# big-nacho/patolette

Measured on AMD Instinct MI355X. Metric: Mpixels/sec quantized (256-color ICtCp + KMeans) at 1 GPU; palette ΔE vs ref, higher is better.
Workload: dtype f64

## Files before the change

### include/patolette_amd.h

```cpp
#ifndef PATOLETTE_AMD_H
#define PATOLETTE_AMD_H

#include <stddef.h>
#include <stdint.h>

#include "patolette.h"

#ifdef __cplusplus
extern "C" {
#endif

int  patolette_amd_device_count(void);
int  patolette_amd_set_device(int ordinal);
const char *patolette_amd_last_error(void);
void *patolette_amd_malloc(size_t bytes);
void patolette_amd_free(void *dptr);
int  patolette_amd_memcpy_h2d(void *dst, const void *src, size_t bytes);
int  patolette_amd_memcpy_d2h(void *dst, const void *src, size_t bytes);
int  patolette_amd_synchronize(void);
void patolette_amd_release_workspace(void);
int  patolette_amd_fill_image(double *d_planar, size_t n, uint64_t seed);
int  patolette_amd_fill_weights(double *d_weights, size_t n, uint64_t seed);

void patolette_amd_device(size_t width, size_t height, const double *d_data, const double *d_weights,
// ... 74 lines not shown
void patolette_amd_measure_device(size_t frames, size_t width, size_t height, const unsigned char *d_pixels, int channels,
                                  const void *d_palette_maps, int map_elem_bytes, const double *palette,
                                  const unsigned char *palette_u8, size_t palette_rows, long long skip_index, uint64_t *entry_count,
                                  uint64_t *entry_sse, uint32_t *entry_max_se, uint64_t *frame_count, uint64_t *frame_sse,
                                  uint32_t *frame_max_se, double *frame_d_sum, double *frame_d_max, int *exit_code);

void patolette_amd_gif_lzw(size_t frames, size_t width, size_t height, const unsigned char *maps, const int32_t *rects,
                           int min_code_size, size_t segment, unsigned char *out, size_t capacity, uint64_t *offsets, int *exit_code);
void patolette_amd_gif_lzw_device(size_t frames, size_t width, size_t height, const unsigned char *d_maps, const int32_t *rects,
                                  int min_code_size, size_t segment, unsigned char *out, size_t capacity, uint64_t *offsets,
                                  int *exit_code);

void patolette_amd_rgba(size_t width, size_t height, const unsigned char *pixels, int alpha_threshold, const double *weights,
                        double tile_size, size_t palette_size, const patolette__QuantizationOptions *options, double *palette,
                        unsigned char *palette_rgba, void *palette_map, int map_elem_bytes, unsigned char *quantized,
                        int *transparent_index, int *exit_code);
void patolette_amd_rgba_device(size_t width, size_t height, const unsigned char *d_pixels, int alpha_threshold, const double *d_weights,
                               double tile_size, size_t palette_size, const patolette__QuantizationOptions *options, double *palette,
                               unsigned char *palette_rgba, void *d_palette_map, int map_elem_bytes, unsigned char *d_quantized,
                               int *transparent_index, int *exit_code);

void patolette_amd_remap_rgba_u8(size_t frames, size_t width, size_t height, const unsigned char *pixels, int alpha_threshold,
                                 const double *palette, const unsigned char *palette_u8, size_t palette_rows, int transparent_index,
                                 int mode, double spread, void *palette_map, int map_elem_bytes, unsigned char *quantized,
                                 int *exit_code);
void patolette_amd_remap_rgba_u8_device(size_t frames, size_t width, size_t height, const unsigned char *d_pixels, int alpha_threshold,
                                        const double *palette, const unsigned char *palette_u8, size_t palette_rows,
                                        int transparent_index, int mode, double spread, void *d_palette_map, int map_elem_bytes,
                                        unsigned char *d_quantized, int *exit_code);
int patolette_amd_debug_rgba_stamp_quad(int mode);

size_t patolette_amd_hist_bytes(int weighted);
int patolette_amd_hist_clear(void *d_hist, int weighted);
void patolette_amd_hist_add_u8(void *d_hist, int weighted, size_t frames, size_t width, size_t height, const unsigned char *pixels,
                               int channels, int alpha_threshold, const double *weights, double tile_size, int *exit_code);
void patolette_amd_hist_add_u8_device(void *d_hist, int weighted, size_t frames, size_t width, size_t height, const unsigned char *d_pixels,
                                      int channels, int alpha_threshold, const double *d_weights, double tile_size, int *exit_code);
int patolette_amd_hist_merge(void *d_hist, const void *d_other, int weighted);
void patolette_amd_hist_totals(const void *d_hist, int weighted, uint64_t *pixels, uint64_t *colors, int *exit_code);
void patolette_amd_hist_export(const void *d_hist, int weighted, size_t capacity, unsigned char *colors, uint64_t *counts, double *weights,
                               int *exit_code);
void patolette_amd_hist_palette(const void *d_hist, int weighted, size_t palette_size, const patolette__QuantizationOptions *options,
                                double *palette, unsigned char *palette_u8, int *exit_code);

void patolette_amd_batch(size_t count, size_t width, size_t height, const double *const *data,
                         const double *const *weights, double tile_size, size_t palette_size,
                         const patolette__QuantizationOptions *options, double *const *palettes,
                         size_t *const *palette_maps, int *exit_codes);

void patolette_amd_batch_rows(size_t count, size_t width, size_t height, const double *const *rows,
                              const double *const *weights, double tile_size, size_t palette_size,
                              const patolette__QuantizationOptions *options, double *const *palettes,
                              size_t *const *palette_maps, int *exit_codes);

void patolette_amd_batch_u8(size_t count, size_t width, size_t height, const unsigned char *const *pixels, int channels,
                            const double *const *weights, double tile_size, size_t palette_size,
                            const patolette__QuantizationOptions *options, double *const *palettes,
                            unsigned char *const *palettes_u8, void *const *palette_maps, int map_elem_bytes,
                            unsigned char *const *quantized, int *exit_codes);

void patolette_amd_batch_dmap(size_t count, size_t width, size_t height, const void *const *images, int pixel_format,
                              const double *const *weights, double tile_size, size_t palette_size,
                              const patolette__QuantizationOptions *options, double *const *palettes, void *d_palette_maps,
                              int map_elem_bytes, int *exit_codes);

typedef int (*patolette_amd_allreduce_sum_fn)(void *ctx, void *buffer, size_t count, int dtype);
typedef struct patolette_amd__Comm {
    int rank, size;
    patolette_amd_allreduce_sum_fn allreduce_sum;
    void *ctx;
    int host_buffers;
} patolette_amd__Comm;
void patolette_amd_slice(size_t total_pixels, size_t slice_begin, size_t slice_pixels, const double *slice_data,
                         const double *slice_weights, size_t palette_size, const patolette__QuantizationOptions *options,
                         const patolette_amd__Comm *comm, double *palette, size_t *slice_map, int *exit_code);
void patolette_amd_slice_device(size_t total_pixels, size_t slice_begin, size_t slice_pixels, const double *d_slice_data,
                                const double *d_slice_weights, size_t palette_size, const patolette__QuantizationOptions *options,
                                const patolette_amd__Comm *comm, double *palette, void *d_slice_map, int map_elem_bytes,
                                int *exit_code);
int patolette_amd_set_invariant_sums(int on);
int patolette_amd_set_kmeans_update(int mode);

int patolette_amd_set_split_loop(int mode);
int patolette_amd_set_global_quantiser(int on_device);

int patolette_amd_set_subsample_cache(int on);

int patolette_amd_subsample_indices(size_t n, size_t take, int32_t *out);
int patolette_amd_eigen_sym3(const double a_colmajor[9], double w[3], double z[9]);
int patolette_amd_principal_axis(const double cov6[6], double axis[3]);
int patolette_amd_eigen_sym3_device(const double *a_colmajor, size_t count, double *w, double *z, int *info);
int patolette_amd_pow(const double *x, double y, double *out, size_t n);

enum {
    PAMD_SRGB_TO_ICTCP = 0,
    PAMD_SRGB_TO_CIELUV = 1,
    PAMD_ICTCP_TO_REC2020 = 2,
    PAMD_CIELUV_TO_REC2020 = 3,
    PAMD_SRGB_TO_REC2020 = 4,
    PAMD_REC2020_TO_SRGB = 5,
    PAMD_CIELUV_TO_ICTCP = 6
};
int patolette_amd_convert(int which, double *planar, size_t n);

int patolette_amd_quantize_clusters(const double *colors, const double *weights, size_t n, size_t K,
                                    double *centers, size_t *n_clusters);

int patolette_amd_kmeans_refine(const double *colors, const double *weights, size_t n,
                                double *centers_io, size_t k, int niter, size_t max_samples);
int patolette_amd_debug_km_route(void);

int patolette_amd_nn_map(const double *colors, size_t n, const double *palette, size_t k, size_t *map);
int patolette_amd_debug_nn_route(int route);
int patolette_amd_debug_nn_map_elem(const double *colors, size_t n, const double *palette, size_t k, int map_elem_bytes, int misalign,
                                    void *map);

int patolette_amd_dither(const double *colors, size_t width, size_t height, const double *palette,
                         size_t k, size_t *map);

void patolette_amd_dither_config(int segments, int warm);
void patolette_amd_dither_layout(int lanes);
int patolette_amd_debug_dither_solo_cap(int cap);
int patolette_amd_debug_dither_stall_passes(int n);
int patolette_amd_dither_layout_in_use(size_t width, size_t height, size_t palette_rows);
void patolette_amd_debug_dither_locate(size_t width, size_t height, unsigned long long t, unsigned long long *d, unsigned long long *c);

typedef struct patolette_amd__Stats {
    double ms_total, ms_upload, ms_convert, ms_gq, ms_lq, ms_kmeans, ms_map, ms_download, ms_saliency;
    size_t n_base_clusters;
    size_t n_clusters;
    size_t split_evals;
    size_t split_px;
    size_t lq_rounds;
    size_t kmeans_samples;
    size_t dither_segments;
    size_t dither_repairs;
    size_t dither_rounds;
    size_t dither_through;
    size_t dither_jumps;
    size_t dither_solo;
} patolette_amd__Stats;
void patolette_amd_last_stats(patolette_amd__Stats *out);
size_t patolette_amd_last_map_palette(double *out, size_t capacity_rows);

typedef struct patolette_amd__SplitRecord {
    int32_t row, new_row;
    int32_t split;
    int32_t degenerate;
    uint64_t n, n_left, n_right;
    double sw;
    double axis[3];
    double cov6[6];
    double dist, dist_left, dist_right, benefit;
} patolette_amd__SplitRecord;
typedef struct patolette_amd__SplitTrace {
    int32_t n_base, n_clusters, n_records, stopped_early;
    double gq_axis[3];
    uint64_t gq_cuts[14];
    double gq_cov6[6];
} patolette_amd__SplitTrace;
size_t patolette_amd_last_split_trace(patolette_amd__SplitTrace *hdr, patolette_amd__SplitRecord *recs, size_t capacity);
size_t patolette_amd_last_cluster_centers(double *out, size_t capacity_rows);

int patolette_amd_debug_fault(int which);

int patolette_amd_debug_workspace(int flags);
unsigned long long patolette_amd_debug_late_growths(void);

void patolette_amd_profile_enable(int on);
void patolette_amd_profile_only(const char *kernel_name);
void patolette_amd_profile_sample(int period);
int  patolette_amd_profile_count(void);
int  patolette_amd_profile_get(int i, char *name64, double *total_ms, size_t *launches, double *total_bytes);

#ifdef __cplusplus
}
#endif
#endif
```

### patolette_amd/_native.py

```python
import ctypes as C
import os

HERE = os.path.dirname(os.path.abspath(__file__))
LIB_PATH = os.path.join(HERE, "lib", "libpatolette_amd.so")

dp = C.POINTER(C.c_double)
zp = C.POINTER(C.c_size_t)


class QuantizationOptions(C.Structure):
    _fields_ = [("dither", C.c_bool), ("palette_only", C.c_bool), ("color_space", C.c_int),
                ("kmeans_niter", C.c_int), ("kmeans_max_samples", C.c_size_t), ("verbose", C.c_bool)]


class Stats(C.Structure):
    _fields_ = [(n, C.c_double) for n in ("ms_total", "ms_upload", "ms_convert", "ms_gq", "ms_lq",
                                          "ms_kmeans", "ms_map", "ms_download", "ms_saliency")] + \
               [(n, C.c_size_t) for n in ("n_base_clusters", "n_clusters", "split_evals", "split_px",
                                          "lq_rounds", "kmeans_samples", "dither_segments", "dither_repairs",
                                          "dither_rounds", "dither_through", "dither_jumps", "dither_solo")]

    def as_dict(self):
        return {n: getattr(self, n) for n, _ in self._fields_}

# ... 31 lines not shown
    "patolette_amd_set_device": (C.c_int, [C.c_int]),
    "patolette_amd_last_error": (C.c_char_p, []),
    "patolette_amd_malloc": (C.c_void_p, [C.c_size_t]),
    "patolette_amd_free": (None, [C.c_void_p]),
    "patolette_amd_memcpy_h2d": (C.c_int, [C.c_void_p, C.c_void_p, C.c_size_t]),
    "patolette_amd_memcpy_d2h": (C.c_int, [C.c_void_p, C.c_void_p, C.c_size_t]),
    "patolette_amd_synchronize": (C.c_int, []),
    "patolette_amd_release_workspace": (None, []),
    "patolette_amd_batch_dmap": (None, [C.c_size_t, C.c_size_t, C.c_size_t, C.POINTER(C.c_void_p), C.c_int, C.POINTER(dp), C.c_double,
                                        C.c_size_t, C.POINTER(QuantizationOptions), C.POINTER(dp), C.c_void_p, C.c_int,
                                        C.POINTER(C.c_int)]),
    "patolette_amd_slice": (None, [C.c_size_t, C.c_size_t, C.c_size_t, dp, dp, C.c_size_t, C.POINTER(QuantizationOptions),
                                   C.POINTER(Comm), dp, zp, C.POINTER(C.c_int)]),
    "patolette_amd_slice_device": (None, [C.c_size_t, C.c_size_t, C.c_size_t, C.c_void_p, C.c_void_p, C.c_size_t,
                                          C.POINTER(QuantizationOptions), C.POINTER(Comm), dp, C.c_void_p, C.c_int, C.POINTER(C.c_int)]),
    "patolette_amd_set_invariant_sums": (C.c_int, [C.c_int]),
    "patolette_amd_set_kmeans_update": (C.c_int, [C.c_int]),
    "patolette_amd_set_subsample_cache": (C.c_int, [C.c_int]),
    "patolette_amd_subsample_indices": (C.c_int, [C.c_size_t, C.c_size_t, C.POINTER(C.c_int32)]),
    "patolette_amd_eigen_sym3": (C.c_int, [dp, dp, dp]),
    "patolette_amd_principal_axis": (C.c_int, [dp, dp]),
    "patolette_amd_eigen_sym3_device": (C.c_int, [dp, C.c_size_t, dp, dp, C.POINTER(C.c_int)]),
    "patolette_amd_fill_image": (C.c_int, [C.c_void_p, C.c_size_t, C.c_uint64]),
    "patolette_amd_fill_weights": (C.c_int, [C.c_void_p, C.c_size_t, C.c_uint64]),
    "patolette_amd_device": (None, [C.c_size_t, C.c_size_t, C.c_void_p, C.c_void_p, C.c_size_t,
                                    C.POINTER(QuantizationOptions), dp, C.c_void_p, C.c_int, C.POINTER(C.c_int)]),
    "patolette_amd_quantize": (None, [C.c_size_t, C.c_size_t, dp, dp, C.c_double, C.c_size_t, C.POINTER(QuantizationOptions), dp, zp,
                                      C.POINTER(C.c_int)]),
    "patolette_amd_quantize_rows": (None, [C.c_size_t, C.c_size_t, dp, dp, C.c_double, C.c_size_t, C.POINTER(QuantizationOptions), dp,
                                           zp, C.POINTER(C.c_int)]),
    "patolette_amd_saliency_weights": (C.c_int, [C.c_size_t, C.c_size_t, dp, C.c_double, dp]),
    "patolette_amd_mbd": (C.c_int, [C.c_size_t, C.c_size_t, C.POINTER(C.c_float), C.c_int, C.POINTER(C.c_float)]),
    **_pair("patolette_amd_u8", None, [C.c_size_t, C.c_size_t, C.c_void_p, C.c_int, C.c_void_p, C.c_double, C.c_size_t,
                                       C.POINTER(QuantizationOptions), dp, C.c_void_p, C.c_void_p, C.c_int, C.c_void_p, C.POINTER(C.c_int)]),
    **_pair("patolette_amd_frames_u8", None, [C.c_size_t, C.c_size_t, C.c_size_t, C.c_void_p, C.c_int, C.c_void_p, C.c_double, C.c_size_t,
                                              C.POINTER(QuantizationOptions), dp, C.c_void_p, C.c_void_p, C.c_int, C.c_void_p,
                                              C.POINTER(C.c_int)]),
    **_pair("patolette_amd_remap_u8", None, [C.c_size_t, C.c_size_t, C.c_size_t, C.c_void_p, C.c_int, dp, C.c_void_p, C.c_size_t, C.c_int,
                                             C.c_void_p, C.c_int, C.c_void_p, C.POINTER(C.c_int)]),
    **_pair("patolette_amd_remap_ordered_u8", None, [C.c_size_t, C.c_size_t, C.c_size_t, C.c_void_p, C.c_int, dp, C.c_void_p, C.c_size_t,
                                                     C.c_double, C.c_void_p, C.c_int, C.c_void_p, C.POINTER(C.c_int)]),
    "patolette_amd_debug_remap_two_pass": (C.c_int, [C.c_int]),
    **_pair("patolette_amd_remap_rgba_u8", None, [C.c_size_t, C.c_size_t, C.c_size_t, C.c_void_p, C.c_int, dp, C.c_void_p, C.c_size_t, C.c_int,
                                                  C.c_int, C.c_double, C.c_void_p, C.c_int, C.c_void_p, C.POINTER(C.c_int)]),
    "patolette_amd_debug_rgba_stamp_quad": (C.c_int, [C.c_int]),
    **_pair("patolette_amd_frame_deltas", None, [C.c_size_t, C.c_size_t, C.c_size_t, C.c_void_p, C.c_int, C.c_size_t, C.c_size_t, C.c_void_p,
                                                 C.c_int, dp, C.c_void_p, C.c_double, C.c_void_p, C.c_void_p, C.POINTER(C.c_int32),
                                                 C.POINTER(C.c_uint64), C.POINTER(C.c_int)]),
    **_pair("patolette_amd_frame_deltas_rgba", None, [C.c_size_t, C.c_size_t, C.c_size_t, C.c_void_p, C.c_int, C.c_size_t, C.c_void_p, C.c_int,
                                                      dp, C.c_void_p, C.c_double, C.c_int, C.c_void_p, C.c_void_p, C.POINTER(C.c_int32),
                                                      C.POINTER(C.c_int32), C.POINTER(C.c_uint64), C.POINTER(C.c_int)]),
    "patolette_amd_debug_delta_quad": (C.c_int, [C.c_int]),
    **_pair("patolette_amd_measure", None, [C.c_size_t, C.c_size_t, C.c_size_t, C.c_void_p, C.c_int, C.c_void_p, C.c_int, dp, C.c_void_p,
                                            C.c_size_t, C.c_longlong, C.POINTER(C.c_uint64), C.POINTER(C.c_uint64), C.POINTER(C.c_uint32),
                                            C.POINTER(C.c_uint64), C.POINTER(C.c_uint64), C.POINTER(C.c_uint32), dp, dp,
                                            C.POINTER(C.c_int)]),
    **_pair("patolette_amd_gif_lzw", None, [C.c_size_t, C.c_size_t, C.c_size_t, C.c_void_p, C.POINTER(C.c_int32), C.c_int, C.c_size_t,
                                            C.c_void_p, C.c_size_t, C.POINTER(C.c_uint64), C.POINTER(C.c_int)]),
    **_pair("patolette_amd_rgba", None, [C.c_size_t, C.c_size_t, C.c_void_p, C.c_int, C.c_void_p, C.c_double, C.c_size_t,
                                         C.POINTER(QuantizationOptions), dp, C.c_void_p, C.c_void_p, C.c_int, C.c_void_p,
                                         C.POINTER(C.c_int), C.POINTER(C.c_int)]),
    "patolette_amd_hist_bytes": (C.c_size_t, [C.c_int]),
    "patolette_amd_hist_clear": (C.c_int, [C.c_void_p, C.c_int]),
    **_pair("patolette_amd_hist_add_u8", None, [C.c_void_p, C.c_int, C.c_size_t, C.c_size_t, C.c_size_t, C.c_void_p, C.c_int, C.c_int,
                                                C.c_void_p, C.c_double, C.POINTER(C.c_int)]),
    "patolette_amd_hist_merge": (C.c_int, [C.c_void_p, C.c_void_p, C.c_int]),
    "patolette_amd_hist_totals": (None, [C.c_void_p, C.c_int, C.POINTER(C.c_uint64), C.POINTER(C.c_uint64), C.POINTER(C.c_int)]),
    "patolette_amd_hist_export": (None, [C.c_void_p, C.c_int, C.c_size_t, C.c_void_p, C.POINTER(C.c_uint64), dp, C.POINTER(C.c_int)]),
    "patolette_amd_hist_palette": (None, [C.c_void_p, C.c_int, C.c_size_t, C.POINTER(QuantizationOptions), dp, C.c_void_p,
                                          C.POINTER(C.c_int)]),
    "patolette_amd_batch": (None, [C.c_size_t, C.c_size_t, C.c_size_t, C.POINTER(dp), C.POINTER(dp), C.c_double, C.c_size_t,
                                   C.POINTER(QuantizationOptions), C.POINTER(dp), C.POINTER(zp), C.POINTER(C.c_int)]),
    "patolette_amd_batch_rows": (None, [C.c_size_t, C.c_size_t, C.c_size_t, C.POINTER(dp), C.POINTER(dp), C.c_double, C.c_size_t,
                                        C.POINTER(QuantizationOptions), C.POINTER(dp), C.POINTER(zp), C.POINTER(C.c_int)]),
    "patolette_amd_batch_u8": (None, [C.c_size_t, C.c_size_t, C.c_size_t, C.POINTER(C.c_void_p), C.c_int, C.POINTER(dp), C.c_double, C.c_size_t,
                                      C.POINTER(QuantizationOptions), C.POINTER(dp), C.POINTER(C.c_void_p), C.POINTER(C.c_void_p), C.c_int,
                                      C.POINTER(C.c_void_p), C.POINTER(C.c_int)]),
    "patolette_amd_pow": (C.c_int, [dp, C.c_double, dp, C.c_size_t]),
    "patolette_amd_convert": (C.c_int, [C.c_int, dp, C.c_size_t]),
    "patolette_amd_quantize_clusters": (C.c_int, [dp, dp, C.c_size_t, C.c_size_t, dp, zp]),
    "patolette_amd_kmeans_refine": (C.c_int, [dp, dp, C.c_size_t, dp, C.c_size_t, C.c_int, C.c_size_t]),
    "patolette_amd_nn_map": (C.c_int, [dp, C.c_size_t, dp, C.c_size_t, zp]),
    "patolette_amd_debug_km_route": (C.c_int, []),
    "patolette_amd_debug_nn_route": (C.c_int, [C.c_int]),
    "patolette_amd_debug_nn_map_elem": (C.c_int, [dp, C.c_size_t, dp, C.c_size_t, C.c_int, C.c_int, C.c_void_p]),
    "patolette_amd_set_global_quantiser": (C.c_int, [C.c_int]),
    "patolette_amd_dither": (C.c_int, [dp, C.c_size_t, C.c_size_t, dp, C.c_size_t, zp]),
    "patolette_amd_dither_config": (None, [C.c_int, C.c_int]),
    "patolette_amd_dither_layout": (None, [C.c_int]),
    "patolette_amd_debug_dither_solo_cap": (C.c_int, [C.c_int]),
    "patolette_amd_debug_dither_stall_passes": (C.c_int, [C.c_int]),
    "patolette_amd_dither_layout_in_use": (C.c_int, [C.c_size_t, C.c_size_t, C.c_size_t]),
    "patolette_amd_debug_dither_locate": (None, [C.c_size_t, C.c_size_t, C.c_ulonglong, C.POINTER(C.c_ulonglong),
                                                 C.POINTER(C.c_ulonglong)]),
    "patolette_amd_last_stats": (None, [C.POINTER(Stats)]),
    "patolette_amd_last_map_palette": (C.c_size_t, [dp, C.c_size_t]),
    "patolette_amd_last_split_trace": (C.c_size_t, [C.POINTER(SplitTrace), C.POINTER(SplitRecord), C.c_size_t]),
    "patolette_amd_last_cluster_centers": (C.c_size_t, [dp, C.c_size_t]),
    "patolette_amd_debug_fault": (C.c_int, [C.c_int]),
    "patolette_amd_debug_workspace": (C.c_int, [C.c_int]),
    "patolette_amd_debug_late_growths": (C.c_ulonglong, []),
    "patolette_amd_set_split_loop": (C.c_int, [C.c_int]),
    "patolette_amd_profile_enable": (None, [C.c_int]),
    "patolette_amd_profile_only": (None, [C.c_char_p]),
    "patolette_amd_profile_sample": (None, [C.c_int]),
    "patolette_amd_profile_count": (C.c_int, []),
    "patolette_amd_profile_get": (C.c_int, [C.c_int, C.c_char_p, dp, zp, dp]),
}

_lib = None


def lib():
    global _lib
    if _lib is None:
        if not os.path.exists(LIB_PATH):
            raise ImportError(
                "patolette_amd: %s not found -- build it with `make -C patolette_amd/csrc` "
                "(hipcc, gfx950). There is no CPU fallback." % LIB_PATH)
        L = C.CDLL(LIB_PATH)
        for name, (res, args) in SYMBOLS.items():
            f = getattr(L, name)
            f.restype = res
            f.argtypes = args
        _lib = L
    return _lib


def last_error():
    return lib().patolette_amd_last_error().decode("utf-8", "replace")


def last_stats():
    s = Stats()
    lib().patolette_amd_last_stats(C.byref(s))
    return s.as_dict()


def last_split_trace():
    hdr = SplitTrace()
    n = lib().patolette_amd_last_split_trace(C.byref(hdr), None, 0)
    recs = (SplitRecord * max(1, n))()
    lib().patolette_amd_last_split_trace(C.byref(hdr), recs, n)
    return dict(n_base=hdr.n_base, n_clusters=hdr.n_clusters, stopped_early=bool(hdr.stopped_early),
                gq_axis=[float(v) for v in hdr.gq_axis], gq_cov6=[float(v) for v in hdr.gq_cov6],
                gq_cuts=[int(v) for v in hdr.gq_cuts][:hdr.n_base + 1],
                splits=[dict(row=r.row, new_row=r.new_row, split=r.split, degenerate=r.degenerate, n=r.n, n_left=r.n_left,
                             n_right=r.n_right, sw=r.sw, axis=[float(v) for v in r.axis], cov6=[float(v) for v in r.cov6],
                             dist=r.dist, dist_left=r.dist_left, dist_right=r.dist_right, benefit=r.benefit) for r in recs[:n]])


def last_cluster_centers():
    import numpy as np
    n = lib().patolette_amd_last_cluster_centers(None, 0)
    out = np.zeros((max(1, n), 3), order="F")
    lib().patolette_amd_last_cluster_centers(out.ctypes.data_as(dp), max(1, n))
    return np.ascontiguousarray(out[:n])


def profile(enable=True, only=None, sample=1):
    lib().patolette_amd_profile_only(only.encode() if only else None)
    lib().patolette_amd_profile_sample(int(sample) if only else 1)
    lib().patolette_amd_profile_enable(1 if enable else 0)


def profile_results():
    L = lib()
    out = {}
    for i in range(L.patolette_amd_profile_count()):
        name = C.create_string_buffer(64)
        ms = C.c_double(0)
        n = C.c_size_t(0)
        by = C.c_double(0)
        if L.patolette_amd_profile_get(i, name, C.byref(ms), C.byref(n), C.byref(by)) == 0:
            out[name.value.decode()] = {"total_ms": ms.value, "launches": n.value, "bytes": by.value}
    return out
```

### patolette_amd/csrc/pipeline.hip

```cpp
#include <algorithm>
#include <functional>
#include <chrono>
#include <cmath>
#include <atomic>
#include <memory>
#include <mutex>
#include <thread>
#include <future>
#include <type_traits>

#include "color_device.h"
#include "common.h"
#include "host_math.h"
#include "kmeans.h"
#include "map.h"
#include "ordered.h"
#include "delta.h"
#include "measure.h"
#include "lzw.h"
#include "hist.h"
#include "saliency.h"
#include "quant.h"
#include "rgba.h"
#include "compact.h"
#include "split_frontier.h"
#include "given.h"

namespace pamd {

void launch_convert(int which, const double *src, double *dst, size_t n, ConvertStats *stats, hipStream_t s, BinK sumk = BinK{0.0, 0.0},
                    BinK momk = BinK{0.0, 0.0}, size_t begin = 0, size_t end = ~(size_t)0, bool init_stats = true);
void launch_convert_rows(int which, const double *rows, double *dst, size_t n, ConvertStats *stats, hipStream_t s,
                         BinK sumk = BinK{0.0, 0.0}, BinK momk = BinK{0.0, 0.0}, size_t begin = 0, size_t end = ~(size_t)0,
                         bool init_stats = true);
void launch_convert_u8(int which, const unsigned char *pixels, int channels, double *dst, size_t n, ConvertStats *stats,
                       hipStream_t s, BinK sumk = BinK{0.0, 0.0}, BinK momk = BinK{0.0, 0.0}, size_t begin = 0, size_t end = ~(size_t)0,
                       bool init_stats = true);
void launch_reconstruct(const void *map, int map_elem, size_t n, const unsigned char *pal_u8, int k, unsigned char *out,
                        hipStream_t s);
void launch_weight_stats(const double *w, size_t n, ConvertStats *stats, hipStream_t s);
void launch_pow(const double *x, double y, double *out, size_t n, hipStream_t s);
void launch_fill_image(double *d, size_t n, uint64_t seed, hipStream_t s);
void launch_fill_weights(double *d, size_t n, uint64_t seed, hipStream_t s);

KernelTimer &ktimer() { static thread_local KernelTimer *t = new KernelTimer; return *t; }

std::atomic<int> g_debug_ws{getenv("PAMD_DEBUG_WORKSPACE") ? atoi(getenv("PAMD_DEBUG_WORKSPACE")) & (kWsPoison | kWsCount | kWsLog) : 0};
std::atomic<unsigned long long> g_late_growths{0};
WsStreams &ws_streams() { static thread_local WsStreams w; return w; }
void ws_growth(size_t bytes, const char *file, int line) {
    const int dbg = g_debug_ws.load(std::memory_order_relaxed);
    if (!(dbg & (kWsCount | kWsLog))) return;
    bool queued = false;
    for (const hipStream_t *sp : ws_streams().s)
        if (sp && *sp && hipStreamQuery(*sp) == hipErrorNotReady) queued = true;
    if (!queued) return;
    g_late_growths.fetch_add(1);
    if (dbg & kWsLog) fprintf(stderr, "patolette_amd: workspace growth to %zu bytes while work is queued (%s:%d)\n", bytes, file, line);
}
void ws_poison_dev(void *p, size_t bytes) {
    if (!bytes) return;
    HIP_CHECK(hipMemsetAsync(p, 0xFF, bytes, nullptr));
    HIP_CHECK(hipStreamSynchronize(nullptr));
}
void ws_poison_dev_rows(void *p, size_t pitch, size_t width, size_t rows) {
    if (!width || !rows) return;
    HIP_CHECK(hipMemset2DAsync(p, pitch, 0xFF, width, rows, nullptr));
    HIP_CHECK(hipStreamSynchronize(nullptr));
}
int KernelTimer::id_of(const char *name) {
    for (size_t i = 0; i < names.size(); i++) if (names[i] == name) return (int)i;
    names.emplace_back(name); total_ms.push_back(0); total_bytes.push_back(0); launches.push_back(0);
    return (int)names.size() - 1;
}
hipEvent_t KernelTimer::get_event() {
    if (!pool.empty()) { hipEvent_t e = pool.back(); pool.pop_back(); return e; }
    hipEvent_t e; HIP_CHECK(hipEventCreate(&e)); return e;
}
void KernelTimer::begin(int id, hipStream_t s, double bytes, const double *src) {
    Rec r; r.id = id; r.bytes = bytes; r.src = src; r.a = get_event(); r.b = get_event();
    HIP_CHECK(hipEventRecord(r.a, s));
    pending.push_back(r);
}
void KernelTimer::end(hipStream_t s) { HIP_CHECK(hipEventRecord(pending.back().b, s)); }
void KernelTimer::collect() {
    for (auto &r : pending) {
        float ms = 0;
        if (hipEventSynchronize(r.b) == hipSuccess && hipEventElapsedTime(&ms, r.a, r.b) == hipSuccess && !(r.src && *r.src == 0.0)) {
            total_ms[r.id] += ms; total_bytes[r.id] += r.src ? r.bytes * *r.src : r.bytes; launches[r.id] += 1;
        }
        pool.push_back(r.a); pool.push_back(r.b);
    }
    pending.clear();
}
void KernelTimer::reset() { collect(); names.clear(); total_ms.clear(); total_bytes.clear(); launches.clear(); }

__global__ __launch_bounds__(256) void k_gq_prepare(Tile *tA, int ntA, Tile *tP, int ntP, unsigned long long N, int *round_nodes, int *node_tile0,
                                                    double *hist, unsigned long long nhist, unsigned long long *hsize, unsigned int *hcount) {
    const unsigned long long stride = (unsigned long long)gridDim.x * blockDim.x, t0 = (unsigned long long)blockIdx.x * blockDim.x + threadIdx.x;
    for (unsigned long long i = t0; i < (unsigned long long)ntA; i += stride) {
        const unsigned long long o = i * (unsigned long long)kTileA;
        tA[i] = Tile{o, (unsigned)(N - o < (unsigned long long)kTileA ? N - o : (unsigned long long)kTileA), 0u};
    }
    for (unsigned long long i = t0; i < (unsigned long long)ntP; i += stride) {
        const unsigned long long o = i * (unsigned long long)kTileP;
        tP[i] = Tile{o, (unsigned)(N - o < (unsigned long long)kTileP ? N - o : (unsigned long long)kTileP), 0u};
    }
    for (unsigned long long i = t0; i < nhist; i += stride) hist[i] = 0.0;
    for (unsigned long long i = t0; i < (unsigned long long)kBuckets; i += stride) { hsize[i] = 0ULL; hcount[i] = 0u; }
    if (t0 == 0) { round_nodes[0] = 0; node_tile0[0] = 0; node_tile0[1] = ntP; }
}

__global__ void k_put_nodes(NodeDev *table, const NodeIn *stage, const int *ids, int n) {
    int i = blockIdx.x * blockDim.x + threadIdx.x;
    if (i >= n) return;
    const NodeIn in = stage[i];
    NodeDev &d = table[ids[i]];
    d.begin = in.begin; d.n = in.n; d.gn = in.gn; d.buf = in.buf; d.slot = in.slot; d.child0 = in.child0; d.nchild = in.nchild;
    for (int j = 0; j < 3; j++) { d.axis[j] = in.axis[j]; d.mean[j] = in.mean[j]; }
    d.sw = in.sw; d.klin = in.klin; d.kquad = in.kquad;
    node_reset_outputs(d);
    d.split = in.split; d.psplit = -1;
}
__global__ void k_put_node1(NodeDev *table, const int id, const NodeIn in) {
    NodeDev &d = table[id];
    d.begin = in.begin; d.n = in.n; d.gn = in.gn; d.buf = in.buf; d.slot = in.slot; d.child0 = in.child0; d.nchild = in.nchild;
    for (int j = 0; j < 3; j++) { d.axis[j] = in.axis[j]; d.mean[j] = in.mean[j]; }
    d.sw = in.sw; d.klin = in.klin; d.kquad = in.kquad;
    node_reset_outputs(d);
    d.split = in.split; d.psplit = -1;
}
__global__ void k_get_nodes(const NodeDev *table, NodeOut *stage, const int *ids, int n) {
    int i = blockIdx.x * blockDim.x + threadIdx.x;
    if (i >= n) return;
    const NodeDev &d = table[ids[i]];
    NodeOut o;
    o.begin = d.begin; o.n = d.n; o.gn = d.gn; o.buf = d.buf; o.degenerate = d.degenerate; o.split = d.split; o.psplit = d.psplit;
    o.sw = d.sw;
    for (int j = 0; j < 3; j++) o.mean[j] = d.mean[j];
    for (int q = 0; q < 7; q++) {
        double s0 = 0, s1 = 0;
        for (int k = 0; k < kSlots; k++) { s0 += d.acc[k][q][0]; s1 += d.acc[k][q][1]; }
        o.acc[q][0] = s0; o.acc[q][1] = s1;
    }
    stage[i] = o;
}

struct RoundSetup {
    const NodeIn *recs; const int *ids; const int *tA0; const int *tP0;
    int nr, ntA, ntP;
    Tile *tilesA, *tilesP;
    double *hist; size_t nhist;
    unsigned long long *hsize; unsigned int *hcount; size_t nbk;
};
__device__ __forceinline__ int node_of_tile(const int *t0, int nr, int t) {
    int lo = 0, hi = nr;
    while (hi - lo > 1) { const int mid = (lo + hi) >> 1; if (t0[mid] <= t) lo = mid; else hi = mid; }
    return lo;
}
__global__ __launch_bounds__(256) void k_round_setup(NodeDev *table, RoundSetup a) {
    const size_t tid = (size_t)blockIdx.x * blockDim.x + threadIdx.x, stride = (size_t)gridDim.x * blockDim.x;
    for (size_t i = tid; i < (size_t)a.nr; i += stride) {
        const NodeIn in = a.recs[i];
        NodeDev &d = table[a.ids[i]];
        d.begin = in.begin; d.n = in.n; d.gn = in.gn; d.buf = in.buf; d.slot = in.slot; d.child0 = in.child0; d.nchild = in.nchild;
        for (int j = 0; j < 3; j++) { d.axis[j] = in.axis[j]; d.mean[j] = in.mean[j]; }
        d.sw = in.sw; d.klin = in.klin; d.kquad = in.kquad;
    }
    for (size_t i = tid; i < (size_t)a.nr * kNodeResetElems; i += stride)
        node_reset_element(table[a.ids[i / kNodeResetElems]], (int)(i % kNodeResetElems));
    for (size_t t = tid; t < (size_t)a.ntA; t += stride) {
        const int r = node_of_tile(a.tA0, a.nr, (int)t);
        const unsigned long long o = (unsigned long long)((int)t - a.tA0[r]) * kTileA, n = a.recs[r].n;
        a.tilesA[t] = Tile{a.recs[r].begin + o, (unsigned)(n - o < (unsigned long long)kTileA ? n - o : kTileA), (unsigned)a.ids[r]};
    }
    for (size_t t = tid; t < (size_t)a.ntP; t += stride) {
        const int r = node_of_tile(a.tP0, a.nr, (int)t);
        const unsigned long long o = (unsigned long long)((int)t - a.tP0[r]) * kTileP, n = a.recs[r].n;
        a.tilesP[t] = Tile{a.recs[r].begin + o, (unsigned)(n - o < (unsigned long long)kTileP ? n - o : kTileP), (unsigned)a.ids[r]};
    }
    for (size_t i = tid; i < a.nhist; i += stride) a.hist[i] = 0.0;
    for (size_t i = tid; i < a.nbk; i += stride) { a.hsize[i] = 0ULL; a.hcount[i] = 0u; }
}


struct GqOut { int kbase, error, pad[2]; int cuts[16]; unsigned long long ticks[8]; };

constexpr int kLqDevMaxK = 256;
constexpr int kLqNodeCap = 16 * kLqDevMaxK + 256;
constexpr int kLqRoundCap = 512;
constexpr int kLqMaxRounds = 96;

struct LqCen { double mean[3]; double gn; };
// ... 576 lines not shown
    for (int k = 0; k < kSlots; k++) { a = d.minkey[k] < a ? d.minkey[k] : a; b = d.maxkey[k] > b ? d.maxkey[k] : b; }
    for (int r = 0; r < size; r++) {
        unsigned long long *row = buf + ((size_t)r * n + i) * 3;
        row[0] = r == rank ? a : 0ULL; row[1] = r == rank ? b : 0ULL; row[2] = r == rank ? d.n : 0ULL;
    }
}
__global__ void k_shard_unpack_keys(NodeDev *table, const int *ids, int n, int rank, int size, const unsigned long long *buf) {
    const int i = blockIdx.x * blockDim.x + threadIdx.x;
    if (i >= n) return;
    NodeDev &d = table[ids[i]];
    unsigned long long a = ~0ULL, b = 0ULL, before = 0ULL;
    for (int r = 0; r < size; r++) {
        const unsigned long long *row = buf + ((size_t)r * n + i) * 3;
        a = row[0] < a ? row[0] : a; b = row[1] > b ? row[1] : b;
        if (r < rank) before += row[2];
    }
    for (int k = 0; k < kSlots; k++) { d.minkey[k] = ~0ULL; d.maxkey[k] = 0ULL; }
    d.minkey[0] = a; d.maxkey[0] = b; d.gslot0 = before;
}
__global__ void k_shard_pack_acc(const NodeDev *table, const int *ids, int n, double *buf) {
    const int i = blockIdx.x * blockDim.x + threadIdx.x;
    if (i >= n) return;
    const NodeDev &d = table[ids[i]];
    for (int q = 0; q < 7; q++) {
        double s0 = 0, s1 = 0;
        for (int k = 0; k < kSlots; k++) { s0 += d.acc[k][q][0]; s1 += d.acc[k][q][1]; }
        buf[(size_t)i * 14 + 2 * q] = s0; buf[(size_t)i * 14 + 2 * q + 1] = s1;
    }
}
__global__ void k_shard_unpack_acc(NodeDev *table, const int *ids, int n, const double *buf) {
    const int i = blockIdx.x * blockDim.x + threadIdx.x;
    if (i >= n) return;
    NodeDev &d = table[ids[i]];
    for (int q = 0; q < 7; q++) {
        for (int k = 1; k < kSlots; k++) { d.acc[k][q][0] = 0; d.acc[k][q][1] = 0; }
        d.acc[0][q][0] = buf[(size_t)i * 14 + 2 * q]; d.acc[0][q][1] = buf[(size_t)i * 14 + 2 * q + 1];
    }
}
__global__ void k_shard_children_local(NodeDev *table, const int *round_nodes, int nround) {
    const int i = blockIdx.x * blockDim.x + threadIdx.x;
    if (i >= nround) return;
    const NodeDev &nd = table[round_nodes[i]];
    for (int k = 0; k < nd.nchild; k++) {
        NodeDev &ch = table[nd.child0 + k];
        ch.begin = nd.cbegin[k]; ch.n = nd.cbegin[k + 1] - nd.cbegin[k];
    }
}

struct Bounds {
    double cmax, range, wmax; int e_lin, e_quad; double lo[3], hi[3];
    bool have_sum = false; double sum[3] = {0, 0, 0};
    bool have_mom = false;
    double sum2[3][2] = {{0, 0}, {0, 0}, {0, 0}}, mom2[6][2] = {{0, 0}, {0, 0}, {0, 0}, {0, 0}, {0, 0}, {0, 0}};
    bool nonfinite = false;
    double wmin = 0; bool bad_w = false;
};

static int exp_bound(double v) {
    if (!(v > 0) || !std::isfinite(v)) return 1;
    return std::ilogb(v) + 1;
}

struct Shard {
    size_t total = 0, begin = 0;
    patolette_amd__Comm comm{};
};

struct Engine {
    int device = -1;
    hipStream_t stream = nullptr;
    const Shard *shard = nullptr;
    bool invariant = false;
    DevBuf<unsigned char> commbuf;
    PinBuf<unsigned char> h_comm;
    DevBuf<int> shard_ids;
    PinBuf<float> h_cent;
    PinBuf<ConvertStats> h_cstats;
    hipEvent_t ev_stats = nullptr;
    hipStream_t stream2 = nullptr;
    hipEvent_t ev_up[2] = {nullptr, nullptr}, ev_join = nullptr;
    size_t prep_N = 0, prep_planes = 0;
    DevBuf<double> src, wsrc, cvt, bufA, bufB, aux;
    DevBuf<unsigned short> bkt;
    DevBuf<NodeDev> nodes;
    DevBuf<NodeIn> stage_in;
    DevBuf<NodeOut> stage_out;
    DevBuf<int> ids, round_nodes, node_tile0;
    DevBuf<Tile> tilesA, tilesP;
    DevBuf<double> hist, sum6, dpal;
    DevBuf<unsigned long long> hsize, tileoff;
    DevBuf<unsigned int> hcount, tilecnt;
    DevBuf<unsigned char> lut, dmap, src8, pal8, quant8;
    DevBuf<unsigned char> dl_maps, dl_shown;
    DevBuf<unsigned long long> dl_words, dl_masks;
    DevBuf<unsigned long long> ms_words;
    DevBuf<MeasureTile> ms_tiles;
    DevBuf<unsigned> ms_p8;
    DevBuf<LzwFrame> lz_frames;
    DevBuf<unsigned> lz_stage, lz_bits, lz_out;
    DevBuf<unsigned long long> lz_gbit, lz_words;
    DevBuf<unsigned> rgba_cnt;
    DevBuf<int> rgba_cpos;
    DevBuf<unsigned char> rgba_rgb, rgba_map;
    DevBuf<double> rgba_w;
    PinBuf<unsigned> h_rgba_m;
    DevBuf<unsigned> rr_words;
    PinBuf<unsigned> h_rr_words;
    DevBuf<unsigned long long> hs_units, hs_words, hs_counts;
    DevBuf<unsigned> hs_tiles;
    DevBuf<unsigned char> hs_rgb;
    DevBuf<double> hs_w;
    DevBuf<ConvertStats> cstats;
    PinBuf<NodeIn> h_stage_in;
    PinBuf<NodeOut> h_stage_out;
    PinBuf<int> h_ids, h_ids_get;
    PinBuf<int> h_round;
    PinBuf<double> h_dbl;
    PinBuf<unsigned char> h_bytes, h_packet, h_mapstage;
    DevBuf<unsigned char> packet;
    KMeansWork km;
    NNWork nn;
    SalWork sal;
    DevBuf<double> wsal;
    DevBuf<GqDpDev> gq;
    PinBuf<GqDpDev> h_gq;
    DevBuf<GqOut> gqout;
    PinBuf<GqOut> h_gqout;
    PinBuf<double> h_pal;
    DevBuf<LqCtl> lqctl;
    PinBuf<LqHead> h_lqhead;
    PinBuf<LqRec> h_lqrec;
    PinBuf<LqCen> h_lqcen;
    std::vector<LqRec> lq_rec_local;
    std::vector<LqCommit> lq_commits;
    bool trace_pending = false;
    size_t lq_hint_N = 0, lq_hint_K = 0; int lq_hint_rounds = 0;
    DevBuf<int> perm_dev;
    size_t perm_N = 0, perm_nx = 0;
    PinBuf<int32_t> h_perm;
    size_t hperm_N = 0, hperm_nx = 0;
    hm::PermScratch perm_ws;
    std::future<void> perm_job;
    patolette_amd__Stats stats{};
    double ms_saliency = 0.0;
    std::string last_error;
    std::vector<double> map_palette;
    patolette_amd__SplitTrace trace_hdr{};
    std::vector<patolette_amd__SplitRecord> trace;
    std::vector<double> cluster_centers;

    void init() {
        if (stream) return;
        int cnt = 0;
        if (hipGetDeviceCount(&cnt) != hipSuccess || cnt <= 0)
            throw HipError("patolette_amd: no HIP device available (this library has no CPU fallback)");
        if (device < 0) { HIP_CHECK(hipGetDevice(&device)); }
        HIP_CHECK(hipSetDevice(device));
        HIP_CHECK(hipStreamCreateWithFlags(&stream, hipStreamNonBlocking));
    }
    void sync() { HIP_CHECK(hipStreamSynchronize(stream)); if (ktimer().enabled) ktimer().collect(); }
    ~Engine() {
        if (stream) { (void)hipSetDevice(device); (void)hipStreamSynchronize(stream); if (ev_stats) (void)hipEventDestroy(ev_stats);
                      for (hipEvent_t e : {ev_up[0], ev_up[1], ev_join}) if (e) (void)hipEventDestroy(e);
                      if (stream2) (void)hipStreamDestroy(stream2);
                      (void)hipStreamDestroy(stream); }
    }
// ... 126 lines not shown
    NodeIn d;
    std::memset(&d, 0, sizeof d);
    d.begin = h.begin; d.n = h.n; d.gn = h.gn; d.buf = h.buf; d.slot = -1; d.child0 = -1; d.nchild = 0; d.split = -1;
    for (int j = 0; j < 3; j++) d.mean[j] = h.mean[j];
    d.sw = h.sw;
    int P = 1;
    while ((1ULL << P) < (h.gn > 1 ? h.gn : 2)) P++;
    d.klin = make_bink(b.e_lin, P);
    d.kquad = make_bink(b.e_quad, P);
    return d;
}

static void put_nodes(Engine &E, const std::vector<int> &ids, const std::vector<NodeIn> &recs) {
    const int n = (int)ids.size();
    if (!n) return;
    if (n == 1) {
        hipLaunchKernelGGL(k_put_node1, 1, 1, 0, E.stream, E.nodes.p, ids[0], recs[0]);
        HIP_CHECK(hipGetLastError());
        return;
    }
    E.stage_in.reserve(n); E.ids.reserve(n); E.h_stage_in.reserve(n); E.h_ids.reserve(n);
    std::memcpy(E.h_stage_in.p, recs.data(), n * sizeof(NodeIn));
    std::memcpy(E.h_ids.p, ids.data(), n * sizeof(int));
    HIP_CHECK(hipMemcpyAsync(E.stage_in.p, E.h_stage_in.p, n * sizeof(NodeIn), hipMemcpyHostToDevice, E.stream));
    HIP_CHECK(hipMemcpyAsync(E.ids.p, E.h_ids.p, n * sizeof(int), hipMemcpyHostToDevice, E.stream));
    hipLaunchKernelGGL(k_put_nodes, (n + 63) / 64, 64, 0, E.stream, E.nodes.p, E.stage_in.p, E.ids.p, n);
    HIP_CHECK(hipGetLastError());
}

static void get_nodes(Engine &E, const std::vector<int> &ids, std::vector<NodeOut> &recs) {
    const int n = (int)ids.size();
    recs.resize(n);
    if (!n) return;
    E.stage_out.reserve(n); E.ids.reserve(n); E.h_stage_out.reserve(n); E.h_ids_get.reserve(n);
    std::memcpy(E.h_ids_get.p, ids.data(), n * sizeof(int));
    HIP_CHECK(hipMemcpyAsync(E.ids.p, E.h_ids_get.p, n * sizeof(int), hipMemcpyHostToDevice, E.stream));
    hipLaunchKernelGGL(k_get_nodes, (n + 63) / 64, 64, 0, E.stream, E.nodes.p, E.stage_out.p, E.ids.p, n);
    HIP_CHECK(hipGetLastError());
    HIP_CHECK(hipMemcpyAsync(E.h_stage_out.p, E.stage_out.p, n * sizeof(NodeOut), hipMemcpyDeviceToHost, E.stream));
    E.sync();
    std::memcpy(recs.data(), E.h_stage_out.p, n * sizeof(NodeOut));
}

static void get_nodes_dev(Engine &E, const int *d_ids, int n, std::vector<NodeOut> &recs) {
    recs.resize(n);
    if (!n) return;
    E.h_stage_out.reserve(n);
    hipLaunchKernelGGL(k_get_nodes, (n + 63) / 64, 64, 0, E.stream, E.nodes.p, E.h_stage_out.p, d_ids, n);
    HIP_CHECK(hipGetLastError());
    E.sync();
    std::memcpy(recs.data(), E.h_stage_out.p, n * sizeof(NodeOut));
}

static void absorb_moments(HNode &h, const NodeOut &d) {
    for (int q = 0; q < 6; q++) h.cov6[q] = d.acc[q][0] + d.acc[q][1];
    h.dist = d.acc[6][0] + d.acc[6][1];
}

static bool node_axis(const HNode &h, double axis[3]) {
    if (h.axis_state != 0) {
        for (int j = 0; j < 3; j++) axis[j] = h.axis[j];
        return h.axis_state > 0;
    }
    double c6[6];
    for (int q = 0; q < 6; q++) c6[q] = h.cov6[q] / h.sw;
    return hm::principal_axis(c6, axis);
}

static void leaf_bound(HNode &h) {
    h.ub = h.dist;
    h.axis_state = 0;
    if (h.gn <= 1 || !(h.sw > 0)) { h.ub = 0; return; }
    double c6[6];
    for (int q = 0; q < 6; q++) c6[q] = h.cov6[q] / h.sw;
    double a[9] = {c6[0], c6[1], c6[2], c6[1], c6[3], c6[4], c6[2], c6[4], c6[5]};
    double w[3];
    if (hm::eigen_sym3(a, w) != 0) { h.axis_state = -1; return; }
    h.axis[0] = a[6]; h.axis[1] = a[7]; h.axis[2] = a[8]; h.axis_state = 1;
    const double b = w[2] * h.sw * (1.0 + 1e-9) + 1e-9 * h.dist;
    if (b == b && b < h.ub) h.ub = b;
}

struct QuantSizes {
    size_t bufA, bufB, bkt, tilesA, tilesP, tilecnt, tileoff, hist, hsize, hcount, lut;
    QuantSizes(size_t pixels, size_t planes, size_t nodes) {
        const size_t slack = nodes > 1 ? nodes : 0;
        bufA = bufB = planes * pixels + 64;
        bkt = pixels;
        tilesA = ceil_div(pixels, (size_t)kTileA) + slack; tilesP = ceil_div(pixels, (size_t)kTileP) + slack;
        tilecnt = tileoff = tilesP * kMaxChildren;
        hist = std::max(hist_slot_doubles(), (size_t)kNQ_LQ * 2 * kBuckets * nodes);
        hsize = hcount = lut = nodes * kBuckets;
    }
};
static void reserve_quant_tables(Engine &E, const QuantSizes &z, const char *file = __builtin_FILE(), int line = __builtin_LINE()) {
    E.bufA.reserve(z.bufA, file, line); E.bufB.reserve(z.bufB, file, line); E.bkt.reserve(z.bkt, file, line);
    E.tilesA.reserve(z.tilesA, file, line); E.tilesP.reserve(z.tilesP, file, line);
    E.tilecnt.reserve(z.tilecnt, file, line); E.tileoff.reserve(z.tileoff, file, line);
    E.hist.reserve(z.hist, file, line); E.hsize.reserve(z.hsize, file, line); E.hcount.reserve(z.hcount, file, line); E.lut.reserve(z.lut, file, line);
}

static void gq_prepare(Engine &E, size_t N, bool weighted) {
    hipStream_t s = E.stream;
    const size_t planes = weighted ? 4 : 3;
    const QuantSizes z(N, planes, 1);
    reserve_quant_tables(E, z);
    const int ntA = (int)z.tilesA, ntP = (int)z.tilesP;
    E.h_round.reserve(kBuckets);
    E.round_nodes.reserve(1); E.node_tile0.reserve(2);
    const size_t hs = hist_slot_doubles();
    hipLaunchKernelGGL(k_gq_prepare, 64, 256, 0, s, E.tilesA.p, ntA, E.tilesP.p, ntP, (unsigned long long)N, E.round_nodes.p, E.node_tile0.p,
                       E.hist.p, (unsigned long long)hs, E.hsize.p, E.hcount.p);
    HIP_CHECK(hipGetLastError());
    E.prep_N = N; E.prep_planes = planes;
}



std::atomic<int> g_lq_device{getenv("PAMD_LQ_DEVICE") ? atoi(getenv("PAMD_LQ_DEVICE")) : 2};
std::atomic<int> g_gq_device{getenv("PAMD_GQ_DEVICE") ? atoi(getenv("PAMD_GQ_DEVICE")) : 1};
constexpr size_t kLqDeviceAutoPixels = (size_t)40 << 20;

static bool lq_device_eligible(const Engine &E, size_t N, size_t K, bool verbose, bool allow_device) {
    const int lq_mode = g_lq_device.load(std::memory_order_relaxed);
    return allow_device && (lq_mode == 1 || (lq_mode == 2 && N < kLqDeviceAutoPixels)) && !E.shard && !verbose && K <= (size_t)kLqDevMaxK;
}

static void ws_prepare(Engine &E, size_t N, size_t K, bool weighted, bool verbose) {
    const size_t planes = weighted ? 4 : 3;
    const bool lq_dev = lq_device_eligible(E, N, K, verbose, true);
    E.cvt.reserve(planes * N); E.cstats.reserve(1);
    reserve_quant_tables(E, QuantSizes(N, planes, lq_dev ? (size_t)kLqRoundCap : 1));
    E.round_nodes.reserve(1); E.node_tile0.reserve(2); E.h_round.reserve(kBuckets);
    E.nodes.reserve(std::max<size_t>(4 * K + 64, lq_dev ? (size_t)kLqNodeCap : 0));
    E.h_dbl.reserve(16 * kBuckets * 2 + 64);
    E.gq.reserve(1); E.gqout.reserve(1); E.h_gqout.reserve(1); E.h_gq.reserve(1);
    const size_t nput = kGqMaxK + 1;
    E.stage_in.reserve(nput); E.stage_out.reserve(nput); E.ids.reserve(nput); E.h_stage_in.reserve(nput); E.h_stage_out.reserve(nput);
    E.h_ids.reserve(nput); E.h_ids_get.reserve(nput);
    E.h_cent.reserve(3 * K);
    if (lq_dev) { E.lqctl.reserve(1); E.h_lqhead.reserve(1); E.h_lqrec.reserve(kLqNodeCap); E.h_lqcen.reserve(kLqNodeCap); }
}

static int lq_device_loop(Engine &E, size_t N, size_t K, bool weighted, bool inv_sums, const Bounds &bnd, const QuantBuffers &qlq, int kbase,
                          int first_base, int nnodes, std::vector<double> &centers, size_t &len, unsigned long long *max_members) {
    hipStream_t s = E.stream;
    const size_t lqs = (size_t)kNQ_LQ * 2 * kBuckets;
    const QuantSizes z(N, weighted ? 4 : 3, kLqRoundCap);
    const int ntA_ub = (int)z.tilesA, ntP_ub = (int)z.tilesP;
    E.lqctl.reserve(1); E.h_lqhead.reserve(1); E.h_lqrec.reserve(kLqNodeCap); E.h_lqcen.reserve(kLqNodeCap);
    reserve_quant_tables(E, z);
    LqCtl *c = E.lqctl.p;
    LqHead *head = E.h_lqhead.p;
    for (int r = 0; r < kLqMaxRounds; r++) { head->round_px[r] = 0.0; head->round_nr[r] = 0.0; }
    const RoundDyn *dyn = &c->dyn;
    const int *d_round = c->round_ids, *d_tP0 = c->tP0;
    int call = 0;
    const GqOut *gq = kbase < 0 ? (const GqOut *)E.gqout.p : nullptr;
    const int kb_ub = kbase < 0 ? kGqMaxK : kbase;
    auto control = [&]() {
        const bool first = call == 0;
        {
            KTIME("k_lq_children", s, 0.0);
            if (first) hipLaunchKernelGGL(k_lq_children, (kb_ub + 3) / 4, 256, 0, s, E.nodes.p, c, call, kb_ub, first_base, nnodes, (int)K, gq);
            else hipLaunchKernelGGL(k_lq_children, 2 * kLqRoundCap / 4, 256, 0, s, E.nodes.p, c, call, 0, 0, 0, 0, (const GqOut *)nullptr);
        }
        KTIME("k_lq_select", s, 0.0);
        hipLaunchKernelGGL(k_lq_select, 1 + (first ? (kb_ub + 3) / 4 : 2 * kLqRoundCap / 4), 256, 0, s, E.nodes.p, c, call, bnd.e_lin, bnd.e_quad);
        HIP_CHECK(hipGetLastError());
        call++;
    };
    int enq = 0;
    auto round = [&]() {
        if (enq >= kLqMaxRounds) throw HipError("patolette_amd: split loop exceeded its round limit");
        const double *px_src = &head->round_px[enq], *nr_src = &head->round_nr[enq];
        const bool rev = enq % 2 == 1;
        static const bool setup_kernel = getenv("PAMD_LQ_SETUP_KERNEL") && atoi(getenv("PAMD_LQ_SETUP_KERNEL")) != 0;
        if (setup_kernel) {
            hipLaunchKernelGGL(k_round_setup_dyn, 1024, 256, 0, s, E.nodes.p, (const LqCtl *)c, E.tilesA.p, E.tilesP.p, E.hist.p, E.hsize.p, E.hcount.p, lqs);
            HIP_CHECK(hipGetLastError());
            launch_minmax(qlq, E.tilesA.p, ntA_ub, 0, E.nodes.p, s, rev, dyn, px_src);
        } else {
            const RoundLists rl{c->round_ids, c->tA0, c->tP0, E.tilesA.p, E.tilesP.p, E.hist.p, lqs, E.hsize.p, E.hcount.p};
            launch_minmax(qlq, E.tilesA.p, ntA_ub, 0, E.nodes.p, s, rev, dyn, px_src, &rl);
        }
        launch_hist(qlq, false, E.tilesA.p, ntA_ub, 0, E.nodes.p, E.hist.p, E.hsize.p, E.hcount.p, s, !rev, false, dyn, px_src);
        launch_cut(weighted, E.nodes.p, d_round, kLqRoundCap, E.hist.p, E.hsize.p, E.hcount.p, E.lut.p, s, dyn, nr_src);
        launch_partition(qlq, E.tilesP.p, ntP_ub, 0, d_round, d_tP0, kLqRoundCap, E.nodes.p, E.lut.p, E.tilecnt.p, E.tileoff.p, true, s, inv_sums, rev, dyn, px_src);
        enq++;
        control();
    };
    control();
    int want = (E.lq_hint_N == N && E.lq_hint_K == K && E.lq_hint_rounds > 0) ? E.lq_hint_rounds : 9;
    const bool fault_full = g_debug_fault.load(std::memory_order_relaxed) == 4;
    if (fault_full) want = 3;
    for (;;) {
        while (enq < want) round();
        hipLaunchKernelGGL(k_lq_export, 16, 256, 0, s, (const LqCtl *)c, head, E.h_lqrec.p, E.h_lqcen.p);
        HIP_CHECK(hipGetLastError());
        E.sync();
        if (fault_full) return -2;
        if (head->done) break;
        want = enq + 2;
    }
    if (head->error == 2) return -2;
    if (head->error == 3) return -1;
    if (kbase < 0) kbase = E.h_gqout.p->kbase;
    E.lq_hint_N = N; E.lq_hint_K = K; E.lq_hint_rounds = head->rounds;
    LqReplay rp;
    const double t_rp0 = now_ms();
    E.lq_rec_local.resize((size_t)head->nnodes);
    std::memcpy(E.lq_rec_local.data(), E.h_lqrec.p, (size_t)head->nnodes * sizeof(LqRec));
    const int fault = g_debug_fault.load(std::memory_order_relaxed);
    const bool replay_ok = lq_replay(E.lq_rec_local.data(), kbase, first_base, K, kDelta, fault, rp);
    const double t_rp1 = now_ms();
    static const bool replay_check = getenv("PAMD_LQ_REPLAY_CHECK") != nullptr;
    if (replay_check || !replay_ok) {
        LqReplay ref;
        const bool ref_ok = lq_replay_plain(E.lq_rec_local.data(), kbase, first_base, K, kDelta, fault, ref);
        if (ref_ok != replay_ok || ref.result != rp.result || ref.stopped_early != rp.stopped_early)
            fprintf(stderr, "patolette_amd: split loop: the two replays DISAGREE (plain %d, %zu rows; blocked %d, %zu rows), kbase %d, K %zu, nodes %d, rounds %d\n",
                    (int)ref_ok, ref.result.size(), (int)replay_ok, rp.result.size(), kbase, K, head->nnodes, head->rounds);
        else if (!replay_ok)
            fprintf(stderr, "patolette_amd: split loop: both replays blocked after %zu commits, kbase %d, K %zu, nodes %d, rounds %d, evaluated %d, tau %.17g\n",
                    rp.commits.size(), kbase, K, head->nnodes, head->rounds, head->neval, head->tau);
    }
    if (!replay_ok) throw HipError("patolette_amd: split loop: the replay met an unevaluated node");
    len = rp.result.size();
    centers.assign(3 * len, 0.0);
    unsigned long long mg = 0;
    for (size_t i = 0; i < len; i++) {
        const LqCen &cn = E.h_lqcen.p[rp.result[i]];
        for (int j = 0; j < 3; j++) centers[(size_t)j * len + i] = cn.mean[j];
        mg = std::max(mg, (unsigned long long)cn.gn);
    }
    if (max_members) *max_members = mg;
    E.stats.split_evals = (size_t)head->split_evals; E.stats.split_px = (size_t)head->split_px; E.stats.lq_rounds = (size_t)head->rounds;
    E.lq_commits.swap(rp.commits);
    E.trace.clear();
    E.trace_pending = true;
    E.trace_hdr.stopped_early = rp.stopped_early ? 1 : 0;
    static const bool lq_times = getenv("PAMD_LQ_TIMES") != nullptr;
    if (lq_times) {
        fprintf(stderr, "patolette_amd: device-driven split loop: %d rounds, %d evaluated, %zu commits, tau %.3g; host replay %.1f us\n", head->rounds, head->neval,
                E.lq_commits.size(), head->tau, 1e3 * (t_rp1 - t_rp0));
        if (gq) {
            const unsigned long long *t = E.h_gqout.p->ticks;
            fprintf(stderr, "patolette_amd: k_gq_control us: prefixes %.1f, axis %.1f, search %.1f, records %.1f\n", (t[1] - t[0]) * 0.01, (t[2] - t[1]) * 0.01,
                    (t[3] - t[2]) * 0.01, (t[4] - t[3]) * 0.01);
            fprintf(stderr, "patolette_amd: k_gq_control us: of the prefixes, staging %.1f\n", (t[5] - t[0]) * 0.01);
        }
    }
    return 0;
}

static void materialise_trace(Engine &E) {
    if (!E.trace_pending) return;
    E.trace_pending = false;
    const int n = (int)E.lq_commits.size();
    E.trace.assign(n, patolette_amd__SplitRecord{});
    if (!n) return;
    DevBuf<LqCommit> dc; DevBuf<patolette_amd__SplitRecord> dr;
    dc.reserve(n); dr.reserve(n);
    HIP_CHECK(hipMemcpyAsync(dc.p, E.lq_commits.data(), sizeof(LqCommit) * n, hipMemcpyHostToDevice, E.stream));
    hipLaunchKernelGGL(k_lq_trace, (n + 63) / 64, 64, 0, E.stream, (const NodeDev *)E.nodes.p, (const LqCommit *)dc.p, n, dr.p);
    HIP_CHECK(hipGetLastError());
    HIP_CHECK(hipMemcpyAsync(E.trace.data(), dr.p, sizeof(patolette_amd__SplitRecord) * n, hipMemcpyDeviceToHost, E.stream));
    HIP_CHECK(hipStreamSynchronize(E.stream));
}

struct QuantCall {
// ... 9 lines not shown
    double t0;
    std::vector<HNode> hn;
    bool mom_path = false;
    double axis[3] = {0, 0, 0};
    int kbase = 0;
    std::vector<int> base_ids;
    std::vector<NodeOut> got;
};

static void gq_root_mean(QuantCall &C) {
    Engine &E = C.E;
    const size_t Nt = C.Nt;
    const Bounds &bnd = C.bnd;
    HNode root; root.begin = 0; root.n = C.N; root.gn = Nt; root.buf = 0; root.sw = (double)Nt;
    E.h_dbl.reserve(16 * kBuckets * 2 + 64);
    if (bnd.have_sum) {
        const double inv = 1 / (double)Nt;
        for (int j = 0; j < 3; j++) root.mean[j] = bnd.sum[j] * inv;
    } else {
        int rootP = 1; while ((1ULL << rootP) < (Nt > 1 ? Nt : 2)) rootP++;
        E.sum6.reserve(kSum3Slots * 6);
        launch_sum3(E.cvt.p, C.N, make_bink(bnd.e_lin, rootP), E.sum6.p, E.stream);
        if (C.sh) comm_sum_dev(E, E.sum6.p, kSum3Slots * 6, 0);
        HIP_CHECK(hipMemcpyAsync(E.h_dbl.p, E.sum6.p, kSum3Slots * 6 * sizeof(double), hipMemcpyDeviceToHost, E.stream));
        E.sync();
        const double inv = 1 / (double)Nt;
        for (int j = 0; j < 3; j++) {
            double p0 = 0, p1 = 0;
            for (int sl = 0; sl < kSum3Slots; sl++) { p0 += E.h_dbl.p[sl * 6 + 2 * j]; p1 += E.h_dbl.p[sl * 6 + 2 * j + 1]; }
            root.mean[j] = (p0 + p1) * inv;
        }
    }
    C.hn.push_back(root);
}

static void gq_root_covariance(QuantCall &C) {
    Engine &E = C.E;
    const Bounds &bnd = C.bnd;
    std::vector<HNode> &hn = C.hn;
    C.mom_path = bnd.have_mom && !C.sh;
    if (C.mom_path) {
        const long double nn = (long double)C.Nt;
        long double s1[3], c6[6], s2d[3] = {0, 0, 0};
        for (int j = 0; j < 3; j++) s1[j] = (long double)bnd.sum2[j][0] + (long double)bnd.sum2[j][1];
        static const int ja[6] = {0, 1, 2, 1, 2, 2}, jb[6] = {0, 0, 0, 1, 1, 2};
        for (int q = 0; q < 6; q++) {
            const long double s2 = (long double)bnd.mom2[q][0] + (long double)bnd.mom2[q][1];
            if (ja[q] == jb[q]) s2d[ja[q]] = s2;
            c6[q] = s2 - s1[ja[q]] * s1[jb[q]] / nn;
        }
        const long double tr = c6[0] + c6[3] + c6[5], tr2 = s2d[0] + s2d[1] + s2d[2];
        if (!(tr > 1e-6L * tr2) || c6[0] < 0 || c6[3] < 0 || c6[5] < 0) C.mom_path = false;
        else {
            for (int q = 0; q < 6; q++) hn[0].cov6[q] = (double)c6[q];
            hn[0].dist = (double)tr;
        }
    }
    if (!C.mom_path) {
        NodeIn d = make_nodedev(hn[0], bnd);
        put_nodes(E, {0}, {d});
        launch_cov_nodes(C.qroot, E.cvt.p, E.tilesA.p, C.ntA0, C.N, E.nodes.p, E.stream, true);
        if (C.sh) shard_exchange_acc(E, shard_upload_ids(E, {0}), 1);
        get_nodes(E, {0}, C.got);
        absorb_moments(hn[0], C.got[0]);
    }
}

static bool gq_root_histogram(QuantCall &C) {
    Engine &E = C.E;
    hipStream_t s = E.stream;
    const HNode &root = C.hn[0];
    if (!node_axis(root, C.axis)) return false;
    E.trace.clear();
    E.trace_pending = false;
    E.trace_hdr = patolette_amd__SplitTrace{};
    for (int j = 0; j < 3; j++) E.trace_hdr.gq_axis[j] = C.axis[j];
    for (int q = 0; q < 6; q++) E.trace_hdr.gq_cov6[q] = root.cov6[q] / root.sw;
    {
        NodeIn d = make_nodedev(root, C.bnd);
        for (int j = 0; j < 3; j++) d.axis[j] = C.axis[j];
        d.slot = 0;
        put_nodes(E, {0}, {d});
    }
    launch_minmax(C.qroot, E.tilesA.p, C.ntA0, C.N, E.nodes.p, s, C.mom_path);
    if (C.sh) shard_exchange_keys(E, shard_upload_ids(E, {0}), 1);
    launch_hist(C.qroot, true, E.tilesA.p, C.ntA0, C.N, E.nodes.p, E.hist.p, E.hsize.p, E.hcount.p, s, !C.mom_path, C.Nt >= ((size_t)1 << 18));
    if (C.sh) { comm_sum_dev(E, E.hist.p, C.hs, 0); comm_sum_dev(E, E.hcount.p, kBuckets, 2); }
    return true;
}

static void gq_trace_header(Engine &E) {
    const GqOut &o = *E.h_gqout.p;
    E.trace_hdr.n_base = o.kbase;
    for (int j = 0; j <= o.kbase && j < 14; j++) E.trace_hdr.gq_cuts[j] = (size_t)o.cuts[j];
}

static int finish_device_loop(QuantCall &C, int kbase, int first_base, int nnodes) {
    Engine &E = C.E;
    if (kbase >= 0) E.stats.n_base_clusters = (size_t)kbase;
    E.stats.ms_gq = now_ms() - C.t0;
    C.t0 = now_ms();
    const int rc = lq_device_loop(E, C.N, C.K, C.weighted, C.inv_sums, C.bnd, C.qlq, kbase, first_base, nnodes, C.centers, C.len, C.max_members);
    if (kbase < 0) {
        gq_trace_header(E);
        E.stats.n_base_clusters = (size_t)E.h_gqout.p->kbase;
    }
    if (rc != 0) return rc;
    E.stats.n_clusters = C.len;
    E.trace_hdr.n_clusters = (int32_t)C.len; E.trace_hdr.n_records = (int32_t)E.lq_commits.size();
    E.cluster_centers = C.centers;
    E.stats.ms_lq = now_ms() - C.t0;
    return 0;
}

constexpr int kHostLoop = 1;

static int gq_device_turn(QuantCall &C) {
    Engine &E = C.E;
    hipStream_t s = E.stream;
    E.gq.reserve(1); E.gqout.reserve(1); E.h_gqout.reserve(1);
    *E.h_gqout.p = GqOut{};
    {
        KTIME("k_gq_control", s, (double)C.hs * 8);
        hipLaunchKernelGGL(k_gq_control, 1, 1024, 0, s, (const double *)E.hist.p, (const unsigned int *)E.hcount.p, E.gq.p, (int)std::min<size_t>(C.K, (size_t)1 << 30),
                           C.weighted ? 1 : 0, E.nodes.p, 1, E.lut.p, E.gqout.p, E.h_gqout.p);
        HIP_CHECK(hipGetLastError());
    }
    launch_partition(C.qroot, E.tilesP.p, C.ntP0, C.N, E.round_nodes.p, E.node_tile0.p, 1, E.nodes.p, E.lut.p, E.tilecnt.p, E.tileoff.p, true, s, C.inv_sums,
                     C.mom_path, nullptr, nullptr, true);
    launch_cov_children(C.qroot, E.tilesA.p, C.ntA0, C.N, E.nodes.p, s, !C.mom_path, true);
    if (C.dev_eligible) return finish_device_loop(C, -1, 1, 0);
    std::vector<int> all(kGqMaxK);
    for (int j = 0; j < kGqMaxK; j++) all[j] = 1 + j;
    get_nodes(E, all, C.got);
    if (E.h_gqout.p->error) return -1;
    gq_trace_header(E);
    C.kbase = E.h_gqout.p->kbase;
    for (int j = 0; j < C.kbase; j++) {
        const NodeOut &g = C.got[j];
        HNode c; c.buf = 1; c.begin = g.begin; c.n = g.n; c.gn = g.gn; c.sw = g.sw;
        for (int q = 0; q < 3; q++) c.mean[q] = g.mean[q];
        absorb_moments(c, g);
        leaf_bound(c);
        C.base_ids.push_back((int)C.hn.size());
        C.hn.push_back(c);
    }
    return kHostLoop;
}

static int gq_host_turn(QuantCall &C) {
    Engine &E = C.E;
    hipStream_t s = E.stream;
    const size_t K = C.K, hs = C.hs;
    const bool weighted = C.weighted;
    std::vector<HNode> &hn = C.hn;
    const int gq_kmax = (int)std::min<size_t>(K, kGqMaxK);
    E.gq.reserve(1); E.h_gq.reserve(1);
    launch_gq_dp(E.hist.p, E.hcount.p, gq_kmax, E.gq.p, s);
    HIP_CHECK(hipMemcpyAsync(E.h_gq.p->cut, E.gq.p->cut, sizeof(E.h_gq.p->cut), hipMemcpyDeviceToHost, s));
    std::vector<double> hh(hs);
    std::vector<unsigned int> hc(kBuckets);
    HIP_CHECK(hipMemcpyAsync(E.h_dbl.p, E.hist.p, hs * sizeof(double), hipMemcpyDeviceToHost, s));
    E.h_round.reserve(kBuckets);
    HIP_CHECK(hipMemcpyAsync(E.h_round.p, E.hcount.p, kBuckets * sizeof(unsigned int), hipMemcpyDeviceToHost, s));
    E.sync();
    std::memcpy(hh.data(), E.h_dbl.p, hs * sizeof(double));
    std::memcpy(hc.data(), E.h_round.p, kBuckets * sizeof(unsigned int));
// ... 106 lines not shown
    leaf_bound(c);
}

static double lq_round_threshold(const SplitFrontier &F, size_t K) {
    double thr = std::max(kDelta, kSpecBeta * F.reference_benefit());
    const size_t R = K - F.count;
    std::vector<double> kb;
    F.known_values(kb);
    if (kb.size() >= R && R > 0) {
        std::nth_element(kb.begin(), kb.begin() + (R - 1), kb.end(), std::greater<double>());
        thr = std::max(thr, kb[R - 1] * (1.0 - 1e-9));
    }
    return thr;
}

static void lq_host_round(QuantCall &C, LqHostLoop &L) {
    Engine &E = C.E;
    hipStream_t s = E.stream;
    std::vector<HNode> &hn = C.hn;
    LqLaps &laps = L.laps;
    const HnRec rec{hn};
    const double thr = lq_round_threshold(L.F, C.K);
    laps.lap(laps.greedy);
    std::vector<int> round;
    {
        std::vector<int> keep;
        for (int id : L.leaves) {
            HNode &h = hn[id];
            if (hn_known(h)) continue;
            if (h.ub >= thr) round.push_back(id); else keep.push_back(id);
        }
        L.leaves.swap(keep);
    }
    if (round.empty()) {
        throw HipError("patolette_amd: split loop blocked without candidates");
    }
    laps.lap(laps.select);
    HIP_CHECK(hipStreamSynchronize(s));
    E.nodes.grow(hn.size() + 2 * round.size() + 2, hn.size());
    std::vector<int> todo;
    std::vector<NodeIn> recs;
    for (int id : round) {
        double ax[3];
        if (!node_axis(hn[id], ax)) { hn[id].nosplit = true; continue; }
        NodeIn d = make_nodedev(hn[id], C.bnd);
        for (int j = 0; j < 3; j++) d.axis[j] = ax[j];
        d.slot = (int)todo.size();
        d.child0 = (int)hn.size(); d.nchild = 2;
        hn[id].left = (int)hn.size(); hn[id].right = (int)hn.size() + 1;
        hn.push_back(HNode()); hn.push_back(HNode());
        todo.push_back(id); recs.push_back(d);
    }
    L.F.reload(rec);
    laps.lap(laps.axes);
    if (todo.empty()) return;
    const int nr = (int)todo.size();
    size_t rpx = 0;
    for (int id : todo) rpx += hn[id].n;
    static const bool lq_trace = getenv("PAMD_LQ_TRACE") != nullptr;
    if (lq_trace) fprintf(stderr, "patolette_amd: split round %zu: %d nodes, %zu pixels (%.2f of the image), %zu of %zu colours committed\n",
                          E.stats.lq_rounds + 1, nr, rpx, (double)rpx / (double)(C.N ? C.N : 1), L.F.count, C.K);
    std::vector<int> cids;
    for (int id : todo) { cids.push_back(hn[id].left); cids.push_back(hn[id].right); }
    std::vector<int> tAg = {0}, tPg = {0};
    for (int id : todo) {
        const unsigned long long n = hn[id].n;
        tAg.push_back(tAg.back() + (int)((n + kTileA - 1) / kTileA)); tPg.push_back(tPg.back() + (int)((n + kTileP - 1) / kTileP));
    }
    const int ntA = tAg[nr], ntP = tPg[nr];
    const size_t o_recs = 0, o_ids = o_recs + (size_t)nr * sizeof(NodeIn), o_cids = o_ids + (size_t)nr * sizeof(int),
                 o_tA = o_cids + cids.size() * sizeof(int), o_tP = o_tA + tAg.size() * sizeof(int),
                 pk_bytes = o_tP + tPg.size() * sizeof(int);
    E.h_packet.reserve(pk_bytes); E.packet.reserve(pk_bytes);
    const size_t lqs = (size_t)kNQ_LQ * 2 * kBuckets;
    reserve_quant_tables(E, QuantSizes(C.N, C.weighted ? 4 : 3, (size_t)nr));
    E.h_stage_out.reserve(cids.size());
    std::memcpy(E.h_packet.p + o_recs, recs.data(), (size_t)nr * sizeof(NodeIn));
    std::memcpy(E.h_packet.p + o_ids, todo.data(), (size_t)nr * sizeof(int));
    std::memcpy(E.h_packet.p + o_cids, cids.data(), cids.size() * sizeof(int));
    std::memcpy(E.h_packet.p + o_tA, tAg.data(), tAg.size() * sizeof(int));
    std::memcpy(E.h_packet.p + o_tP, tPg.data(), tPg.size() * sizeof(int));
    laps.lap(laps.packet);
    HIP_CHECK(hipMemcpyAsync(E.packet.p, E.h_packet.p, pk_bytes, hipMemcpyHostToDevice, s));
    const bool rev = E.stats.lq_rounds % 2 == 1;
    const int *d_ids = (const int *)(E.packet.p + o_ids), *d_cids = (const int *)(E.packet.p + o_cids);
    const int *d_tA0 = (const int *)(E.packet.p + o_tA), *d_tP0 = (const int *)(E.packet.p + o_tP);
    RoundSetup rs{(const NodeIn *)(E.packet.p + o_recs), d_ids, d_tA0, d_tP0, nr, ntA, ntP,
                  E.tilesA.p, E.tilesP.p, E.hist.p, lqs * nr, E.hsize.p, E.hcount.p, (size_t)nr * kBuckets};
    {
        const size_t work = std::max<size_t>(std::max<size_t>(std::max<size_t>(ntP, lqs * nr / 4), (size_t)nr * kNodeResetElems), 256);
        hipLaunchKernelGGL(k_round_setup, (unsigned)std::min<size_t>((work + 255) / 256, 2048), 256, 0, s, E.nodes.p, rs);
        HIP_CHECK(hipGetLastError());
    }
    launch_minmax(C.qlq, E.tilesA.p, ntA, rpx, E.nodes.p, s, rev);
    if (C.sh) shard_exchange_keys(E, d_ids, nr);
    launch_hist(C.qlq, false, E.tilesA.p, ntA, rpx, E.nodes.p, E.hist.p, E.hsize.p, E.hcount.p, s, !rev);
    if (C.sh) {
        comm_sum_dev(E, E.hist.p, lqs * nr, 0);
        if (C.weighted) comm_sum_dev(E, E.hsize.p, (size_t)nr * kBuckets, 1);
        comm_sum_dev(E, E.hcount.p, (size_t)nr * kBuckets, 2);
    }
    launch_cut(C.weighted, E.nodes.p, d_ids, nr, E.hist.p, E.hsize.p, E.hcount.p, E.lut.p, s);
    launch_partition(C.qlq, E.tilesP.p, ntP, rpx, d_ids, d_tP0, nr, E.nodes.p, E.lut.p, E.tilecnt.p, E.tileoff.p, true, s, C.inv_sums, rev);
    if (C.sh) {
        hipLaunchKernelGGL(k_shard_children_local, (nr + 63) / 64, 64, 0, s, E.nodes.p, d_ids, nr);
        HIP_CHECK(hipGetLastError());
        shard_exchange_acc(E, d_cids, 2 * nr);
    }
    laps.lap(laps.enqueue);
    get_nodes_dev(E, d_cids, (int)cids.size(), C.got);
    laps.lap(laps.wait);
    for (size_t i = 0; i < cids.size(); i++) absorb_child(hn[cids[i]], C.got[i]);
    for (int id : todo) { hn[id].split_done = true; E.stats.split_evals++; E.stats.split_px += hn[id].n; }
    for (int id : cids) L.leaves.push_back(id);
    L.F.reload(rec);
    E.stats.lq_rounds++;
    laps.lap(laps.children);
}

static void lq_host_loop(QuantCall &C, LqHostLoop &L) {
    Engine &E = C.E;
    const std::vector<HNode> &hn = C.hn;
    const HnRec rec{hn};
    SplitFrontier &F = L.F;
    E.stats.split_evals = 0; E.stats.split_px = 0; E.stats.lq_rounds = 0;
    if (F.count >= C.K) return;
    while (F.count < C.K) {
        const SplitFrontier::Step st = F.step(rec, g_debug_fault.load(std::memory_order_relaxed));
        if (st.status == SplitFrontier::kBlocked) { lq_host_round(C, L); continue; }
        if (st.status == SplitFrontier::kStopped) { E.trace_hdr.stopped_early = 1; break; }
        const HNode &h = hn[st.commit.node];
        const int l = st.commit.left, r = l + 1;
        patolette_amd__SplitRecord tr{};
        tr.row = st.commit.row; tr.new_row = st.commit.new_row;
        tr.split = hn[l].psplit < 0 ? -1 : (hn[l].psplit & 0xffff); tr.degenerate = hn[l].psplit < 0 ? 0 : (hn[l].psplit >> 16) & 1;
        tr.n = h.gn; tr.n_left = hn[l].gn; tr.n_right = hn[r].gn; tr.sw = h.sw;
        for (int j = 0; j < 3; j++) tr.axis[j] = h.axis[j];
        for (int q = 0; q < 6; q++) tr.cov6[q] = h.cov6[q] / h.sw;
        tr.dist = h.dist; tr.dist_left = hn[l].dist; tr.dist_right = hn[r].dist; tr.benefit = st.benefit;
        E.trace.push_back(tr);
        if (C.verbose) { printf("patolette ======== Processed colors: %zu\r", F.count); fflush(stdout); }
    }
    const LqLaps &t = L.laps;
    if (t.on) fprintf(stderr, "patolette_amd: split loop host ms: greedy %.3f select %.3f axes %.3f packet %.3f enqueue %.3f wait(gpu) %.3f children %.3f\n",
                      t.greedy, t.select, t.axes, t.packet, t.enqueue, t.wait, t.children);
}

static void lq_host_epilogue(QuantCall &C, const SplitFrontier &F) {
    Engine &E = C.E;
    const std::vector<HNode> &hn = C.hn;
    const size_t len = C.len = F.count;
    C.centers.assign(3 * len, 0.0);
    for (size_t i = 0; i < len; i++) for (int j = 0; j < 3; j++) C.centers[(size_t)j * len + i] = hn[F.result[i]].mean[j];
    if (C.max_members) { *C.max_members = 0; for (size_t i = 0; i < len; i++) *C.max_members = std::max(*C.max_members, hn[F.result[i]].gn); }
    E.stats.n_clusters = len;
    E.trace_hdr.n_clusters = (int32_t)len; E.trace_hdr.n_records = (int32_t)E.trace.size();
    E.cluster_centers = C.centers;
    E.stats.ms_lq = now_ms() - C.t0;
}

static int quantize_clusters_run(Engine &E, size_t N, size_t K, bool weighted, const Bounds &bnd,
                                 std::vector<double> &centers, size_t &len, bool verbose, unsigned long long *max_members, bool allow_device) {
    const size_t planes = weighted ? 4 : 3;
    const Shard *sh = E.shard;
    if (E.prep_N != N || E.prep_planes != planes) gq_prepare(E, N, weighted);
    E.prep_N = 0;
    const bool dev_eligible = lq_device_eligible(E, N, K, verbose, allow_device);
    E.nodes.reserve(std::max<size_t>(4 * K + 64, dev_eligible ? (size_t)kLqNodeCap : 0));
    const QuantSizes root(N, planes, 1);
    QuantCall C{E, N, sh ? sh->total : N, K, weighted, sh || E.invariant, verbose, dev_eligible, sh, bnd, centers, len, max_members,
                QuantBuffers{{E.cvt.p, E.bufA.p}, E.bkt.p, N, weighted}, QuantBuffers{{E.bufB.p, E.bufA.p}, E.bkt.p, N, weighted},
                (int)root.tilesA, (int)root.tilesP, hist_slot_doubles(), now_ms()};
    C.hn.reserve(4 * K + 64);

    gq_root_mean(C);
    gq_root_covariance(C);
    if (!gq_root_histogram(C)) return -1;
    const bool gq_dev = g_gq_device.load(std::memory_order_relaxed) != 0 && !sh && !verbose && K > (size_t)kGqMaxK;
    const int rc = gq_dev ? gq_device_turn(C) : gq_host_turn(C);
    if (rc != kHostLoop) return rc;
    E.stats.n_base_clusters = (size_t)C.kbase;
    if (verbose) printf("patolette ======== Base cluster count: %zu\n", (size_t)C.kbase);
    E.stats.ms_gq = now_ms() - C.t0;
    C.t0 = now_ms();

    LqHostLoop L{SplitFrontier(K, C.kbase, C.base_ids[0], kDelta, HnRec{C.hn}), C.base_ids, LqLaps{}};
    lq_host_loop(C, L);
    lq_host_epilogue(C, L.F);
    return 0;
}

static int quantize_clusters(Engine &E, size_t N, size_t K, bool weighted, const Bounds &bnd,
                             std::vector<double> &centers, size_t &len, bool verbose = false, unsigned long long *max_members = nullptr) {
    WsGuard wg(&E.stream, &E.stream2);
    int rc = quantize_clusters_run(E, N, K, weighted, bnd, centers, len, verbose, max_members, true);
    if (rc == -2) {
        E.prep_N = 0;
        rc = quantize_clusters_run(E, N, K, weighted, bnd, centers, len, verbose, max_members, false);
    }
    return rc;
}

std::atomic<int> g_km_update{-1};
std::atomic<int> g_perm_cache{1};

static void subsample_start(Engine &E, size_t Nt, size_t K, size_t max_samples) {
    if (E.perm_job.valid()) {
        try { E.perm_job.get(); } catch (...) { E.hperm_N = 0; E.hperm_nx = 0; }
    }
    const size_t ms = std::max(max_samples, (size_t)(256 * 256));
    if (K == 0 || Nt < K) return;
    const size_t nxK = K * (size_t)(int)(ms / K);
    if (!(Nt > nxK)) return;
    const size_t take = std::min(ms, Nt);
    if (!g_perm_cache.load(std::memory_order_relaxed)) { E.perm_N = 0; E.perm_nx = 0; E.hperm_N = 0; E.hperm_nx = 0; }
    if (E.perm_N == Nt && E.perm_nx >= nxK) return;
    if (E.hperm_N == Nt && E.hperm_nx >= nxK) return;
    E.h_perm.reserve(take);
    E.hperm_N = 0; E.hperm_nx = 0;
    int32_t *dst = E.h_perm.p;
    hm::PermScratch *ws = &E.perm_ws;
    E.perm_job = std::async(std::launch::async, [dst, Nt, take, ws] { hm::rand_perm_prefix(Nt, take, 1234u, dst, *ws); });
    E.hperm_N = Nt; E.hperm_nx = take;
}
static const int *subsample_list(Engine &E, size_t Nt, size_t nx, hipStream_t s) {
    if (E.perm_job.valid()) {
        try { E.perm_job.get(); } catch (...) { E.hperm_N = 0; E.hperm_nx = 0; throw; }
    }
    if (E.perm_N == Nt && E.perm_nx >= nx) return E.perm_dev.p;
    if (!(E.hperm_N == Nt && E.hperm_nx >= nx)) {
        E.h_perm.reserve(nx);
        hm::rand_perm_prefix(Nt, nx, 1234u, E.h_perm.p, E.perm_ws);
        E.hperm_N = Nt; E.hperm_nx = nx;
    }
    E.perm_dev.reserve(E.hperm_nx);
    HIP_CHECK(hipMemcpyAsync(E.perm_dev.p, E.h_perm.p, E.hperm_nx * sizeof(int), hipMemcpyHostToDevice, s));
    E.perm_N = Nt; E.perm_nx = E.hperm_nx;
    return E.perm_dev.p;
}
static bool km_update_order_free() {
    static const bool env = getenv("PAMD_KMEANS_UPDATE") && atoi(getenv("PAMD_KMEANS_UPDATE")) != 0;
    const int v = g_km_update.load(std::memory_order_relaxed);
    return v < 0 ? env : v != 0;
}
static bool km_domain_ok(const double bound_x, const double bound_c, const bool weighted, const double bound_w, const double min_w, const size_t nx) {
    const double fmax = 3.4028234663852886e38, fmin = 1.1754943508222875e-38;
    const double B = std::max(1.0, std::max(bound_x, bound_c)), m = (double)std::min<size_t>(nx, (size_t)1 << 25);
    if (!(B < fmax) || !(bound_w < fmax)) return false;
    double Cb = 8.0 * B;
    if (weighted) {
        if (min_w > 0 && min_w < fmin) return false;
        const double by_n = std::exp(std::min((double)nx * 0x1p-23, 700.0)) * B;
        Cb = 4.0 * (min_w > 0 ? std::min(by_n, 4.0 * m * (std::max(bound_w, min_w) / min_w) * B) : by_n);
    }
// ... 1955 lines not shown
                         double tile_size, size_t palette_size, const patolette__QuantizationOptions *options, double *const *palettes,
                         size_t *const *palette_maps, int *exit_codes) {
    batch_impl(false, count, width, height, data, weights, tile_size, palette_size, options, palettes, palette_maps, exit_codes);
}
void patolette_amd_batch_rows(size_t count, size_t width, size_t height, const double *const *rows, const double *const *weights,
                              double tile_size, size_t palette_size, const patolette__QuantizationOptions *options,
                              double *const *palettes, size_t *const *palette_maps, int *exit_codes) {
    batch_impl(true, count, width, height, rows, weights, tile_size, palette_size, options, palettes, palette_maps, exit_codes);
}

int patolette_amd_pow(const double *x, double y, double *out, size_t n) {
    return guarded([&](Engine &E) -> int {
        if (n == 0) return 0;
        E.src.reserve(2 * n);
        HIP_CHECK(hipMemcpyAsync(E.src.p, x, n * sizeof(double), hipMemcpyHostToDevice, E.stream));
        launch_pow(E.src.p, y, E.src.p + n, n, E.stream);
        HIP_CHECK(hipMemcpyAsync(out, E.src.p + n, n * sizeof(double), hipMemcpyDeviceToHost, E.stream));
        E.sync();
        return 0;
    });
}

int patolette_amd_convert(int which, double *planar, size_t n) {
    return guarded([&](Engine &E) -> int {
        if (n == 0) return 0;
        E.src.reserve(3 * n); E.aux.reserve(3 * n);
        HIP_CHECK(hipMemcpy(E.src.p, planar, 3 * n * sizeof(double), hipMemcpyHostToDevice));
        launch_convert(which, E.src.p, E.aux.p, n, nullptr, E.stream);
        E.sync();
        HIP_CHECK(hipMemcpy(planar, E.aux.p, 3 * n * sizeof(double), hipMemcpyDeviceToHost));
        return 0;
    });
}

int patolette_amd_quantize_clusters(const double *colors, const double *weights, size_t n, size_t K, double *centers, size_t *n_clusters) {
    return guarded([&](Engine &E) -> int {
        if (n == 0 || K == 0) return -1;
        const bool weighted = weights != nullptr;
        E.src.reserve(3 * n);
        E.cvt.reserve((weighted ? 4 : 3) * n);
        E.cstats.reserve(1);
        HIP_CHECK(hipMemcpy(E.src.p, colors, 3 * n * sizeof(double), hipMemcpyHostToDevice));
        launch_convert(PAMD_COPY, E.src.p, E.cvt.p, n, E.cstats.p, E.stream);
        if (weighted) {
            HIP_CHECK(hipMemcpyAsync(E.cvt.p + 3 * n, weights, n * sizeof(double), hipMemcpyHostToDevice, E.stream));
            launch_weight_stats(E.cvt.p + 3 * n, n, E.cstats.p, E.stream);
        }
        Bounds b = read_bounds(E, weighted);
        E.stats = patolette_amd__Stats{};
        std::vector<double> pal;
        size_t len = 0;
        if (quantize_clusters(E, n, K, weighted, b, pal, len) != 0) return -1;
        for (size_t j = 0; j < 3 * K; j++) centers[j] = NAN;
        for (int j = 0; j < 3; j++) for (size_t i = 0; i < len; i++) centers[(size_t)j * K + i] = pal[(size_t)j * len + i];
        *n_clusters = len;
        return 0;
    });
}

int patolette_amd_kmeans_refine(const double *colors, const double *weights, size_t n, double *centers_io, size_t k, int niter, size_t max_samples) {
    return guarded([&](Engine &E) -> int {
        const bool weighted = weights != nullptr;
        E.cvt.reserve((weighted ? 4 : 3) * n);
        HIP_CHECK(hipMemcpy(E.cvt.p, colors, 3 * n * sizeof(double), hipMemcpyHostToDevice));
        if (weighted) HIP_CHECK(hipMemcpy(E.cvt.p + 3 * n, weights, n * sizeof(double), hipMemcpyHostToDevice));
        std::vector<double> pal(centers_io, centers_io + 3 * k);
        bool nonfinite = false;
        double bx = 0, bw = 1, min_w = 0;
        for (size_t i = 0; i < 3 * n && !nonfinite; i++) { nonfinite = !(std::fabs(colors[i]) < 0x1.ffffffp127); bx = std::max(bx, std::fabs(colors[i])); }
        bool bad_w = false;
        if (!nonfinite && weighted) for (size_t i = 0; i < n; i++) {
            const float wf = (float)weights[i];
            bw = std::max(bw, std::fabs(weights[i]));
            if (!(wf >= 0.f) || !std::isfinite(wf)) bad_w = true;
            else if (wf > 0.f && (min_w == 0 || (double)wf < min_w)) min_w = (double)wf;
        }
        kmeans_refine(E, n, weighted, pal, k, niter, max_samples, nonfinite, 0, bx, bw, min_w, bad_w);
        std::memcpy(centers_io, pal.data(), 3 * k * sizeof(double));
        return 0;
    });
}

int patolette_amd_debug_km_route(void) { return holder().e ? holder().e->km.route : 0; }

int patolette_amd_debug_nn_route(int route) { return nn_debug_route(route); }

int patolette_amd_debug_nn_map_elem(const double *colors, size_t n, const double *palette, size_t k, int map_elem_bytes, int misalign, void *map) {
    return guarded([&](Engine &E) -> int {
        const int eb = map_elem_bytes;
        if ((eb != 1 && eb != 4 && eb != 8) || (eb == 1 && k > 256) || k == 0 || (misalign != 0 && (misalign != 1 || eb != 1)))
            throw HipError("patolette_amd_debug_nn_map_elem: elements of 1 (up to 256 rows), 4 or 8 bytes; misalign 0, or 1 with 1-byte elements");
        if (n == 0) return 0;
        E.src.reserve(3 * n); E.dpal.reserve(3 * k); E.dmap.reserve(n * (size_t)eb + 1);
        HIP_CHECK(hipMemcpy(E.src.p, colors, 3 * n * sizeof(double), hipMemcpyHostToDevice));
        HIP_CHECK(hipMemcpy(E.dpal.p, palette, 3 * k * sizeof(double), hipMemcpyHostToDevice));
        launch_nn_map(E.src.p, n, n, E.dpal.p, (int)k, E.dmap.p + misalign, eb, nullptr, nullptr, E.nn, E.stream);
        E.sync();
        HIP_CHECK(hipMemcpy(map, E.dmap.p + misalign, n * (size_t)eb, hipMemcpyDeviceToHost));
        return 0;
    });
}

int patolette_amd_nn_map(const double *colors, size_t n, const double *palette, size_t k, size_t *map) {
    return guarded([&](Engine &E) -> int {
        if (n == 0) return 0;
        E.src.reserve(3 * n); E.dpal.reserve(3 * k); E.dmap.reserve(n * 4);
        HIP_CHECK(hipMemcpy(E.src.p, colors, 3 * n * sizeof(double), hipMemcpyHostToDevice));
        HIP_CHECK(hipMemcpy(E.dpal.p, palette, 3 * k * sizeof(double), hipMemcpyHostToDevice));
        launch_nn_map(E.src.p, n, n, E.dpal.p, (int)k, E.dmap.p, 4, nullptr, nullptr, E.nn, E.stream);
        E.sync();
        download_map(E.dmap.p, 4, n, map, 8);
        return 0;
    });
}

int patolette_amd_dither(const double *colors, size_t width, size_t height, const double *palette, size_t k, size_t *map) {
    return guarded([&](Engine &E) -> int {
        const size_t n = width * height;
        if (n == 0) return 0;
        E.src.reserve(3 * n); E.dpal.reserve(3 * k); E.dmap.reserve(n * 4);
        HIP_CHECK(hipMemcpy(E.src.p, colors, 3 * n * sizeof(double), hipMemcpyHostToDevice));
        HIP_CHECK(hipMemcpy(E.dpal.p, palette, 3 * k * sizeof(double), hipMemcpyHostToDevice));
        launch_dither(E.src.p, n, PAMD_COPY, width, height, E.dpal.p, palette, (int)k, E.dmap.p, 4, E.nn, E.stream);
        copy_dither_stats(E);
        E.sync();
        if (map_touched(true, width, height)) download_map(E.dmap.p, 4, n, map, 8);
        return 0;
    });
}

int patolette_amd_debug_fault(int which) { return g_debug_fault.exchange(which); }
int patolette_amd_debug_workspace(int flags) { return g_debug_ws.exchange(flags & (kWsPoison | kWsCount | kWsLog)); }
unsigned long long patolette_amd_debug_late_growths(void) { return g_late_growths.load(); }
int patolette_amd_set_split_loop(int mode) { return g_lq_device.exchange(mode < 0 || mode > 2 ? 2 : mode); }
int patolette_amd_set_global_quantiser(int on_device) { return g_gq_device.exchange(on_device ? 1 : 0); }
void patolette_amd_dither_config(int segments, int warm) { dither_config(segments, warm); }
void patolette_amd_dither_layout(int lanes) { dither_layout(lanes); }
int patolette_amd_debug_dither_solo_cap(int cap) { return dither_solo_cap(cap); }
int patolette_amd_debug_dither_stall_passes(int n) { return dither_stall_passes(n); }
int patolette_amd_dither_layout_in_use(size_t width, size_t height, size_t k) { return dither_lane_layout(width, height, (int)k) ? 1 : 0; }
void patolette_amd_last_stats(patolette_amd__Stats *out) { *out = engine().stats; }
size_t patolette_amd_last_split_trace(patolette_amd__SplitTrace *hdr, patolette_amd__SplitRecord *recs, size_t capacity) {
    Engine &E = engine();
    try { materialise_trace(E); } catch (const std::exception &e) { E.last_error = e.what(); E.trace.clear(); }
    if (hdr) *hdr = E.trace_hdr;
    if (recs) std::memcpy(recs, E.trace.data(), sizeof *recs * std::min(capacity, E.trace.size()));
    return E.trace.size();
}
size_t patolette_amd_last_cluster_centers(double *out, size_t capacity_rows) {
    Engine &E = engine();
    const size_t len = E.cluster_centers.size() / 3;
    if (out && len <= capacity_rows)
        for (int j = 0; j < 3; j++) for (size_t i = 0; i < len; i++) out[(size_t)j * capacity_rows + i] = E.cluster_centers[(size_t)j * len + i];
    return len;
}
size_t patolette_amd_last_map_palette(double *out, size_t capacity_rows) {
    const std::vector<double> &mp = engine().map_palette;
    const size_t len = mp.size() / 3;
    if (out && capacity_rows >= len)
        for (int j = 0; j < 3; j++) for (size_t i = 0; i < len; i++) out[(size_t)j * capacity_rows + i] = mp[(size_t)j * len + i];
    return len;
}

void patolette_amd_profile_enable(int on) {
    KernelTimer &t = ktimer();
    if (engine().stream) (void)hipStreamSynchronize(engine().stream);
    t.reset();
    t.enabled = on != 0;
}
void patolette_amd_profile_only(const char *kernel_name) { ktimer().only = kernel_name ? kernel_name : ""; ktimer().only_seen = 0; }
void patolette_amd_profile_sample(int period) { ktimer().sample_period = period > 1 ? (unsigned)period : 1u; }
int patolette_amd_profile_count(void) { return (int)ktimer().names.size(); }
int patolette_amd_profile_get(int i, char *name64, double *total_ms, size_t *launches, double *total_bytes) {
    KernelTimer &t = ktimer();
    if (i < 0 || i >= (int)t.names.size()) return -1;
    snprintf(name64, 64, "%s", t.names[i].c_str());
    *total_ms = t.total_ms[i];
    *launches = t.launches[i];
    *total_bytes = t.total_bytes[i];
    return 0;
}

}
```

### patolette_amd/csrc/quant.h

```cpp
#pragma once

#include <atomic>

#include "common.h"
#include "devutil.h"

namespace pamd {

constexpr int kMaxChildren = 16;
constexpr int kTileA = 8192;
constexpr int kTileP = 2048;
constexpr size_t kInfinityCacheBytes = (size_t)256 << 20;

constexpr int kNQ_LQ = 4;
constexpr int kNQ_GQ = 14;

constexpr int kSlots = 16;

struct NodeIn {
    unsigned long long begin, n, gn;
    int buf, slot, child0, nchild;
    int split;
    double axis[3], mean[3], sw;
    BinK klin, kquad;
};
struct NodeOut {
    unsigned long long begin, n, gn;
    int buf, degenerate, split, psplit;
    double sw, mean[3];
    double acc[7][2];
};

struct NodeDev {
    unsigned long long begin;
    unsigned long long n;
    unsigned long long gn;
    unsigned long long gslot0;
    int buf;
    int slot;
    int child0;
    int nchild;
    double axis[3];
    double mean[3];
    double sw;
    BinK klin, kquad;
    unsigned long long minkey[kSlots], maxkey[kSlots];
    int degenerate;
    int split;
    int psplit;
    int axis_state;
    double cov6[6], dist, ub;
    unsigned long long cbegin[kMaxChildren + 1];
    double acc[kSlots][7][2];
};

template <> struct WsPoison<NodeDev> {
    static void dev(NodeDev *p, size_t a, size_t b) {
        char *c = reinterpret_cast<char *>(p + a);
        ws_poison_dev_rows(c + offsetof(NodeDev, axis), sizeof(NodeDev), offsetof(NodeDev, klin) - offsetof(NodeDev, axis), b - a);
        ws_poison_dev_rows(c + offsetof(NodeDev, cov6), sizeof(NodeDev), offsetof(NodeDev, cbegin) - offsetof(NodeDev, cov6), b - a);
        ws_poison_dev_rows(c + offsetof(NodeDev, acc), sizeof(NodeDev), sizeof(NodeDev::acc), b - a);
    }
    static void host(NodeDev *, size_t, size_t) {}
};

__device__ __forceinline__ void node_reset_outputs(NodeDev &d) {
    for (int i = 0; i < kSlots; i++) { d.minkey[i] = ~0ULL; d.maxkey[i] = 0ULL; }
    for (int i = 0; i < kSlots; i++) for (int q = 0; q < 7; q++) { d.acc[i][q][0] = 0; d.acc[i][q][1] = 0; }
    d.degenerate = 0; d.split = -1; d.gslot0 = 0;
}
constexpr int kNodeResetElems = kSlots * 14 + 2 * kSlots;
__device__ __forceinline__ void node_reset_element(NodeDev &d, int e) {
    if (e < kSlots * 14) (&d.acc[0][0][0])[e] = 0.0;
    else if (e < kSlots * 15) d.minkey[e - kSlots * 14] = ~0ULL;
    else d.maxkey[e - kSlots * 15] = 0ULL;
    if (e == 0) { d.degenerate = 0; d.split = -1; d.gslot0 = 0; }
}
__device__ __forceinline__ void node_minmax(const NodeDev &d, double &mn, double &mx) {
    unsigned long long a = ~0ULL, b = 0ULL;
    for (int i = 0; i < kSlots; i++) { a = d.minkey[i] < a ? d.minkey[i] : a; b = d.maxkey[i] > b ? d.maxkey[i] : b; }
    mn = key_f64(a); mx = key_f64(b);
}

struct RoundDyn {
    int nr;
    int ntA, ntP;
    int pad;
};

struct RoundLists {
    const int *round_ids, *tA0, *tP0;
    struct Tile *tilesA, *tilesP;
    double *hist; size_t lqs;
    unsigned long long *hsize; unsigned int *hcount;
};

struct Tile {
    unsigned long long start;
    unsigned int count;
    unsigned int node;
};

struct QuantBuffers {
    double *buf[2];
    unsigned short *bkt;
    size_t N;
    bool weighted;
};

constexpr int kSum3Slots = 32;
void launch_sum3(const double *planar, size_t N, BinK k, double *d_out6, hipStream_t s);
constexpr int kGqMaxK = 12;
struct GqDpDev {
    unsigned long long w0[kBuckets + 1];
    double w1[3][kBuckets + 1], w2[kBuckets + 1];
    double E[2][kBuckets + 1];
    int cut[kGqMaxK + 1][kBuckets + 1];
};
void launch_gq_dp(const double *d_hist, const unsigned int *d_hcount, int kmax, GqDpDev *d_g, hipStream_t s);

void launch_minmax(const QuantBuffers &qb, const Tile *d_tiles, int ntiles, size_t px, NodeDev *d_nodes, hipStream_t s, bool from_end = false,
                   const RoundDyn *dyn = nullptr, const double *px_src = nullptr, const RoundLists *lists = nullptr);
void launch_hist(const QuantBuffers &qb, bool gq, const Tile *d_tiles, int ntiles, size_t px, NodeDev *d_nodes,
                 double *d_hist, unsigned long long *d_hsize, unsigned int *d_hcount, hipStream_t s, bool from_end = false,
                 bool fixed_point = false, const RoundDyn *dyn = nullptr, const double *px_src = nullptr);
void launch_cut(bool weighted, NodeDev *d_nodes, const int *d_round_nodes, int nround, const double *d_hist,
                const unsigned long long *d_hsize, const unsigned int *d_hcount, unsigned char *d_lut, hipStream_t s,
                const RoundDyn *dyn = nullptr, const double *nr_src = nullptr);
void launch_partition(const QuantBuffers &qb, const Tile *d_ptiles, int nptiles, size_t px, const int *d_round_nodes,
                      const int *d_node_tile0, int nround, NodeDev *d_nodes, const unsigned char *d_lut,
                      unsigned int *d_tilecnt, unsigned long long *d_tileoff, bool fuse_cov, hipStream_t s,
                      bool invariant = false, bool from_end = false, const RoundDyn *dyn = nullptr, const double *px_src = nullptr,
                      bool gated = false);
void launch_cov_children(const QuantBuffers &qb, const Tile *d_tiles, int ntiles, size_t px, NodeDev *d_nodes, hipStream_t s, bool from_end = false,
                         bool gated = false);
void launch_cov_nodes(const QuantBuffers &qb, const double *planar_override, const Tile *d_tiles, int ntiles, size_t px,
                      NodeDev *d_nodes, hipStream_t s, bool from_end = false);

extern std::atomic<int> g_debug_fault;
size_t hist_slot_doubles();

}
```

### patolette_amd/csrc/quant.hip

```cpp
#include "quant.h"

#include <atomic>

#include <type_traits>

namespace pamd {

template <typename T>
__device__ __forceinline__ T block_scan_incl(T v, T *smem) {
    const int lane = threadIdx.x & 63, wid = threadIdx.x >> 6, nw = blockDim.x >> 6;
#pragma unroll
    for (int o = 1; o < 64; o <<= 1) {
        T t = __shfl_up(v, o, 64);
        if (lane >= o) v += t;
    }
    __syncthreads();
    if (lane == 63) smem[wid] = v;
    __syncthreads();
    if (wid == 0) {
        T s = lane < nw ? smem[lane] : T(0);
#pragma unroll
        for (int o = 1; o < 16; o <<= 1) {
            T t = __shfl_up(s, o, 64);
            if (lane >= o) s += t;
        }
        if (lane < nw) smem[lane] = s;
    }
    __syncthreads();
    if (wid > 0) v += smem[wid - 1];
    return v;
}
template <typename T, int N>
__device__ __forceinline__ void block_scan_incl_vec(T (&v)[N], T *smem) {
    const int lane = threadIdx.x & 63, wid = threadIdx.x >> 6, nw = blockDim.x >> 6;
#pragma unroll
    for (int o = 1; o < 64; o <<= 1) {
#pragma unroll
        for (int i = 0; i < N; i++) { T t = __shfl_up(v[i], o, 64); if (lane >= o) v[i] += t; }
    }
    __syncthreads();
    if (lane == 63) {
#pragma unroll
        for (int i = 0; i < N; i++) smem[i * 16 + wid] = v[i];
    }
    __syncthreads();
    if (wid == 0 && lane < 16 * N) {
        const int i = lane >> 4, e = lane & 15;
        T s = (i < N && e < nw) ? smem[i * 16 + e] : T(0);
#pragma unroll
        for (int o = 1; o < 16; o <<= 1) { T t = __shfl_up(s, o, 16); if (e >= o) s += t; }
        if (i < N && e < nw) smem[i * 16 + e] = s;
    }
    __syncthreads();
    if (wid > 0) {
#pragma unroll
        for (int i = 0; i < N; i++) v[i] += smem[i * 16 + wid - 1];
    }
}

__global__ __launch_bounds__(256) void k_sum3(const double *__restrict__ c, size_t N, BinK k, double *out6) {
    __shared__ double sm[6 * 4];
    double a[6] = {0, 0, 0, 0, 0, 0};
    const size_t stride = (size_t)gridDim.x * blockDim.x;
    for (size_t i = (size_t)blockIdx.x * blockDim.x + threadIdx.x; i < N; i += stride) {
        bin_add(c[i], k, a[0], a[1]);
        bin_add(c[N + i], k, a[2], a[3]);
        bin_add(c[2 * N + i], k, a[4], a[5]);
    }
    block_sum<6>(a, sm);
    if (threadIdx.x == 0)
        for (int q = 0; q < 6; q++) unsafeAtomicAdd(&out6[(blockIdx.x & (kSum3Slots - 1)) * 6 + q], a[q]);
}

__device__ __forceinline__ double project(double x, double y, double z, const double a0, const double a1, const double a2) {
    return (x * a0 + y * a1) + z * a2;
}

template <bool NT, typename T>
__device__ __forceinline__ T load_last_use(const T *p) {
    if constexpr (NT) return __builtin_nontemporal_load(p); else return *p;
}

__device__ __forceinline__ int tile_node(const int *t0, int nr, int t) {
    int lo = 0, hi = nr;
    while (hi - lo > 1) { const int mid = (lo + hi) >> 1; if (t0[mid] <= t) lo = mid; else hi = mid; }
    return lo;
}
template <bool LISTS>
__global__ __launch_bounds__(256) void k_minmax(QuantBuffers qb, const Tile *__restrict__ tiles, NodeDev *nodes, const int from_end,
                                                const RoundDyn *__restrict__ dyn, const RoundLists L) {
    const unsigned nt = dyn ? (unsigned)dyn->ntA : gridDim.x;
    if (blockIdx.x >= nt) return;
    const unsigned tix = from_end ? nt - 1u - blockIdx.x : blockIdx.x;
    Tile t;
    if constexpr (LISTS) {
        const int nr = dyn->nr, ntP = dyn->ntP;
        {
            const int r = tile_node(L.tA0, nr, (int)tix);
            const int id = L.round_ids[r];
            const unsigned long long o = (unsigned long long)((int)tix - L.tA0[r]) * kTileA, n = nodes[id].n;
            t = Tile{nodes[id].begin + o, (unsigned)(n - o < (unsigned long long)kTileA ? n - o : kTileA), (unsigned)id};
            if (threadIdx.x == 0) L.tilesA[tix] = t;
        }
        for (int tp = (int)blockIdx.x + (int)threadIdx.x * (int)nt; tp < ntP; tp += (int)nt * 256) {
            const int r = tile_node(L.tP0, nr, tp);
            const int id = L.round_ids[r];
            const unsigned long long o = (unsigned long long)(tp - L.tP0[r]) * kTileP, n = nodes[id].n;
            L.tilesP[tp] = Tile{nodes[id].begin + o, (unsigned)(n - o < (unsigned long long)kTileP ? n - o : kTileP), (unsigned)id};
        }
        const size_t nh = L.lqs * (size_t)nr, nb = (size_t)nr * kBuckets;
        for (size_t i = (size_t)blockIdx.x * 256 + threadIdx.x; i < nh; i += (size_t)nt * 256) L.hist[i] = 0.0;
        for (size_t i = (size_t)blockIdx.x * 256 + threadIdx.x; i < nb; i += (size_t)nt * 256) { L.hsize[i] = 0ULL; L.hcount[i] = 0u; }
    } else {
        t = tiles[tix];
    }
    NodeDev &nd = nodes[t.node];
    const double a0 = nd.axis[0], a1 = nd.axis[1], a2 = nd.axis[2];
    const double *px = qb.buf[nd.buf], *py = px + qb.N, *pz = py + qb.N;
    double mn = INFINITY, mx = -INFINITY;
    unsigned i = threadIdx.x;
    for (; i + 3 * 256 < t.count; i += 4 * 256) {
        const size_t p = t.start + i;
        double x[4], y[4], z[4];
#pragma unroll
        for (int u = 0; u < 4; u++) { x[u] = px[p + u * 256]; y[u] = py[p + u * 256]; z[u] = pz[p + u * 256]; }
#pragma unroll
        for (int u = 0; u < 4; u++) {
            double d = project(x[u], y[u], z[u], a0, a1, a2);
            mn = fmin(mn, d); mx = fmax(mx, d);
        }
    }
    for (; i < t.count; i += 256) {
        size_t p = t.start + i;
        double d = project(px[p], py[p], pz[p], a0, a1, a2);
        mn = fmin(mn, d); mx = fmax(mx, d);
    }
#pragma unroll
    for (int o = 32; o > 0; o >>= 1) { mn = fmin(mn, __shfl_down(mn, o, 64)); mx = fmax(mx, __shfl_down(mx, o, 64)); }
    __shared__ double smn[4], smx[4];
    if ((threadIdx.x & 63) == 0) { smn[threadIdx.x >> 6] = mn; smx[threadIdx.x >> 6] = mx; }
    __syncthreads();
    if (threadIdx.x == 0) {
        for (int w = 1; w < 4; w++) { mn = fmin(mn, smn[w]); mx = fmax(mx, smx[w]); }
        if (mn <= mx) {
            atomicMin(&nd.minkey[blockIdx.x & (kSlots - 1)], f64_key(mn));
            atomicMax(&nd.maxkey[blockIdx.x & (kSlots - 1)], f64_key(mx));
        }
    }
}

constexpr int kHistCombineMin = 12;
template <bool W, bool GQ>
__global__ __launch_bounds__(512) void k_hist(QuantBuffers qb, const Tile *__restrict__ tiles, int ntiles, NodeDev *nodes,
                                              double *hist, unsigned long long *hsize, unsigned int *hcount, const int from_end,
                                              const RoundDyn *__restrict__ dyn) {
    constexpr int NQ = GQ ? (W ? 14 : 10) : (W ? 4 : 3);
    int nblk = (int)gridDim.x;
    if (dyn) {
        ntiles = dyn->ntA;
        nblk = min(ntiles, nblk);
        if ((int)blockIdx.x >= nblk) return;
    }
    constexpr int NQS = GQ ? kNQ_GQ : kNQ_LQ;
    extern __shared__ double lds[];
    double *h = lds;
    unsigned long long *siz = (unsigned long long *)(h + NQ * 2 * kBuckets);
    unsigned int *cnt = (unsigned int *)(siz + kBuckets);
    for (int i = threadIdx.x; i < NQ * 2 * kBuckets; i += blockDim.x) h[i] = 0.0;
    for (int i = threadIdx.x; i < kBuckets; i += blockDim.x) { cnt[i] = 0u; siz[i] = 0ULL; }
    __syncthreads();

    const int per = (ntiles + nblk - 1) / nblk;
    const int bid = from_end ? nblk - 1 - (int)blockIdx.x : (int)blockIdx.x;
    const int tfirst = bid * per, tlast = min(ntiles, tfirst + per);
    for (int ti = tfirst; ti < tlast; ti++) {
        const Tile t = tiles[ti];
        NodeDev &nd = nodes[t.node];
        const double a0 = nd.axis[0], a1 = nd.axis[1], a2 = nd.axis[2];
        double mn, mx;
        node_minmax(nd, mn, mx);
        const bool degenerate = (mx - mn < kDelta);
        const double sc = 1 / (mx - mn);
        const BinK klin = nd.klin, kquad = nd.kquad;
        const double *px = qb.buf[nd.buf], *py = px + qb.N, *pz = py + qb.N, *pw = pz + qb.N;
        const unsigned long long gslot0 = nd.gslot0;
        if (threadIdx.x == 0) nd.degenerate = degenerate ? 1 : 0;

        auto one = [&](const size_t p, const double x, const double y, const double z, const double w) {
            unsigned b;
            if (degenerate) {
                b = (unsigned)((p - nd.begin + gslot0) % kBuckets);
            } else {
                double ratio = (project(x, y, z, a0, a1, a2) - mn) * sc;
                unsigned long long bq = (unsigned long long)((double)kBuckets * ratio);
                b = bq < (unsigned long long)(kBuckets - 1) ? (unsigned)bq : (unsigned)(kBuckets - 1);
            }
            qb.bkt[p] = (unsigned short)b;
            double pv[2 * NQ];
#define HPART(q, val, K) bin_split((val), (K), pv[2 * (q)], pv[2 * (q) + 1])
            if constexpr (!GQ) {
                HPART(0, x * w, klin); HPART(1, y * w, klin); HPART(2, z * w, klin);
                if constexpr (W) HPART(3, w, klin);
            } else {
                HPART(0, x, klin); HPART(1, y, klin); HPART(2, z, klin);
                HPART(3, (x * x + y * y) + z * z, kquad);
                HPART(4, x * x, kquad); HPART(5, x * y, kquad); HPART(6, y * y, kquad);
                HPART(7, x * z, kquad); HPART(8, y * z, kquad); HPART(9, z * z, kquad);
                if constexpr (W) { HPART(10, x * w, klin); HPART(11, y * w, klin); HPART(12, z * w, klin); HPART(13, w, klin); }
            }
#undef HPART
            unsigned long long wi = 0ULL;
            if constexpr (W && !GQ) wi = (unsigned long long)w;
            bool direct = true;
            if (__ballot(true) == ~0ULL) {
                unsigned long long left = ~0ULL;
#pragma unroll 1
                for (int g = 0; g < 3 && left != 0ULL; g++) {
                    const int first = __builtin_ctzll(left);
                    const unsigned b0 = (unsigned)__builtin_amdgcn_readlane((int)b, first);
                    const bool mine = direct && b == b0;
                    const unsigned long long m = __ballot(mine);
                    if (__popcll(m) < kHistCombineMin) break;
#pragma unroll
                    for (int k2 = 0; k2 < 2 * NQ; k2++) {
                        const double sum = wave_sum_dpp63(mine ? pv[k2] : 0.0);
                        if ((threadIdx.x & 63) == 63) unsafeAtomicAdd(&h[k2 * kBuckets + b0], sum);
                    }
                    if constexpr (W && !GQ) {
                        unsigned long long sw2 = mine ? wi : 0ULL;
// ... 114 lines not shown
#undef HPART
            unsigned long long wi = 0ULL;
            if constexpr (W && !GQ) wi = (unsigned long long)w;
            bool direct = true;
            if (__ballot(true) == ~0ULL) {
                unsigned long long left = ~0ULL;
#pragma unroll 1
                for (int g = 0; g < 3 && left != 0ULL; g++) {
                    const int first = __builtin_ctzll(left);
                    const unsigned b0 = (unsigned)__builtin_amdgcn_readlane((int)b, first);
                    const bool mine = direct && b == b0;
                    const unsigned long long m = __ballot(mine);
                    if (__popcll(m) < kHistCombineMin) break;
#pragma unroll
                    for (int k2 = 0; k2 < NQ; k2++) {
                        const double vq = (pv[k2] + pm[k2]) - pm[k2];
                        const double sum = wave_sum_dpp63(mine ? vq : 0.0);
                        if ((threadIdx.x & 63) == 63) atomicAdd(&h[k2 * kBuckets + b0], (unsigned long long)fix_quant(sum, pm[k2]));
                    }
                    if constexpr (W && !GQ) {
                        unsigned long long sw2 = mine ? wi : 0ULL;
#pragma unroll
                        for (int o = 32; o > 0; o >>= 1) sw2 += __shfl_down(sw2, o, 64);
                        if ((threadIdx.x & 63) == 0) atomicAdd(&siz[b0], sw2);
                    }
                    if ((threadIdx.x & 63) == 0) atomicAdd(&cnt[b0], (unsigned)__popcll(m));
                    if (mine) direct = false;
                    left &= ~m;
                }
            }
            if (direct) {
                atomicAdd(&cnt[b], 1u);
#pragma unroll
                for (int k2 = 0; k2 < NQ; k2++) atomicAdd(&h[k2 * kBuckets + b], (unsigned long long)fix_quant(pv[k2], pm[k2]));
                if constexpr (W && !GQ) atomicAdd(&siz[b], wi);
            }
        };
        unsigned i = threadIdx.x;
        for (; i + 512 < t.count; i += 1024) {
            const size_t p0 = t.start + i, p1 = p0 + 512;
            const double x0 = px[p0], y0 = py[p0], z0 = pz[p0], x1 = px[p1], y1 = py[p1], z1 = pz[p1];
            double w0 = 1.0, w1 = 1.0;
            if constexpr (W) { w0 = pw[p0]; w1 = pw[p1]; }
            one(p0, x0, y0, z0, w0);
            one(p1, x1, y1, z1, w1);
        }
        for (; i < t.count; i += 512) {
            const size_t p = t.start + i;
            double w = 1.0;
            if constexpr (W) w = pw[p];
            one(p, px[p], py[p], pz[p], w);
        }
        since_flush++;
        const bool flush = (ti + 1 == tlast) || tiles[ti + 1].node != t.node || since_flush >= 16;
        if (!flush) continue;
        since_flush = 0;
        __syncthreads();
        const size_t slot = (size_t)nd.slot;
        double *gh = hist + slot * (size_t)(NQS * 2 * kBuckets);
        for (int i2 = threadIdx.x; i2 < NQ * kBuckets; i2 += blockDim.x) {
            const long long S = (long long)h[i2];
            if (S != 0) {
                const int q = i2 / kBuckets, bb = i2 % kBuckets;
                const bool quad = GQ && q >= 3 && q <= 9;
                const FixK &f = quad ? fquad : flin;
                const long long Sh = (S + (1LL << (f.s - 1))) >> f.s, Sl = S - (Sh << f.s);
                if (Sh != 0) unsafeAtomicAdd(&gh[(q * 2 + 0) * kBuckets + bb], (double)Sh * f.ghi);
                if (Sl != 0) unsafeAtomicAdd(&gh[(q * 2 + 1) * kBuckets + bb], (double)Sl * f.glo);
                h[i2] = 0ULL;
            }
        }
        for (int b = threadIdx.x; b < kBuckets; b += blockDim.x) {
            unsigned c = cnt[b];
            if (c) { atomicAdd(&hcount[slot * kBuckets + b], c); cnt[b] = 0u; }
            if constexpr (W && !GQ) { const unsigned long long s2 = siz[b]; if (s2) { atomicAdd(&hsize[slot * kBuckets + b], s2); siz[b] = 0ULL; } }
        }
        __syncthreads();
    }
}

template <bool W>
__global__ __launch_bounds__(512) void k_cut(NodeDev *nodes, const int *__restrict__ round_nodes, const double *__restrict__ hist,
                                             const unsigned long long *__restrict__ hsize, const unsigned int *__restrict__ hcount,
                                             unsigned char *lut, const int fault, const RoundDyn *__restrict__ dyn) {
    if (dyn && (int)blockIdx.x >= dyn->nr) return;
    __shared__ double sd[4 * 16];
    __shared__ unsigned long long su[2 * 16];
    __shared__ double best_v[8];
    __shared__ int best_i[8];
    __shared__ double tot[8];
    __shared__ unsigned long long tots[2];
    __shared__ int s_split;
    const int b = threadIdx.x;
    NodeDev &nd = nodes[round_nodes[blockIdx.x]];
    const size_t slot = (size_t)nd.slot;
    const double *gh = hist + slot * (size_t)(kNQ_LQ * 2 * kBuckets);
    constexpr int NQ = W ? 4 : 3;
    double p[NQ][2];
    {
        double v0[NQ], v1[NQ];
#pragma unroll
        for (int q = 0; q < NQ; q++) { v0[q] = gh[(q * 2 + 0) * kBuckets + b]; v1[q] = gh[(q * 2 + 1) * kBuckets + b]; }
        block_scan_incl_vec<double, NQ>(v0, sd);
        block_scan_incl_vec<double, NQ>(v1, sd);
#pragma unroll
        for (int q = 0; q < NQ; q++) { p[q][0] = v0[q]; p[q][1] = v1[q]; }
    }
    unsigned long long cs[2] = {(unsigned long long)hcount[slot * kBuckets + b], W ? hsize[slot * kBuckets + b] : 0ULL};
    block_scan_incl_vec<unsigned long long, 2>(cs, su);
    const unsigned long long cnt = cs[0], siz = W ? cs[1] : cs[0];
    __syncthreads();
    if (b == kBuckets - 1) {
#pragma unroll
        for (int q = 0; q < NQ; q++) { tot[q * 2] = p[q][0]; tot[q * 2 + 1] = p[q][1]; }
        tots[0] = cnt; tots[1] = siz;
    }
    __syncthreads();
    double obj = 0;
    {
        const double sl = (double)siz, sr = (double)tots[1] - sl;
#pragma unroll
        for (int j = 0; j < 3; j++) {
            double csl = p[j][0] + p[j][1];
            double csr = (tot[j * 2] + tot[j * 2 + 1]) - csl;
            double v = 0;
            if (sl != 0) v += (csl * csl) / sl;
            if (sr != 0) v += (csr * csr) / sr;
            obj += v;
        }
    }
    double bv = obj; int bi = b;
#pragma unroll
    for (int o = 32; o > 0; o >>= 1) {
        double ov = __shfl_down(bv, o, 64); int oi = __shfl_down(bi, o, 64);
        if (ov > bv || (ov == bv && (fault == 3 ? oi > bi : oi < bi))) { bv = ov; bi = oi; }
    }
    if ((b & 63) == 0) { best_v[b >> 6] = bv; best_i[b >> 6] = bi; }
    __syncthreads();
    if (b == 0) {
        for (int w = 1; w < 8; w++)
            if (best_v[w] > bv || (best_v[w] == bv && (fault == 3 ? best_i[w] > bi : best_i[w] < bi))) { bv = best_v[w]; bi = best_i[w]; }
        if (fault == 1) {
            unsigned long long upto = 0;
            for (int i = 0; i <= bi; i++) upto += hcount[slot * kBuckets + i];
            int b2 = bi + 1;
            while (b2 < kBuckets - 1 && hcount[slot * kBuckets + b2] == 0u) b2++;
            if (b2 < kBuckets - 1 && upto + hcount[slot * kBuckets + b2] < tots[0]) bi = b2;
        }
        s_split = bi;
    }
    __syncthreads();
    const int split = s_split;
    lut[slot * kBuckets + b] = b > split ? 1 : 0;
    if (b == split) {
        nd.split = split;
        const unsigned long long nL = cnt, nR = tots[0] - cnt;
        nd.cbegin[0] = nd.begin; nd.cbegin[1] = nd.begin + nL; nd.cbegin[2] = nd.begin + nd.n;
        for (int side = 0; side < 2; side++) {
            NodeDev &ch = nodes[nd.child0 + side];
            ch.begin = side == 0 ? nd.begin : nd.begin + nL;
            ch.n = side == 0 ? nL : nR;
            ch.gn = ch.n;
            ch.buf = 1 - nd.buf;
            ch.slot = -1; ch.child0 = -1; ch.nchild = 0;
            ch.klin = nd.klin; ch.kquad = nd.kquad;
            ch.psplit = split | (nd.degenerate ? 0x10000 : 0);
            double s0[NQ], s1[NQ];
#pragma unroll
            for (int q = 0; q < NQ; q++) {
                s0[q] = side == 0 ? p[q][0] : tot[q * 2] - p[q][0];
                s1[q] = side == 0 ? p[q][1] : tot[q * 2 + 1] - p[q][1];
            }
            double sw = W ? (s0[NQ - 1] + s1[NQ - 1]) : (double)ch.n;
            ch.sw = sw;
            const double inv = 1 / sw;
            for (int j = 0; j < 3; j++) ch.mean[j] = (s0[j] + s1[j]) * inv;
            ch.axis[0] = ch.axis[1] = ch.axis[2] = 0;
        }
    }
    for (int i = b; i < 2 * kNodeResetElems; i += kBuckets)
        node_reset_element(nodes[nd.child0 + i / kNodeResetElems], i % kNodeResetElems);
}

__global__ __launch_bounds__(256) void k_count(QuantBuffers qb, const Tile *__restrict__ tiles, const NodeDev *__restrict__ nodes,
                                               const unsigned char *__restrict__ lut, unsigned int *tilecnt, const int from_end,
                                               const RoundDyn *__restrict__ dyn) {
    __shared__ unsigned int c[kMaxChildren];
    __shared__ unsigned char sl[kBuckets];
    const unsigned nt = dyn ? (unsigned)dyn->ntP : gridDim.x;
    if (blockIdx.x >= nt) return;
    const unsigned tix = from_end ? nt - 1u - blockIdx.x : blockIdx.x;
    const Tile t = tiles[tix];
    const NodeDev &nd = nodes[t.node];
    const unsigned char *l = lut + (size_t)nd.slot * kBuckets;
    if (threadIdx.x < kMaxChildren) c[threadIdx.x] = 0;
    const int nch = nd.nchild;
    typedef unsigned short us8 __attribute__((ext_vector_type(8), aligned(2)));
    const int split = nd.split;
    if (nch == 2 && split >= 0) {
        const unsigned i0 = threadIdx.x * 8u;
        unsigned right = 0;
        if (i0 + 8u <= t.count) {
            const us8 v = *reinterpret_cast<const us8 *>(qb.bkt + t.start + i0);
#pragma unroll
            for (int j = 0; j < 8; j++) right += (int)v[j] > split ? 1u : 0u;
        } else {
            for (unsigned i = i0; i < t.count && i < i0 + 8u; i++) right += (int)qb.bkt[t.start + i] > split ? 1u : 0u;
        }
        __syncthreads();
        right = wave_sum_u32(right);
        if ((threadIdx.x & 63) == 0 && right) atomicAdd(&c[1], right);
        __syncthreads();
        if (threadIdx.x == 0) c[0] = t.count - c[1];
        __syncthreads();
    } else if (nch == 2) {
        for (int b = threadIdx.x; b < kBuckets; b += blockDim.x) sl[b] = l[b];
        __syncthreads();
        const unsigned i0 = threadIdx.x * 8u;
        unsigned right = 0;
        if (i0 + 8u <= t.count) {
            const us8 v = *reinterpret_cast<const us8 *>(qb.bkt + t.start + i0);
#pragma unroll
            for (int j = 0; j < 8; j++) right += sl[v[j]];
        } else {
            for (unsigned i = i0; i < t.count && i < i0 + 8u; i++) right += sl[qb.bkt[t.start + i]];
        }
        right = wave_sum_u32(right);
        if ((threadIdx.x & 63) == 0 && right) atomicAdd(&c[1], right);
        __syncthreads();
        if (threadIdx.x == 0) c[0] = t.count - c[1];
        __syncthreads();
    } else {
        __syncthreads();
        for (unsigned i = threadIdx.x; i < ((t.count + 255u) & ~255u); i += blockDim.x) {
            int child = i < t.count ? (int)l[qb.bkt[t.start + i]] : 255;
            for (int k = 0; k < nch; k++) {
                unsigned long long m = __ballot(child == k);
                if ((threadIdx.x & 63) == 0 && m) atomicAdd(&c[k], (unsigned)__popcll(m));
            }
        }
        __syncthreads();
    }
    if (threadIdx.x < kMaxChildren) tilecnt[(size_t)tix * kMaxChildren + threadIdx.x] = c[threadIdx.x];
}
__global__ __launch_bounds__(1024) void k_scan(const int *__restrict__ round_nodes, const int *__restrict__ node_tile0, NodeDev *nodes,
                                              const unsigned int *__restrict__ tilecnt, unsigned long long *tileoff,
                                              const RoundDyn *__restrict__ dyn) {
    if (dyn && (int)blockIdx.x >= dyn->nr) return;
    __shared__ unsigned long long su[16];
// ... 41 lines not shown
#pragma unroll
            for (int q = 0; q < 8; q++) v[q] = g + q < b ? tilecnt[(size_t)(g + q) * kMaxChildren + k] : 0u;
#pragma unroll
            for (int q = 0; q < 8; q++) sum += v[q];
        }
        const unsigned long long inc = block_scan_incl<unsigned long long>(sum, su);
        if (threadIdx.x == blockDim.x - 1) total = inc;
        unsigned long long run = base + inc - sum;
        for (int g = a; g < b; g += 8) {
            unsigned v[8];
#pragma unroll
            for (int q = 0; q < 8; q++) v[q] = g + q < b ? tilecnt[(size_t)(g + q) * kMaxChildren + k] : 0u;
#pragma unroll
            for (int q = 0; q < 8; q++) {
                if (g + q < b) tileoff[(size_t)(g + q) * kMaxChildren + k] = run;
                run += v[q];
            }
        }
        if (threadIdx.x == 0) nd.cbegin[k] = base;
        __syncthreads();
        base += total;
        __syncthreads();
    }
    if (threadIdx.x == 0) nd.cbegin[nch] = base;
}

template <bool W>
__global__ __launch_bounds__(256, 5) void k_scatter(QuantBuffers qb, const Tile *__restrict__ tiles, int ntiles, NodeDev *nodes,
                                                    const unsigned char *__restrict__ lut, const unsigned long long *__restrict__ tileoff,
                                                    const int from_end) {
    constexpr int R = kTileP / 256;
    __shared__ unsigned long long off[R][4][kMaxChildren];
    const int lane = threadIdx.x & 63, wid = threadIdx.x >> 6;
    const unsigned long long ltmask = (1ULL << lane) - 1ULL;
    if ((from_end & 4) && nodes[0].nchild == 2) return;
    const int per = (ntiles + (int)gridDim.x - 1) / (int)gridDim.x;
    const int bid = (from_end & 1) ? (int)gridDim.x - 1 - (int)blockIdx.x : (int)blockIdx.x;
    const int tfirst = bid * per, tlast = min(ntiles, tfirst + per);
    for (int ti = tfirst; ti < tlast; ti++) {
        const Tile t = tiles[ti];
        const NodeDev &nd = nodes[t.node];
        const unsigned char *l = lut + (size_t)nd.slot * kBuckets;
        const int nch = nd.nchild;
        unsigned cr[R];
#pragma unroll
        for (int r = 0; r < R; r++) {
            unsigned i = r * 256 + threadIdx.x;
            int ch = 255;
            if (i < t.count) ch = (int)l[qb.bkt[t.start + i]];
            unsigned rk = 0;
            for (int k = 0; k < nch; k++) {
                unsigned long long m = __ballot(ch == k);
                if (ch == k) rk = (unsigned)__popcll(m & ltmask);
                if (lane == 0) off[r][wid][k] = (unsigned long long)__popcll(m);
            }
            cr[r] = (unsigned)ch | (rk << 8);
        }
        __syncthreads();
        if ((int)threadIdx.x < nch) {
            unsigned long long run = tileoff[(size_t)ti * kMaxChildren + threadIdx.x];
            for (int r = 0; r < R; r++)
                for (int w = 0; w < 4; w++) { unsigned long long c = off[r][w][threadIdx.x]; off[r][w][threadIdx.x] = run; run += c; }
        }
        __syncthreads();
        const double *sx = qb.buf[nd.buf], *sy = sx + qb.N, *sz = sy + qb.N, *sw = sz + qb.N;
        double *dx = qb.buf[1 - nd.buf], *dy = dx + qb.N, *dz = dy + qb.N, *dw = dz + qb.N;
#pragma unroll
        for (int r = 0; r < R; r++) {
            const int ch = (int)(cr[r] & 255u);
            if (ch != 255) {
                const size_t src = t.start + r * 256 + threadIdx.x;
                const size_t dst = off[r][wid][ch] + (cr[r] >> 8);
                const double x = sx[src], y = sy[src], z = sz[src];
                double w = 1.0;
                if constexpr (W) w = sw[src];
                dx[dst] = x; dy[dst] = y; dz[dst] = z;
                if constexpr (W) dw[dst] = w;
            }
        }
        __syncthreads();
    }
}

template <bool W, bool INV, bool NT>
__global__ __launch_bounds__(256, (W || INV) ? 2 : 3) void k_scatter_bin(QuantBuffers qb, const Tile *__restrict__ tiles, int ntiles, NodeDev *nodes,
                                                                        const NodeDev *__restrict__ nodes_ro,
                                                                        const unsigned long long *__restrict__ tileoff, const int from_end,
                                                                        const RoundDyn *__restrict__ dyn) {
    constexpr int R = kTileP / 256;
    static_assert(R * 4 == 32, "one 32-lane group per child");
    __shared__ unsigned int wcnt[2][2][R * 4];
    __shared__ double sm[28 * 4];
    const int lane = threadIdx.x & 63, wid = __builtin_amdgcn_readfirstlane((int)(threadIdx.x >> 6));
    const unsigned long long ltmask = (1ULL << lane) - 1ULL;
    int nblk = (int)gridDim.x;
    if ((from_end & 2) && nodes_ro[0].nchild != 2) return;
    if (dyn) {
        ntiles = dyn->ntP;
        nblk = min(ntiles, nblk);
        if ((int)blockIdx.x >= nblk) return;
    }
    const int per = (ntiles + nblk - 1) / nblk;
    const int bid = (from_end & 1) ? nblk - 1 - (int)blockIdx.x : (int)blockIdx.x;
    const int tfirst = bid * per, tlast = min(ntiles, tfirst + per);
    if (tfirst >= tlast) return;
    constexpr int NP = INV ? 14 : 7;
    double pl[NP], pr[NP];
#pragma unroll
    for (int i = 0; i < NP; i++) { pl[i] = 0; pr[i] = 0; }

    auto fetch_buckets = [&](const Tile &tt, const int ti, unsigned (&b)[R], unsigned long long &toff) {
        const unsigned last = tt.count - 1u;
#pragma unroll
        for (int r = 0; r < R; r++) b[r] = load_last_use<NT>(qb.bkt + tt.start + min((unsigned)(r * 256) + threadIdx.x, last));
        toff = tileoff[(size_t)ti * kMaxChildren + (lane >> 5)];
    };
    auto classify = [&](const Tile &tt, const unsigned (&b)[R], const int split, const int par, unsigned (&cr)[R]) {
#pragma unroll
        for (int r = 0; r < R; r++) {
            const bool valid = (unsigned)(r * 256) + threadIdx.x < tt.count;
            const bool right = (int)b[r] > split;
            const unsigned long long mR = __ballot(valid && right), mL = __ballot(valid && !right);
            const unsigned rk = (unsigned)__popcll((right ? mR : mL) & ltmask);
            cr[r] = (valid ? (right ? 1u : 0u) : 2u) | (rk << 8);
            if (lane == 0) { wcnt[par][0][r * 4 + wid] = (unsigned)__popcll(mL); wcnt[par][1][r * 4 + wid] = (unsigned)__popcll(mR); }
        }
    };
    auto lane64 = [](const unsigned long long v, const int l) {
        return ((unsigned long long)(unsigned)__builtin_amdgcn_readlane((int)(unsigned)(v >> 32), l) << 32) |
               (unsigned)__builtin_amdgcn_readlane((int)(unsigned)v, l);
    };
    Tile t = tiles[tfirst];
    unsigned cr[R];
    unsigned long long baseL, baseR;
    {
        unsigned b0[R];
        unsigned long long toff;
        fetch_buckets(t, tfirst, b0, toff);
        classify(t, b0, nodes_ro[t.node].split, 0, cr);
        baseL = lane64(toff, 0); baseR = lane64(toff, 32);
    }
    for (int ti = tfirst; ti < tlast; ti++) {
        const int par = (ti - tfirst) & 1;
        const NodeDev &nd = nodes_ro[t.node];
        const int child0 = nd.child0;
        const double *sx = qb.buf[nd.buf], *sy = sx + qb.N, *sz = sy + qb.N, *sw = sz + qb.N;
        double *dx = qb.buf[1 - nd.buf], *dy = dx + qb.N, *dz = dy + qb.N, *dw = dz + qb.N;
        double x[R], y[R], z[R], w[R];
        {
            const unsigned last = t.count - 1u;
#pragma unroll
            for (int r = 0; r < R; r++) {
                const size_t src = t.start + min((unsigned)(r * 256) + threadIdx.x, last);
                x[r] = load_last_use<NT>(sx + src); y[r] = load_last_use<NT>(sy + src); z[r] = load_last_use<NT>(sz + src);
                w[r] = 1.0;
                if constexpr (W) w[r] = load_last_use<NT>(sw + src);
            }
        }
        const bool more = ti + 1 < tlast;
        const int tnx = more ? ti + 1 : ti;
        const Tile tn = tiles[tnx];
        unsigned bkn[R];
        unsigned long long toffn;
        fetch_buckets(tn, tnx, bkn, toffn);
        __syncthreads();
        const unsigned c = wcnt[par][lane >> 5][lane & 31];
        const unsigned incl = wave_scan_incl_u32(c);
        const unsigned tot0 = (unsigned)__builtin_amdgcn_readlane((int)incl, 31);
        const unsigned excl = incl - c - (lane >= 32 ? tot0 : 0u);
        const NodeDev &c0 = nodes_ro[child0], &c1 = nodes_ro[child0 + 1];
        const double m0L = c0.mean[0], m1L = c0.mean[1], m2L = c0.mean[2], m0R = c1.mean[0], m1R = c1.mean[1], m2R = c1.mean[2];
        BinK kinv{0.0, 0.0};
        if constexpr (INV) kinv = nd.kquad;
        const size_t slack = (size_t)(W ? 4 : 3) * qb.N + (size_t)lane;
#pragma unroll
        for (int r = 0; r < R; r++) {
            const unsigned eL = (unsigned)__builtin_amdgcn_readlane((int)excl, r * 4 + wid);
            const unsigned eR = (unsigned)__builtin_amdgcn_readlane((int)excl, 32 + r * 4 + wid);
            const unsigned ch = cr[r] & 255u;
            const bool right = ch == 1u, none = ch == 2u;
            const size_t dst = (right ? baseR + eR : baseL + eL) + (cr[r] >> 8);
            dx[none ? slack : dst] = x[r]; dy[none ? slack - qb.N : dst] = y[r]; dz[none ? slack - 2 * qb.N : dst] = z[r];
            if constexpr (W) dw[none ? slack - 3 * qb.N : dst] = w[r];
            const double rf = right ? 1.0 : 0.0, lf = ch == 0u ? 1.0 : 0.0;
            const double ex = x[r] - (right ? m0R : m0L), ey = y[r] - (right ? m1R : m1L), ez = z[r] - (right ? m2R : m2L);
            const double wx = w[r] * ex, wy = w[r] * ey, wz = w[r] * ez;
            const double q[7] = {wx * ex, wy * ex, wz * ex, wy * ey, wz * ey, wz * ez, ((ex * ex + ey * ey) + ez * ez) * w[r]};
            if constexpr (INV) {
#pragma unroll
                for (int i = 0; i < 7; i++) {
                    double v0, v1;
                    bin_split(q[i], kinv, v0, v1);
                    pl[2 * i] = __builtin_fma(v0, lf, pl[2 * i]); pl[2 * i + 1] = __builtin_fma(v1, lf, pl[2 * i + 1]);
                    pr[2 * i] = __builtin_fma(v0, rf, pr[2 * i]); pr[2 * i + 1] = __builtin_fma(v1, rf, pr[2 * i + 1]);
                }
            } else {
#pragma unroll
                for (int i = 0; i < 7; i++) { pl[i] = __builtin_fma(q[i], lf, pl[i]); pr[i] = __builtin_fma(q[i], rf, pr[i]); }
            }
        }
        const bool flush = !more || tn.node != t.node;
        if (flush) {
            const BinK kq = nd.kquad;
            double a[28];
            if constexpr (INV) {
#pragma unroll
                for (int i = 0; i < 14; i++) { a[i] = pl[i]; a[14 + i] = pr[i]; pl[i] = 0; pr[i] = 0; }
            } else {
#pragma unroll
                for (int i = 0; i < 7; i++) {
                    bin_split(pl[i], kq, a[2 * i], a[2 * i + 1]);
                    bin_split(pr[i], kq, a[14 + 2 * i], a[14 + 2 * i + 1]);
                    pl[i] = 0; pr[i] = 0;
                }
            }
            block_sum<28>(a, sm);
            if (threadIdx.x == 0) {
                for (int side = 0; side < 2; side++) {
                    NodeDev &chn = nodes[child0 + side];
                    for (int i = 0; i < 7; i++) {
                        if (a[14 * side + 2 * i] != 0.0) unsafeAtomicAdd(&chn.acc[blockIdx.x & (kSlots - 1)][i][0], a[14 * side + 2 * i]);
                        if (a[14 * side + 2 * i + 1] != 0.0) unsafeAtomicAdd(&chn.acc[blockIdx.x & (kSlots - 1)][i][1], a[14 * side + 2 * i + 1]);
                    }
                }
            }
        }
        if (more) {
            classify(tn, bkn, nodes_ro[tn.node].split, par ^ 1, cr);
            baseL = lane64(toffn, 0); baseR = lane64(toffn, 32);
        }
        t = tn;
    }
}

template <bool W>
__device__ __forceinline__ void cov_accumulate(const double *px, const double *py, const double *pz, const double *pw,
                                               size_t lo, size_t hi, const double m0, const double m1, const double m2,
                                               const BinK kq, double (&a)[14]) {
    for (size_t p = lo + threadIdx.x; p < hi; p += blockDim.x) {
        double dx = px[p] - m0, dy = py[p] - m1, dz = pz[p] - m2;
        double w = 1.0;
        if constexpr (W) w = pw[p];
        double wx = w * dx, wy = w * dy, wz = w * dz;
        bin_add(wx * dx, kq, a[0], a[1]);
        bin_add(wy * dx, kq, a[2], a[3]);
        bin_add(wz * dx, kq, a[4], a[5]);
        bin_add(wy * dy, kq, a[6], a[7]);
        bin_add(wz * dy, kq, a[8], a[9]);
        bin_add(wz * dz, kq, a[10], a[11]);
        bin_add(((dx * dx + dy * dy) + dz * dz) * w, kq, a[12], a[13]);
    }
}

template <bool W>
__global__ __launch_bounds__(256) void k_cov_children(QuantBuffers qb, const Tile *__restrict__ tiles, NodeDev *nodes, const int from_end) {
    __shared__ double sm[14 * 4];
    if ((from_end & 4) && nodes[0].nchild == 2) return;
    const Tile t = tiles[(from_end & 1) ? gridDim.x - 1u - blockIdx.x : blockIdx.x];
    const NodeDev &nd = nodes[t.node];
    const double *px = qb.buf[1 - nd.buf], *py = px + qb.N, *pz = py + qb.N, *pw = pz + qb.N;
    const size_t t_lo = t.start, t_hi = t.start + t.count;
    for (int k = 0; k < nd.nchild; k++) {
        size_t lo = nd.cbegin[k] > t_lo ? nd.cbegin[k] : t_lo;
        size_t hi = nd.cbegin[k + 1] < t_hi ? nd.cbegin[k + 1] : t_hi;
        if (lo >= hi) continue;
        NodeDev &ch = nodes[nd.child0 + k];
        double a[14];
#pragma unroll
        for (int i = 0; i < 14; i++) a[i] = 0;
        cov_accumulate<W>(px, py, pz, pw, lo, hi, ch.mean[0], ch.mean[1], ch.mean[2], nd.kquad, a);
        block_sum<14>(a, sm);
        if (threadIdx.x == 0)
            for (int q = 0; q < 7; q++) { unsafeAtomicAdd(&ch.acc[blockIdx.x & (kSlots - 1)][q][0], a[2 * q]); unsafeAtomicAdd(&ch.acc[blockIdx.x & (kSlots - 1)][q][1], a[2 * q + 1]); }
    }
}

template <bool W>
__global__ __launch_bounds__(256) void k_cov_nodes(QuantBuffers qb, const double *planar, const Tile *__restrict__ tiles, NodeDev *nodes,
                                                   const int from_end) {
    __shared__ double sm[14 * 4];
    const Tile t = tiles[from_end ? gridDim.x - 1u - blockIdx.x : blockIdx.x];
    NodeDev &nd = nodes[t.node];
    const double *px = planar ? planar : qb.buf[nd.buf], *py = px + qb.N, *pz = py + qb.N, *pw = pz + qb.N;
    double a[14];
#pragma unroll
    for (int i = 0; i < 14; i++) a[i] = 0;
    cov_accumulate<W>(px, py, pz, pw, t.start, t.start + t.count, nd.mean[0], nd.mean[1], nd.mean[2], nd.kquad, a);
    block_sum<14>(a, sm);
    if (threadIdx.x == 0)
        for (int q = 0; q < 7; q++) { unsafeAtomicAdd(&nd.acc[blockIdx.x & (kSlots - 1)][q][0], a[2 * q]); unsafeAtomicAdd(&nd.acc[blockIdx.x & (kSlots - 1)][q][1], a[2 * q + 1]); }
}

size_t hist_slot_doubles() { return (size_t)kNQ_GQ * 2 * kBuckets; }

void launch_sum3(const double *planar, size_t N, BinK k, double *d_out6, hipStream_t s) {
    HIP_CHECK(hipMemsetAsync(d_out6, 0, kSum3Slots * 6 * sizeof(double), s));
    size_t g = ceil_div(N, 256 * 16);
    if (g > 2048) g = 2048;
    if (g < 1) g = 1;
    KTIME("k_sum3", s, 24.0 * N);
    hipLaunchKernelGGL(k_sum3, (int)g, 256, 0, s, planar, N, k, d_out6);
    HIP_CHECK(hipGetLastError());
}

void launch_minmax(const QuantBuffers &qb, const Tile *d_tiles, int ntiles, size_t px, NodeDev *d_nodes, hipStream_t s, bool from_end,
                   const RoundDyn *dyn, const double *px_src, const RoundLists *lists) {
    if (!ntiles) return;
    KTIME_DYN("k_minmax", s, 24.0, px, px_src);
    if (dyn && lists) hipLaunchKernelGGL(k_minmax<true>, ntiles, 256, 0, s, qb, d_tiles, d_nodes, from_end ? 1 : 0, dyn, *lists);
    else hipLaunchKernelGGL(k_minmax<false>, ntiles, 256, 0, s, qb, d_tiles, d_nodes, from_end ? 1 : 0, dyn, RoundLists{});
    HIP_CHECK(hipGetLastError());
}

template <bool W>
static void launch_hist_fix(const QuantBuffers &qb, const Tile *d_tiles, int ntiles, size_t px, NodeDev *d_nodes, double *d_hist,
                            unsigned long long *d_hsize, unsigned int *d_hcount, hipStream_t s, bool from_end) {
    constexpr int NQ = W ? 14 : 10;
    const size_t lds = (size_t)NQ * kBuckets * sizeof(unsigned long long) + kBuckets * (sizeof(unsigned int) + sizeof(unsigned long long));
    static PerDeviceOnce attr_set;
    attr_set.once([&] { HIP_CHECK(hipFuncSetAttribute((const void *)k_hist_fix<W, true>, hipFuncAttributeMaxDynamicSharedMemorySize, (int)lds)); });
    KTIME("k_hist_gq", s, (W ? 34.0 : 26.0) * px);
    const int g = std::min(ntiles, 256 * (W ? 2 : 3));
    hipLaunchKernelGGL((k_hist_fix<W, true>), g, 512, lds, s, qb, d_tiles, ntiles, d_nodes, d_hist, d_hsize, d_hcount, from_end ? 1 : 0);
    HIP_CHECK(hipGetLastError());
}

template <bool W, bool GQ>
static void launch_hist_t(const QuantBuffers &qb, const Tile *d_tiles, int ntiles, size_t px, NodeDev *d_nodes, double *d_hist,
                          unsigned long long *d_hsize, unsigned int *d_hcount, hipStream_t s, bool from_end,
                          const RoundDyn *dyn = nullptr, const double *px_src = nullptr) {
    constexpr int NQ = GQ ? (W ? 14 : 10) : (W ? 4 : 3);
    size_t lds = (size_t)NQ * 2 * kBuckets * sizeof(double) + kBuckets * (sizeof(unsigned int) + sizeof(unsigned long long));
    static PerDeviceOnce attr_set;
    attr_set.once([&] { HIP_CHECK(hipFuncSetAttribute((const void *)k_hist<W, GQ>, hipFuncAttributeMaxDynamicSharedMemorySize, (int)lds)); });
    KTIME_DYN(GQ ? "k_hist_gq" : "k_hist_lq", s, (W ? 34.0 : 26.0), px, px_src);
    const int g = std::min(ntiles, 256 * (GQ ? 1 : 4));
    hipLaunchKernelGGL((k_hist<W, GQ>), g, 512, lds, s, qb, d_tiles, ntiles, d_nodes, d_hist, d_hsize, d_hcount, from_end ? 1 : 0, dyn);
    HIP_CHECK(hipGetLastError());
}

__global__ __launch_bounds__(512) void k_gq_prefix(const double *__restrict__ hist, const unsigned int *__restrict__ hcount, GqDpDev *g) {
    __shared__ double sh[4][kBuckets + 1];
    __shared__ unsigned long long sc[kBuckets + 1];
    const int b = threadIdx.x;
#pragma unroll
    for (int hq = 0; hq < 4; hq++)
        sh[hq][b + 1] = hist[(size_t)(hq * 2 + 0) * kBuckets + b] + hist[(size_t)(hq * 2 + 1) * kBuckets + b];
    sc[b + 1] = hcount[b];
    if (b < 4) sh[b][0] = 0;
    if (b == 4) sc[0] = 0;
    __syncthreads();
    if (b == 0) { unsigned long long a = 0; for (int i = 1; i <= kBuckets; i++) { a += sc[i]; sc[i] = a; } }
    else if ((b & 63) == 0 && b <= 256) {
        double *t = sh[(b >> 6) - 1];
        double a = 0;
        for (int i = 1; i <= kBuckets; i++) { a = t[i] + a; t[i] = a; }
    }
    __syncthreads();
    for (int i = b; i <= kBuckets; i += 512) {
        g->w0[i] = sc[i];
        g->w1[0][i] = sh[0][i]; g->w1[1][i] = sh[1][i]; g->w1[2][i] = sh[2][i]; g->w2[i] = sh[3][i];
    }
}
__device__ __forceinline__ double gq_distortion(const GqDpDev *g, int a, int b) {
    if (g->w0[a] == g->w0[b]) return 0;
    const double q0 = g->w1[0][b] - g->w1[0][a], q1 = g->w1[1][b] - g->w1[1][a], q2 = g->w1[2][b] - g->w1[2][a];
    return g->w2[b] - g->w2[a] - (q0 * q0 + q1 * q1 + q2 * q2) / (double)(g->w0[b] - g->w0[a]);
}
__global__ void k_gq_init(GqDpDev *g) {
    const int i = blockIdx.x * blockDim.x + threadIdx.x;
    if (i <= kBuckets) g->E[0][i] = i >= 1 ? gq_distortion(g, 0, i) : 0.0;
}
__global__ __launch_bounds__(256) void k_gq_dp(GqDpDev *g, int k) {
    const int n = (int)blockIdx.x;
    const double *Ep = g->E[k & 1];
    double *En = g->E[(k & 1) ^ 1];
    if (n < k + 1) { if (threadIdx.x == 0) En[n] = Ep[n]; return; }
    double best = INFINITY; int bt = -1;
    for (int t = n - 2 - (int)threadIdx.x; t >= k - 1; t -= (int)blockDim.x) {
        const double v = Ep[t] + gq_distortion(g, t, n);
        if (v < best) { best = v; bt = t; }
    }
    __shared__ double sv[256];
    __shared__ int st[256];
    sv[threadIdx.x] = best; st[threadIdx.x] = bt;
    __syncthreads();
    for (int o = 128; o > 0; o >>= 1) {
        if ((int)threadIdx.x < o) {
            const double v2 = sv[threadIdx.x + o]; const int t2 = st[threadIdx.x + o];
            const double v1 = sv[threadIdx.x]; const int t1 = st[threadIdx.x];
            if (t2 >= 0 && (t1 < 0 || v2 < v1 || (v2 == v1 && t2 > t1))) { sv[threadIdx.x] = v2; st[threadIdx.x] = t2; }
        }
        __syncthreads();
    }
    if (threadIdx.x == 0) {
        double e = Ep[n - 1]; int cut = n - 1;
        if (st[0] >= 0 && sv[0] < e) { e = sv[0]; cut = st[0]; }
        En[n] = e;
        g->cut[k][n] = cut;
    }
}

void launch_gq_dp(const double *d_hist, const unsigned int *d_hcount, int kmax, GqDpDev *d_g, hipStream_t s) {
    KTIME("k_gq_dp", s, (double)kmax * 513 * 513 * 8);
    hipLaunchKernelGGL(k_gq_prefix, 1, 512, 0, s, d_hist, d_hcount, d_g);
    hipLaunchKernelGGL(k_gq_init, 3, 256, 0, s, d_g);
    for (int k = 2; k <= kmax; k++) hipLaunchKernelGGL(k_gq_dp, kBuckets + 1, 256, 0, s, d_g, k);
    HIP_CHECK(hipGetLastError());
}

void launch_hist(const QuantBuffers &qb, bool gq, const Tile *d_tiles, int ntiles, size_t px, NodeDev *d_nodes,
                 double *d_hist, unsigned long long *d_hsize, unsigned int *d_hcount, hipStream_t s, bool from_end, bool fixed_point,
                 const RoundDyn *dyn, const double *px_src) {
    if (!ntiles) return;
    if (gq && fixed_point) {
        if (qb.weighted) launch_hist_fix<true>(qb, d_tiles, ntiles, px, d_nodes, d_hist, d_hsize, d_hcount, s, from_end);
        else launch_hist_fix<false>(qb, d_tiles, ntiles, px, d_nodes, d_hist, d_hsize, d_hcount, s, from_end);
        return;
    }
    if (qb.weighted) { if (gq) launch_hist_t<true, true>(qb, d_tiles, ntiles, px, d_nodes, d_hist, d_hsize, d_hcount, s, from_end);
                       else launch_hist_t<true, false>(qb, d_tiles, ntiles, px, d_nodes, d_hist, d_hsize, d_hcount, s, from_end, dyn, px_src); }
    else { if (gq) launch_hist_t<false, true>(qb, d_tiles, ntiles, px, d_nodes, d_hist, d_hsize, d_hcount, s, from_end);
           else launch_hist_t<false, false>(qb, d_tiles, ntiles, px, d_nodes, d_hist, d_hsize, d_hcount, s, from_end, dyn, px_src); }
}

std::atomic<int> g_debug_fault{0};
void launch_cut(bool weighted, NodeDev *d_nodes, const int *d_round_nodes, int nround, const double *d_hist,
                const unsigned long long *d_hsize, const unsigned int *d_hcount, unsigned char *d_lut, hipStream_t s, const RoundDyn *dyn, const double *nr_src) {
    if (!nround) return;
    KTIME_DYN("k_cut", s, (double)kNQ_LQ * 2 * kBuckets * 8, nround, nr_src);
    const int fault = g_debug_fault.load(std::memory_order_relaxed);
    if (weighted) hipLaunchKernelGGL(k_cut<true>, nround, 512, 0, s, d_nodes, d_round_nodes, d_hist, d_hsize, d_hcount, d_lut, fault, dyn);
    else hipLaunchKernelGGL(k_cut<false>, nround, 512, 0, s, d_nodes, d_round_nodes, d_hist, d_hsize, d_hcount, d_lut, fault, dyn);
    HIP_CHECK(hipGetLastError());
}

void launch_partition(const QuantBuffers &qb, const Tile *d_ptiles, int nptiles, size_t px, const int *d_round_nodes,
                      const int *d_node_tile0, int nround, NodeDev *d_nodes, const unsigned char *d_lut,
                      unsigned int *d_tilecnt, unsigned long long *d_tileoff, bool fuse_cov, hipStream_t s, bool invariant, bool from_end,
                      const RoundDyn *dyn, const double *px_src, bool gated) {
    const int fe = (from_end ? 1 : 0) | (gated ? 2 : 0);
    if (!nround) return;
    if (nptiles) { KTIME_DYN("k_count", s, 2.0, px, px_src); hipLaunchKernelGGL(k_count, nptiles, 256, 0, s, qb, d_ptiles, d_nodes, d_lut, d_tilecnt, fe & 1, dyn); }
    { KTIME_DYN("k_scan", s, 12.0 * kMaxChildren / (double)kTileP, dyn ? px : (size_t)nptiles * kTileP, px_src);
      hipLaunchKernelGGL(k_scan, nround, 1024, 0, s, d_round_nodes, d_node_tile0, d_nodes, d_tilecnt, d_tileoff, dyn); }
    if (nptiles) {
        KTIME_DYN(fuse_cov ? "k_scatter_cov" : "k_scatter", s, (qb.weighted ? 66.0 : 50.0), px, px_src);
        if (fuse_cov) {
            const int gb = std::min(nptiles, 256 * ((invariant || qb.weighted) ? 2 : 3));
            const bool nt = 2 * (size_t)(qb.weighted ? 4 : 3) * qb.N * sizeof(double) > kInfinityCacheBytes;
            auto go = [&](auto kernel) {
                hipLaunchKernelGGL(kernel, gb, 256, 0, s, qb, d_ptiles, nptiles, d_nodes, (const NodeDev *)d_nodes, d_tileoff, fe, dyn);
            };
            if (invariant) {
                if (qb.weighted) { if (nt) go(k_scatter_bin<true, true, true>); else go(k_scatter_bin<true, true, false>); }
                else { if (nt) go(k_scatter_bin<false, true, true>); else go(k_scatter_bin<false, true, false>); }
            } else if (qb.weighted) { if (nt) go(k_scatter_bin<true, false, true>); else go(k_scatter_bin<true, false, false>); }
            else { if (nt) go(k_scatter_bin<false, false, true>); else go(k_scatter_bin<false, false, false>); }
            if (gated) {
                HIP_CHECK(hipGetLastError());
                const int fg = (from_end ? 1 : 0) | 4;
                if (qb.weighted) hipLaunchKernelGGL((k_scatter<true>), nptiles, 256, 0, s, qb, d_ptiles, nptiles, d_nodes, d_lut, d_tileoff, fg);
                else hipLaunchKernelGGL((k_scatter<false>), nptiles, 256, 0, s, qb, d_ptiles, nptiles, d_nodes, d_lut, d_tileoff, fg);
            }
        } else {
            if (qb.weighted) hipLaunchKernelGGL((k_scatter<true>), nptiles, 256, 0, s, qb, d_ptiles, nptiles, d_nodes, d_lut, d_tileoff, fe);
            else hipLaunchKernelGGL((k_scatter<false>), nptiles, 256, 0, s, qb, d_ptiles, nptiles, d_nodes, d_lut, d_tileoff, fe);
        }
    }
    HIP_CHECK(hipGetLastError());
}

void launch_cov_children(const QuantBuffers &qb, const Tile *d_tiles, int ntiles, size_t px, NodeDev *d_nodes, hipStream_t s, bool from_end, bool gated) {
    if (!ntiles) return;
    KTIME("k_cov", s, (qb.weighted ? 32.0 : 24.0) * px);
    const int fe = (from_end ? 1 : 0) | (gated ? 4 : 0);
    if (qb.weighted) hipLaunchKernelGGL(k_cov_children<true>, ntiles, 256, 0, s, qb, d_tiles, d_nodes, fe);
    else hipLaunchKernelGGL(k_cov_children<false>, ntiles, 256, 0, s, qb, d_tiles, d_nodes, fe);
    HIP_CHECK(hipGetLastError());
}

void launch_cov_nodes(const QuantBuffers &qb, const double *planar_override, const Tile *d_tiles, int ntiles, size_t px,
                      NodeDev *d_nodes, hipStream_t s, bool from_end) {
    if (!ntiles) return;
    KTIME("k_cov", s, ((qb.weighted && !planar_override) ? 32.0 : 24.0) * px);
    if (qb.weighted && !planar_override) hipLaunchKernelGGL(k_cov_nodes<true>, ntiles, 256, 0, s, qb, planar_override, d_tiles, d_nodes, from_end ? 1 : 0);
    else hipLaunchKernelGGL(k_cov_nodes<false>, ntiles, 256, 0, s, qb, planar_override, d_tiles, d_nodes, from_end ? 1 : 0);
    HIP_CHECK(hipGetLastError());
}

}
```

Baseline: 3168.

## Use packed 10-bit per-axis keys for minmax in local quantiser rounds

Adds a per-pixel 30-bit key buffer, written during the fused scatter, that quantises each color into a per-node frame. Later split rounds can bound node min/max (and projections) from the 4-byte keys instead of reading three f64 planes, with a fallback path when the key bound is ambiguous. It is enabled automatically for large images that exceed the infinity cache. The scan direction for keyed rounds is fixed to match the buffer the keys were written to. In exchange it adds key-buffer memory, extra writes in scatter, and more complex cut and frame logic.

```diff
diff --git a/include/patolette_amd.h b/include/patolette_amd.h
--- a/include/patolette_amd.h
+++ b/include/patolette_amd.h
@@ -180,6 +180,7 @@
 int patolette_amd_set_kmeans_update(int mode);
 
 int patolette_amd_set_split_loop(int mode);
+int patolette_amd_set_minmax_keys(int mode);
 int patolette_amd_set_global_quantiser(int on_device);
 
 int patolette_amd_set_subsample_cache(int on);
@@ -207,6 +208,7 @@
 int patolette_amd_kmeans_refine(const double *colors, const double *weights, size_t n,
                                 double *centers_io, size_t k, int niter, size_t max_samples);
 int patolette_amd_debug_km_route(void);
+int patolette_amd_debug_minmax_route(unsigned long long out[4]);
 
 int patolette_amd_nn_map(const double *colors, size_t n, const double *palette, size_t k, size_t *map);
 int patolette_amd_debug_nn_route(int route);
diff --git a/patolette_amd/_native.py b/patolette_amd/_native.py
--- a/patolette_amd/_native.py
+++ b/patolette_amd/_native.py
@@ -137,6 +137,7 @@
     "patolette_amd_kmeans_refine": (C.c_int, [dp, dp, C.c_size_t, dp, C.c_size_t, C.c_int, C.c_size_t]),
     "patolette_amd_nn_map": (C.c_int, [dp, C.c_size_t, dp, C.c_size_t, zp]),
     "patolette_amd_debug_km_route": (C.c_int, []),
+    "patolette_amd_debug_minmax_route": (C.c_int, [C.POINTER(C.c_ulonglong)]),
     "patolette_amd_debug_nn_route": (C.c_int, [C.c_int]),
     "patolette_amd_debug_nn_map_elem": (C.c_int, [dp, C.c_size_t, dp, C.c_size_t, C.c_int, C.c_int, C.c_void_p]),
     "patolette_amd_set_global_quantiser": (C.c_int, [C.c_int]),
@@ -156,6 +157,7 @@
     "patolette_amd_debug_workspace": (C.c_int, [C.c_int]),
     "patolette_amd_debug_late_growths": (C.c_ulonglong, []),
     "patolette_amd_set_split_loop": (C.c_int, [C.c_int]),
+    "patolette_amd_set_minmax_keys": (C.c_int, [C.c_int]),
     "patolette_amd_profile_enable": (None, [C.c_int]),
     "patolette_amd_profile_only": (None, [C.c_char_p]),
     "patolette_amd_profile_sample": (None, [C.c_int]),
diff --git a/patolette_amd/csrc/minmax_keys.h b/patolette_amd/csrc/minmax_keys.h
--- /dev/null
+++ b/patolette_amd/csrc/minmax_keys.h
@@ -0,0 +1,67 @@
+#pragma once
+
+#include <cmath>
+
+#if defined(__HIPCC__)
+#define PAMD_KEYS_HD __host__ __device__ __forceinline__
+#else
+#define PAMD_KEYS_HD inline
+#endif
+
+namespace pamd {
+
+constexpr int kKeyBits = 10;
+constexpr int kKeyCells = 1 << kKeyBits;
+constexpr unsigned kKeyMask = kKeyCells - 1;
+constexpr double kKeyFrameMin = 0x1p-100, kKeyFrameMax = 0x1p100;
+
+struct KeyFrame { double lo[3], w[3], inv[3]; };
+
+PAMD_KEYS_HD bool key_frame_make(const double lo[3], const double hi[3], KeyFrame &f) {
+    bool ok = true;
+    for (int i = 0; i < 3; i++) {
+        const double e = hi[i] - lo[i];
+        f.lo[i] = lo[i];
+        if (e == 0.0) { f.w[i] = 0.0; f.inv[i] = 0.0; }
+        else { ok = ok && e >= kKeyFrameMin && e <= kKeyFrameMax; f.w[i] = e * (1.0 / kKeyCells); f.inv[i] = (double)kKeyCells / e; }
+        ok = ok && std::fabs(lo[i]) <= kKeyFrameMax && std::fabs(hi[i]) <= kKeyFrameMax;
+    }
+    return ok;
+}
+
+PAMD_KEYS_HD unsigned key_cell(const double c, const double lo, const double inv) {
+    double t = (c - lo) * inv;
+    t = t > 0.0 ? t : 0.0;
+    t = t < (double)(kKeyCells - 1) ? t : (double)(kKeyCells - 1);
+    return (unsigned)(int)t;
+}
+PAMD_KEYS_HD unsigned key_pack(const KeyFrame &f, const double x, const double y, const double z) {
+    return key_cell(x, f.lo[0], f.inv[0]) | (key_cell(y, f.lo[1], f.inv[1]) << kKeyBits) | (key_cell(z, f.lo[2], f.inv[2]) << (2 * kKeyBits));
+}
+
+PAMD_KEYS_HD void key_child_box(const KeyFrame &f, const unsigned qmin[3], const unsigned qmax[3], double lo[3], double hi[3]) {
+    for (int i = 0; i < 3; i++) {
+        if (f.w[i] == 0.0) { lo[i] = hi[i] = f.lo[i]; continue; }
+        lo[i] = f.lo[i] + ((double)qmin[i] - 1.0) * f.w[i];
+        hi[i] = f.lo[i] + ((double)qmax[i] + 2.0) * f.w[i];
+    }
+}
+
+struct KeyProj { double b, g[3], H; };
+PAMD_KEYS_HD KeyProj key_proj_make(const KeyFrame &f, const double a0, const double a1, const double a2) {
+    const double a[3] = {a0, a1, a2};
+    KeyProj p;
+    p.b = 0.0; p.H = 0x1p-1000;
+    for (int i = 0; i < 3; i++) {
+        p.g[i] = a[i] * f.w[i];
+        p.b += a[i] * (f.lo[i] + 0.5 * f.w[i]);
+        p.H += std::fabs(a[i]) * (0.5 * f.w[i] * (1.0 + 0x1p-20) + 0x1p-40 * (std::fabs(f.lo[i]) + (double)kKeyCells * f.w[i]));
+    }
+    return p;
+}
+PAMD_KEYS_HD double key_centre(const KeyProj &p, const unsigned key) {
+    return p.b + ((double)(key & kKeyMask) * p.g[0] + (double)((key >> kKeyBits) & kKeyMask) * p.g[1] +
+                  (double)((key >> (2 * kKeyBits)) & kKeyMask) * p.g[2]);
+}
+
+}
diff --git a/patolette_amd/csrc/pipeline.hip b/patolette_amd/csrc/pipeline.hip
--- a/patolette_amd/csrc/pipeline.hip
+++ b/patolette_amd/csrc/pipeline.hip
@@ -96,7 +96,8 @@
 void KernelTimer::reset() { collect(); names.clear(); total_ms.clear(); total_bytes.clear(); launches.clear(); }
 
 __global__ __launch_bounds__(256) void k_gq_prepare(Tile *tA, int ntA, Tile *tP, int ntP, unsigned long long N, int *round_nodes, int *node_tile0,
-                                                    double *hist, unsigned long long nhist, unsigned long long *hsize, unsigned int *hcount) {
+                                                    double *hist, unsigned long long nhist, unsigned long long *hsize, unsigned int *hcount,
+                                                    MinmaxRoute *route) {
     const unsigned long long stride = (unsigned long long)gridDim.x * blockDim.x, t0 = (unsigned long long)blockIdx.x * blockDim.x + threadIdx.x;
     for (unsigned long long i = t0; i < (unsigned long long)ntA; i += stride) {
         const unsigned long long o = i * (unsigned long long)kTileA;
@@ -109,6 +110,7 @@
     for (unsigned long long i = t0; i < nhist; i += stride) hist[i] = 0.0;
     for (unsigned long long i = t0; i < (unsigned long long)kBuckets; i += stride) { hsize[i] = 0ULL; hcount[i] = 0u; }
     if (t0 == 0) { round_nodes[0] = 0; node_tile0[0] = 0; node_tile0[1] = ntP; }
+    if (t0 < (unsigned long long)kMinmaxRouteSlots) route[t0] = MinmaxRoute{0ULL, 0ULL, 0ULL, 0ULL};
 }
 
 __global__ void k_put_nodes(NodeDev *table, const NodeIn *stage, const int *ids, int n) {
@@ -851,6 +853,8 @@
     size_t prep_N = 0, prep_planes = 0;
     DevBuf<double> src, wsrc, cvt, bufA, bufB, aux;
     DevBuf<unsigned short> bkt;
+    DevBuf<unsigned> keyA, keyB;
+    DevBuf<MinmaxRoute> mmroute;
     DevBuf<NodeDev> nodes;
     DevBuf<NodeIn> stage_in;
     DevBuf<NodeOut> stage_out;
@@ -1143,10 +1147,11 @@
 }
 
 struct QuantSizes {
-    size_t bufA, bufB, bkt, tilesA, tilesP, tilecnt, tileoff, hist, hsize, hcount, lut;
+    size_t bufA, bufB, keyA, keyB, bkt, tilesA, tilesP, tilecnt, tileoff, hist, hsize, hcount, lut;
     QuantSizes(size_t pixels, size_t planes, size_t nodes) {
         const size_t slack = nodes > 1 ? nodes : 0;
         bufA = bufB = planes * pixels + 64;
+        keyA = keyB = pixels + 64;
         bkt = pixels;
         tilesA = ceil_div(pixels, (size_t)kTileA) + slack; tilesP = ceil_div(pixels, (size_t)kTileP) + slack;
         tilecnt = tileoff = tilesP * kMaxChildren;
@@ -1156,6 +1161,7 @@
 };
 static void reserve_quant_tables(Engine &E, const QuantSizes &z, const char *file = __builtin_FILE(), int line = __builtin_LINE()) {
     E.bufA.reserve(z.bufA, file, line); E.bufB.reserve(z.bufB, file, line); E.bkt.reserve(z.bkt, file, line);
+    E.keyA.reserve(z.keyA, file, line); E.keyB.reserve(z.keyB, file, line); E.mmroute.reserve(kMinmaxRouteSlots, file, line);
     E.tilesA.reserve(z.tilesA, file, line); E.tilesP.reserve(z.tilesP, file, line);
     E.tilecnt.reserve(z.tilecnt, file, line); E.tileoff.reserve(z.tileoff, file, line);
     E.hist.reserve(z.hist, file, line); E.hsize.reserve(z.hsize, file, line); E.hcount.reserve(z.hcount, file, line); E.lut.reserve(z.lut, file, line);
@@ -1171,7 +1177,7 @@
     E.round_nodes.reserve(1); E.node_tile0.reserve(2);
     const size_t hs = hist_slot_doubles();
     hipLaunchKernelGGL(k_gq_prepare, 64, 256, 0, s, E.tilesA.p, ntA, E.tilesP.p, ntP, (unsigned long long)N, E.round_nodes.p, E.node_tile0.p,
-                       E.hist.p, (unsigned long long)hs, E.hsize.p, E.hcount.p);
+                       E.hist.p, (unsigned long long)hs, E.hsize.p, E.hcount.p, E.mmroute.p);
     HIP_CHECK(hipGetLastError());
     E.prep_N = N; E.prep_planes = planes;
 }
@@ -1181,6 +1187,15 @@
 std::atomic<int> g_lq_device{getenv("PAMD_LQ_DEVICE") ? atoi(getenv("PAMD_LQ_DEVICE")) : 2};
 std::atomic<int> g_gq_device{getenv("PAMD_GQ_DEVICE") ? atoi(getenv("PAMD_GQ_DEVICE")) : 1};
 constexpr size_t kLqDeviceAutoPixels = (size_t)40 << 20;
+std::atomic<int> g_minmax_keys{2};
+constexpr size_t kMinmaxKeysAutoBytes = 2 * kInfinityCacheBytes;
+static bool minmax_keys_on(const Engine &E, size_t N) {
+    const int mode = g_minmax_keys.load(std::memory_order_relaxed);
+    return (mode == 1 || (mode == 2 && 3 * N * sizeof(double) >= kMinmaxKeysAutoBytes)) && !E.shard;
+}
+static KeyRoot make_keyroot(const Bounds &b, const QuantBuffers &q) {
+    return KeyRoot{{b.lo[0], b.lo[1], b.lo[2]}, {b.hi[0], b.hi[1], b.hi[2]}, q.key[0] ? 1 : 0};
+}
 
 static bool lq_device_eligible(const Engine &E, size_t N, size_t K, bool verbose, bool allow_device) {
     const int lq_mode = g_lq_device.load(std::memory_order_relaxed);
@@ -1215,6 +1230,7 @@
     LqHead *head = E.h_lqhead.p;
     for (int r = 0; r < kLqMaxRounds; r++) { head->round_px[r] = 0.0; head->round_nr[r] = 0.0; }
     const RoundDyn *dyn = &c->dyn;
+    const KeyRoot kroot = make_keyroot(bnd, qlq);
     const int *d_round = c->round_ids, *d_tP0 = c->tP0;
     int call = 0;
     const GqOut *gq = kbase < 0 ? (const GqOut *)E.gqout.p : nullptr;
@@ -1235,19 +1251,21 @@
     auto round = [&]() {
         if (enq >= kLqMaxRounds) throw HipError("patolette_amd: split loop exceeded its round limit");
         const double *px_src = &head->round_px[enq], *nr_src = &head->round_nr[enq];
-        const bool rev = enq % 2 == 1;
+        const bool keyed = kroot.on != 0 && enq >= 1;
+        const bool rev = keyed ? true : enq % 2 == 1;
         static const bool setup_kernel = getenv("PAMD_LQ_SETUP_KERNEL") && atoi(getenv("PAMD_LQ_SETUP_KERNEL")) != 0;
         if (setup_kernel) {
             hipLaunchKernelGGL(k_round_setup_dyn, 1024, 256, 0, s, E.nodes.p, (const LqCtl *)c, E.tilesA.p, E.tilesP.p, E.hist.p, E.hsize.p, E.hcount.p, lqs);
             HIP_CHECK(hipGetLastError());
-            launch_minmax(qlq, E.tilesA.p, ntA_ub, 0, E.nodes.p, s, rev, dyn, px_src);
+            launch_minmax(qlq, E.tilesA.p, ntA_ub, 0, E.nodes.p, s, rev, E.mmroute.p, dyn, px_src);
         } else {
             const RoundLists rl{c->round_ids, c->tA0, c->tP0, E.tilesA.p, E.tilesP.p, E.hist.p, lqs, E.hsize.p, E.hcount.p};
-            launch_minmax(qlq, E.tilesA.p, ntA_ub, 0, E.nodes.p, s, rev, dyn, px_src, &rl);
+            launch_minmax(qlq, E.tilesA.p, ntA_ub, 0, E.nodes.p, s, rev, E.mmroute.p, dyn, px_src, &rl);
         }
-        launch_hist(qlq, false, E.tilesA.p, ntA_ub, 0, E.nodes.p, E.hist.p, E.hsize.p, E.hcount.p, s, !rev, false, dyn, px_src);
-        launch_cut(weighted, E.nodes.p, d_round, kLqRoundCap, E.hist.p, E.hsize.p, E.hcount.p, E.lut.p, s, dyn, nr_src);
-        launch_partition(qlq, E.tilesP.p, ntP_ub, 0, d_round, d_tP0, kLqRoundCap, E.nodes.p, E.lut.p, E.tilecnt.p, E.tileoff.p, true, s, inv_sums, rev, dyn, px_src);
+        launch_hist(qlq, false, E.tilesA.p, ntA_ub, 0, E.nodes.p, E.hist.p, E.hsize.p, E.hcount.p, s, keyed ? rev : !rev, false, dyn, px_src);
+        launch_cut(weighted, E.nodes.p, d_round, kLqRoundCap, E.hist.p, E.hsize.p, E.hcount.p, E.lut.p, s, dyn, nr_src, kroot);
+        launch_partition(qlq, E.tilesP.p, ntP_ub, 0, d_round, d_tP0, kLqRoundCap, E.nodes.p, E.lut.p, E.tilecnt.p, E.tileoff.p, true, s, inv_sums, keyed ? !rev : rev, dyn, px_src,
+                         false, kroot.on != 0);
         enq++;
         control();
     };
@@ -1423,7 +1441,7 @@
         d.slot = 0;
         put_nodes(E, {0}, {d});
     }
-    launch_minmax(C.qroot, E.tilesA.p, C.ntA0, C.N, E.nodes.p, s, C.mom_path);
+    launch_minmax(C.qroot, E.tilesA.p, C.ntA0, C.N, E.nodes.p, s, C.mom_path, E.mmroute.p);
     if (C.sh) shard_exchange_keys(E, shard_upload_ids(E, {0}), 1);
     launch_hist(C.qroot, true, E.tilesA.p, C.ntA0, C.N, E.nodes.p, E.hist.p, E.hsize.p, E.hcount.p, s, !C.mom_path, C.Nt >= ((size_t)1 << 18));
     if (C.sh) { comm_sum_dev(E, E.hist.p, C.hs, 0); comm_sum_dev(E, E.hcount.p, kBuckets, 2); }
@@ -1696,7 +1714,9 @@
     std::memcpy(E.h_packet.p + o_tP, tPg.data(), tPg.size() * sizeof(int));
     laps.lap(laps.packet);
     HIP_CHECK(hipMemcpyAsync(E.packet.p, E.h_packet.p, pk_bytes, hipMemcpyHostToDevice, s));
-    const bool rev = E.stats.lq_rounds % 2 == 1;
+    const KeyRoot kroot = make_keyroot(C.bnd, C.qlq);
+    const bool keyed = kroot.on != 0 && E.stats.lq_rounds >= 1;
+    const bool rev = keyed ? true : E.stats.lq_rounds % 2 == 1;
     const int *d_ids = (const int *)(E.packet.p + o_ids), *d_cids = (const int *)(E.packet.p + o_cids);
     const int *d_tA0 = (const int *)(E.packet.p + o_tA), *d_tP0 = (const int *)(E.packet.p + o_tP);
     RoundSetup rs{(const NodeIn *)(E.packet.p + o_recs), d_ids, d_tA0, d_tP0, nr, ntA, ntP,
@@ -1706,16 +1726,17 @@
         hipLaunchKernelGGL(k_round_setup, (unsigned)std::min<size_t>((work + 255) / 256, 2048), 256, 0, s, E.nodes.p, rs);
         HIP_CHECK(hipGetLastError());
     }
-    launch_minmax(C.qlq, E.tilesA.p, ntA, rpx, E.nodes.p, s, rev);
+    launch_minmax(C.qlq, E.tilesA.p, ntA, rpx, E.nodes.p, s, rev, E.mmroute.p);
     if (C.sh) shard_exchange_keys(E, d_ids, nr);
-    launch_hist(C.qlq, false, E.tilesA.p, ntA, rpx, E.nodes.p, E.hist.p, E.hsize.p, E.hcount.p, s, !rev);
+    launch_hist(C.qlq, false, E.tilesA.p, ntA, rpx, E.nodes.p, E.hist.p, E.hsize.p, E.hcount.p, s, keyed ? rev : !rev);
     if (C.sh) {
         comm_sum_dev(E, E.hist.p, lqs * nr, 0);
         if (C.weighted) comm_sum_dev(E, E.hsize.p, (size_t)nr * kBuckets, 1);
         comm_sum_dev(E, E.hcount.p, (size_t)nr * kBuckets, 2);
     }
-    launch_cut(C.weighted, E.nodes.p, d_ids, nr, E.hist.p, E.hsize.p, E.hcount.p, E.lut.p, s);
-    launch_partition(C.qlq, E.tilesP.p, ntP, rpx, d_ids, d_tP0, nr, E.nodes.p, E.lut.p, E.tilecnt.p, E.tileoff.p, true, s, C.inv_sums, rev);
+    launch_cut(C.weighted, E.nodes.p, d_ids, nr, E.hist.p, E.hsize.p, E.hcount.p, E.lut.p, s, nullptr, nullptr, kroot);
+    launch_partition(C.qlq, E.tilesP.p, ntP, rpx, d_ids, d_tP0, nr, E.nodes.p, E.lut.p, E.tilecnt.p, E.tileoff.p, true, s, C.inv_sums, keyed ? !rev : rev, nullptr, nullptr,
+                     false, kroot.on != 0);
     if (C.sh) {
         hipLaunchKernelGGL(k_shard_children_local, (nr + 63) / 64, 64, 0, s, E.nodes.p, d_ids, nr);
         HIP_CHECK(hipGetLastError());
@@ -1782,8 +1803,10 @@
     const bool dev_eligible = lq_device_eligible(E, N, K, verbose, allow_device);
     E.nodes.reserve(std::max<size_t>(4 * K + 64, dev_eligible ? (size_t)kLqNodeCap : 0));
     const QuantSizes root(N, planes, 1);
+    const bool keys_on = minmax_keys_on(E, N);
     QuantCall C{E, N, sh ? sh->total : N, K, weighted, sh || E.invariant, verbose, dev_eligible, sh, bnd, centers, len, max_members,
-                QuantBuffers{{E.cvt.p, E.bufA.p}, E.bkt.p, N, weighted}, QuantBuffers{{E.bufB.p, E.bufA.p}, E.bkt.p, N, weighted},
+                QuantBuffers{{E.cvt.p, E.bufA.p}, E.bkt.p, N, weighted},
+                keys_on ? QuantBuffers{{E.bufB.p, E.bufA.p}, E.bkt.p, N, weighted, {E.keyB.p, E.keyA.p}} : QuantBuffers{{E.bufB.p, E.bufA.p}, E.bkt.p, N, weighted},
                 (int)root.tilesA, (int)root.tilesP, hist_slot_doubles(), now_ms()};
     C.hn.reserve(4 * K + 64);
 
@@ -3905,6 +3928,16 @@
 }
 
 int patolette_amd_debug_km_route(void) { return holder().e ? holder().e->km.route : 0; }
+int patolette_amd_debug_minmax_route(unsigned long long out[4]) {
+    for (int i = 0; i < 4; i++) out[i] = 0;
+    Engine *e = holder().e;
+    if (!e || !e->mmroute.p) return -1;
+    MinmaxRoute r[kMinmaxRouteSlots];
+    if (hipSetDevice(e->device) != hipSuccess || hipStreamSynchronize(e->stream) != hipSuccess ||
+        hipMemcpy(r, e->mmroute.p, sizeof r, hipMemcpyDeviceToHost) != hipSuccess) return -1;
+    for (int i = 0; i < kMinmaxRouteSlots; i++) { out[0] += r[i].nodes; out[1] += r[i].key_tiles; out[2] += r[i].fallback_tiles; out[3] += r[i].candidates; }
+    return 0;
+}
 
 int patolette_amd_debug_nn_route(int route) { return nn_debug_route(route); }
 
@@ -3955,6 +3988,7 @@
 int patolette_amd_debug_fault(int which) { return g_debug_fault.exchange(which); }
 int patolette_amd_debug_workspace(int flags) { return g_debug_ws.exchange(flags & (kWsPoison | kWsCount | kWsLog)); }
 unsigned long long patolette_amd_debug_late_growths(void) { return g_late_growths.load(); }
+int patolette_amd_set_minmax_keys(int mode) { return g_minmax_keys.exchange(mode < 0 || mode > 2 ? 2 : mode); }
 int patolette_amd_set_split_loop(int mode) { return g_lq_device.exchange(mode < 0 || mode > 2 ? 2 : mode); }
 int patolette_amd_set_global_quantiser(int on_device) { return g_gq_device.exchange(on_device ? 1 : 0); }
 void patolette_amd_dither_config(int segments, int warm) { dither_config(segments, warm); }
diff --git a/patolette_amd/csrc/quant.h b/patolette_amd/csrc/quant.h
--- a/patolette_amd/csrc/quant.h
+++ b/patolette_amd/csrc/quant.h
@@ -4,6 +4,7 @@
 
 #include "common.h"
 #include "devutil.h"
+#include "minmax_keys.h"
 
 namespace pamd {
 
@@ -49,9 +50,12 @@
     int split;
     int psplit;
     int axis_state;
+    int keys;
     double cov6[6], dist, ub;
     unsigned long long cbegin[kMaxChildren + 1];
     double acc[kSlots][7][2];
+    KeyFrame kf;
+    unsigned kqmin[kSlots][3], kqmax[kSlots][3];
 };
 
 template <> struct WsPoison<NodeDev> {
@@ -67,13 +71,17 @@
 __device__ __forceinline__ void node_reset_outputs(NodeDev &d) {
     for (int i = 0; i < kSlots; i++) { d.minkey[i] = ~0ULL; d.maxkey[i] = 0ULL; }
     for (int i = 0; i < kSlots; i++) for (int q = 0; q < 7; q++) { d.acc[i][q][0] = 0; d.acc[i][q][1] = 0; }
+    for (int i = 0; i < kSlots; i++) for (int j = 0; j < 3; j++) { d.kqmin[i][j] = ~0u; d.kqmax[i][j] = 0u; }
     d.degenerate = 0; d.split = -1; d.gslot0 = 0;
+    d.keys = 0;
 }
-constexpr int kNodeResetElems = kSlots * 14 + 2 * kSlots;
+constexpr int kNodeResetElems = kSlots * 14 + 2 * kSlots + 6 * kSlots;
 __device__ __forceinline__ void node_reset_element(NodeDev &d, int e) {
     if (e < kSlots * 14) (&d.acc[0][0][0])[e] = 0.0;
     else if (e < kSlots * 15) d.minkey[e - kSlots * 14] = ~0ULL;
-    else d.maxkey[e - kSlots * 15] = 0ULL;
+    else if (e < kSlots * 16) d.maxkey[e - kSlots * 15] = 0ULL;
+    else if (e < kSlots * 19) (&d.kqmin[0][0])[e - kSlots * 16] = ~0u;
+    else (&d.kqmax[0][0])[e - kSlots * 19] = 0u;
     if (e == 0) { d.degenerate = 0; d.split = -1; d.gslot0 = 0; }
 }
 __device__ __forceinline__ void node_minmax(const NodeDev &d, double &mn, double &mx) {
@@ -106,7 +114,12 @@
     unsigned short *bkt;
     size_t N;
     bool weighted;
+    unsigned *key[2] = {nullptr, nullptr};
 };
+
+struct KeyRoot { double lo[3], hi[3]; int on; };
+constexpr int kMinmaxRouteSlots = 16;
+struct MinmaxRoute { unsigned long long nodes, key_tiles, fallback_tiles, candidates; };
 
 constexpr int kSum3Slots = 32;
 void launch_sum3(const double *planar, size_t N, BinK k, double *d_out6, hipStream_t s);
@@ -119,19 +132,19 @@
 };
 void launch_gq_dp(const double *d_hist, const unsigned int *d_hcount, int kmax, GqDpDev *d_g, hipStream_t s);
 
-void launch_minmax(const QuantBuffers &qb, const Tile *d_tiles, int ntiles, size_t px, NodeDev *d_nodes, hipStream_t s, bool from_end = false,
-                   const RoundDyn *dyn = nullptr, const double *px_src = nullptr, const RoundLists *lists = nullptr);
+void launch_minmax(const QuantBuffers &qb, const Tile *d_tiles, int ntiles, size_t px, NodeDev *d_nodes, hipStream_t s, bool from_end,
+                   MinmaxRoute *d_route, const RoundDyn *dyn = nullptr, const double *px_src = nullptr, const RoundLists *lists = nullptr);
 void launch_hist(const QuantBuffers &qb, bool gq, const Tile *d_tiles, int ntiles, size_t px, NodeDev *d_nodes,
                  double *d_hist, unsigned long long *d_hsize, unsigned int *d_hcount, hipStream_t s, bool from_end = false,
                  bool fixed_point = false, const RoundDyn *dyn = nullptr, const double *px_src = nullptr);
 void launch_cut(bool weighted, NodeDev *d_nodes, const int *d_round_nodes, int nround, const double *d_hist,
                 const unsigned long long *d_hsize, const unsigned int *d_hcount, unsigned char *d_lut, hipStream_t s,
-                const RoundDyn *dyn = nullptr, const double *nr_src = nullptr);
+                const RoundDyn *dyn = nullptr, const double *nr_src = nullptr, const KeyRoot &kroot = KeyRoot{{0, 0, 0}, {0, 0, 0}, 0});
 void launch_partition(const QuantBuffers &qb, const Tile *d_ptiles, int nptiles, size_t px, const int *d_round_nodes,
                       const int *d_node_tile0, int nround, NodeDev *d_nodes, const unsigned char *d_lut,
                       unsigned int *d_tilecnt, unsigned long long *d_tileoff, bool fuse_cov, hipStream_t s,
                       bool invariant = false, bool from_end = false, const RoundDyn *dyn = nullptr, const double *px_src = nullptr,
-                      bool gated = false);
+                      bool gated = false, bool keys = false);
 void launch_cov_children(const QuantBuffers &qb, const Tile *d_tiles, int ntiles, size_t px, NodeDev *d_nodes, hipStream_t s, bool from_end = false,
                          bool gated = false);
 void launch_cov_nodes(const QuantBuffers &qb, const double *planar_override, const Tile *d_tiles, int ntiles, size_t px,
diff --git a/patolette_amd/csrc/quant.hip b/patolette_amd/csrc/quant.hip
--- a/patolette_amd/csrc/quant.hip
+++ b/patolette_amd/csrc/quant.hip
@@ -86,13 +86,15 @@
     while (hi - lo > 1) { const int mid = (lo + hi) >> 1; if (t0[mid] <= t) lo = mid; else hi = mid; }
     return lo;
 }
+constexpr unsigned kKeyCandShare = 16;
 template <bool LISTS>
-__global__ __launch_bounds__(256) void k_minmax(QuantBuffers qb, const Tile *__restrict__ tiles, NodeDev *nodes, const int from_end,
-                                                const RoundDyn *__restrict__ dyn, const RoundLists L) {
+__global__ __launch_bounds__(256, 4) void k_minmax_keys(QuantBuffers qb, const Tile *__restrict__ tiles, NodeDev *nodes, const int from_end,
+                                                     const RoundDyn *__restrict__ dyn, const RoundLists L, MinmaxRoute *route) {
     const unsigned nt = dyn ? (unsigned)dyn->ntA : gridDim.x;
     if (blockIdx.x >= nt) return;
     const unsigned tix = from_end ? nt - 1u - blockIdx.x : blockIdx.x;
     Tile t;
+    bool first_tile;
     if constexpr (LISTS) {
         const int nr = dyn->nr, ntP = dyn->ntP;
         {
@@ -115,29 +117,103 @@
         t = tiles[tix];
     }
     NodeDev &nd = nodes[t.node];
+    first_tile = t.start == nd.begin;
     const double a0 = nd.axis[0], a1 = nd.axis[1], a2 = nd.axis[2];
     const double *px = qb.buf[nd.buf], *py = px + qb.N, *pz = py + qb.N;
     double mn = INFINITY, mx = -INFINITY;
-    unsigned i = threadIdx.x;
-    for (; i + 3 * 256 < t.count; i += 4 * 256) {
-        const size_t p = t.start + i;
-        double x[4], y[4], z[4];
-#pragma unroll
-        for (int u = 0; u < 4; u++) { x[u] = px[p + u * 256]; y[u] = py[p + u * 256]; z[u] = pz[p + u * 256]; }
-#pragma unroll
-        for (int u = 0; u < 4; u++) {
-            double d = project(x[u], y[u], z[u], a0, a1, a2);
+    __shared__ double smn[4], smx[4];
+    const int lane = threadIdx.x & 63, wid = threadIdx.x >> 6;
+    const bool keyed = nd.keys != 0 && t.count != 0u;
+    bool whole = !keyed;
+    unsigned ncand = 0;
+    if (keyed) {
+        constexpr int U = kTileA / 256;
+        static_assert(U == 32, "one candidate bit per pixel of a lane");
+        __shared__ unsigned sq[4][6], scand[4];
+        __shared__ unsigned short clist[kTileA / kKeyCandShare];
+        const unsigned *pk = qb.key[nd.buf] + t.start;
+        const KeyProj kp = key_proj_make(nd.kf, a0, a1, a2);
+        unsigned key[U];
+        const unsigned last = t.count - 1u;
+#pragma unroll
+        for (int u = 0; u < U; u++) key[u] = pk[min((unsigned)(u * 256) + threadIdx.x, last)];
+        double cmn = INFINITY, cmx = -INFINITY;
+        unsigned q[6] = {~0u, ~0u, ~0u, 0u, 0u, 0u};
+#pragma unroll
+        for (int u = 0; u < U; u++) {
+            const double c = key_centre(kp, key[u]);
+            cmn = fmin(cmn, c); cmx = fmax(cmx, c);
+            const unsigned q0 = key[u] & kKeyMask, q1 = (key[u] >> kKeyBits) & kKeyMask, q2 = key[u] >> (2 * kKeyBits);
+            q[0] = min(q[0], q0); q[1] = min(q[1], q1); q[2] = min(q[2], q2);
+            q[3] = max(q[3], q0); q[4] = max(q[4], q1); q[5] = max(q[5], q2);
+        }
+#pragma unroll
+        for (int o = 32; o > 0; o >>= 1) {
+            cmn = fmin(cmn, __shfl_down(cmn, o, 64)); cmx = fmax(cmx, __shfl_down(cmx, o, 64));
+#pragma unroll
+            for (int j = 0; j < 3; j++) { q[j] = min(q[j], (unsigned)__shfl_down(q[j], o, 64)); q[3 + j] = max(q[3 + j], (unsigned)__shfl_down(q[3 + j], o, 64)); }
+        }
+        if (lane == 0) {
+            smn[wid] = cmn; smx[wid] = cmx;
+#pragma unroll
+            for (int j = 0; j < 6; j++) sq[wid][j] = q[j];
+        }
+        __syncthreads();
+        cmn = fmin(fmin(smn[0], smn[1]), fmin(smn[2], smn[3]));
+        cmx = fmax(fmax(smx[0], smx[1]), fmax(smx[2], smx[3]));
+        if (threadIdx.x < 6) {
+            const int j = threadIdx.x;
+            if (j < 3) atomicMin(&nd.kqmin[blockIdx.x & (kSlots - 1)][j], min(min(sq[0][j], sq[1][j]), min(sq[2][j], sq[3][j])));
+            else atomicMax(&nd.kqmax[blockIdx.x & (kSlots - 1)][j - 3], max(max(sq[0][j], sq[1][j]), max(sq[2][j], sq[3][j])));
+        }
+        const double thi = cmx - 2.0 * kp.H, tlo = cmn + 2.0 * kp.H;
+        unsigned mask = 0;
+#pragma unroll
+        for (int u = 0; u < U; u++) {
+            const bool valid = (unsigned)(u * 256) + threadIdx.x < t.count;
+            asm volatile("" : "+v"(key[u]));
+            const double c = key_centre(kp, key[u]);
+            if (valid && (!(c < thi) || !(c > tlo))) mask |= 1u << u;
+        }
+        const unsigned nc = (unsigned)__popc(mask);
+        const unsigned incl = wave_scan_incl_u32(nc);
+        if (lane == 63) scand[wid] = incl;
+        __syncthreads();
+        unsigned base = 0;
+        for (int w = 0; w < 4; w++) { if (w < wid) base += scand[w]; ncand += scand[w]; }
+        whole = ncand > t.count / kKeyCandShare;
+        if (!whole) {
+            unsigned at = base + incl - nc;
+            while (mask) { const int u = __builtin_ctz(mask); mask &= mask - 1u; clist[at++] = (unsigned short)(u * 256 + (int)threadIdx.x); }
+            __syncthreads();
+            for (unsigned j = threadIdx.x; j < ncand; j += 256) {
+                const size_t p = t.start + clist[j];
+                const double d = project(px[p], py[p], pz[p], a0, a1, a2);
+                mn = fmin(mn, d); mx = fmax(mx, d);
+            }
+        }
+    }
+    if (whole) {
+        unsigned i = threadIdx.x;
+        for (; i + 3 * 256 < t.count; i += 4 * 256) {
+            const size_t p = t.start + i;
+            double x[4], y[4], z[4];
+#pragma unroll
+            for (int u = 0; u < 4; u++) { x[u] = px[p + u * 256]; y[u] = py[p + u * 256]; z[u] = pz[p + u * 256]; }
+#pragma unroll
+            for (int u = 0; u < 4; u++) {
+                double d = project(x[u], y[u], z[u], a0, a1, a2);
+                mn = fmin(mn, d); mx = fmax(mx, d);
+            }
+        }
+        for (; i < t.count; i += 256) {
+            size_t p = t.start + i;
+            double d = project(px[p], py[p], pz[p], a0, a1, a2);
             mn = fmin(mn, d); mx = fmax(mx, d);
         }
     }
-    for (; i < t.count; i += 256) {
-        size_t p = t.start + i;
-        double d = project(px[p], py[p], pz[p], a0, a1, a2);
-        mn = fmin(mn, d); mx = fmax(mx, d);
-    }
 #pragma unroll
     for (int o = 32; o > 0; o >>= 1) { mn = fmin(mn, __shfl_down(mn, o, 64)); mx = fmax(mx, __shfl_down(mx, o, 64)); }
-    __shared__ double smn[4], smx[4];
     if ((threadIdx.x & 63) == 0) { smn[threadIdx.x >> 6] = mn; smx[threadIdx.x >> 6] = mx; }
     __syncthreads();
     if (threadIdx.x == 0) {
@@ -145,6 +221,12 @@
         if (mn <= mx) {
             atomicMin(&nd.minkey[blockIdx.x & (kSlots - 1)], f64_key(mn));
             atomicMax(&nd.maxkey[blockIdx.x & (kSlots - 1)], f64_key(mx));
+        }
+        if (keyed) {
+            MinmaxRoute &r = route[blockIdx.x & (kMinmaxRouteSlots - 1)];
+            if (first_tile) atomicAdd(&r.nodes, 1ULL);
+            if (whole) atomicAdd(&r.fallback_tiles, 1ULL); else atomicAdd(&r.candidates, (unsigned long long)ncand);
+            atomicAdd(&r.key_tiles, 1ULL);
         }
     }
 }
@@ -425,7 +507,7 @@
 template <bool W>
 __global__ __launch_bounds__(512) void k_cut(NodeDev *nodes, const int *__restrict__ round_nodes, const double *__restrict__ hist,
                                              const unsigned long long *__restrict__ hsize, const unsigned int *__restrict__ hcount,
-                                             unsigned char *lut, const int fault, const RoundDyn *__restrict__ dyn) {
+                                             unsigned char *lut, const int fault, const RoundDyn *__restrict__ dyn, const KeyRoot kroot) {
     if (dyn && (int)blockIdx.x >= dyn->nr) return;
     __shared__ double sd[4 * 16];
     __shared__ unsigned long long su[2 * 16];
@@ -434,8 +516,14 @@
     __shared__ double tot[8];
     __shared__ unsigned long long tots[2];
     __shared__ int s_split;
+    __shared__ unsigned s_kq[6];
     const int b = threadIdx.x;
     NodeDev &nd = nodes[round_nodes[blockIdx.x]];
+    if (b < 6 && kroot.on && nd.keys) {
+        unsigned v = b < 3 ? ~0u : 0u;
+        for (int k = 0; k < kSlots; k++) v = b < 3 ? min(v, nd.kqmin[k][b]) : max(v, nd.kqmax[k][b - 3]);
+        s_kq[b] = v;
+    }
     const size_t slot = (size_t)nd.slot;
     const double *gh = hist + slot * (size_t)(kNQ_LQ * 2 * kBuckets);
     constexpr int NQ = W ? 4 : 3;
@@ -499,6 +587,16 @@
         nd.split = split;
         const unsigned long long nL = cnt, nR = tots[0] - cnt;
         nd.cbegin[0] = nd.begin; nd.cbegin[1] = nd.begin + nL; nd.cbegin[2] = nd.begin + nd.n;
+        KeyFrame cf;
+        bool ckeys = kroot.on != 0;
+        if (ckeys) {
+            double lo[3] = {kroot.lo[0], kroot.lo[1], kroot.lo[2]}, hi[3] = {kroot.hi[0], kroot.hi[1], kroot.hi[2]};
+            if (nd.keys) {
+                const unsigned qa[3] = {s_kq[0], s_kq[1], s_kq[2]}, qb2[3] = {s_kq[3], s_kq[4], s_kq[5]};
+                if (qa[0] <= qb2[0]) key_child_box(nd.kf, qa, qb2, lo, hi);
+            }
+            ckeys = key_frame_make(lo, hi, cf);
+        }
         for (int side = 0; side < 2; side++) {
             NodeDev &ch = nodes[nd.child0 + side];
             ch.begin = side == 0 ? nd.begin : nd.begin + nL;
@@ -508,6 +606,8 @@
             ch.slot = -1; ch.child0 = -1; ch.nchild = 0;
             ch.klin = nd.klin; ch.kquad = nd.kquad;
             ch.psplit = split | (nd.degenerate ? 0x10000 : 0);
+            ch.keys = ckeys ? 1 : 0;
+            if (ckeys) ch.kf = cf;
             double s0[NQ], s1[NQ];
 #pragma unroll
             for (int q = 0; q < NQ; q++) {
@@ -715,7 +815,7 @@
     }
 }
 
-template <bool W, bool INV, bool NT>
+template <bool W, bool INV, bool NT, bool KEYS>
 __global__ __launch_bounds__(256, (W || INV) ? 2 : 3) void k_scatter_bin(QuantBuffers qb, const Tile *__restrict__ tiles, int ntiles, NodeDev *nodes,
                                                                         const NodeDev *__restrict__ nodes_ro,
                                                                         const unsigned long long *__restrict__ tileoff, const int from_end,
@@ -805,6 +905,9 @@
         const double m0L = c0.mean[0], m1L = c0.mean[1], m2L = c0.mean[2], m0R = c1.mean[0], m1R = c1.mean[1], m2R = c1.mean[2];
         BinK kinv{0.0, 0.0};
         if constexpr (INV) kinv = nd.kquad;
+        KeyFrame kfr{};
+        unsigned *dk = nullptr;
+        if constexpr (KEYS) { kfr = c0.kf; dk = qb.key[1 - nd.buf]; }
         const size_t slack = (size_t)(W ? 4 : 3) * qb.N + (size_t)lane;
 #pragma unroll
         for (int r = 0; r < R; r++) {
@@ -815,6 +918,7 @@
             const size_t dst = (right ? baseR + eR : baseL + eL) + (cr[r] >> 8);
             dx[none ? slack : dst] = x[r]; dy[none ? slack - qb.N : dst] = y[r]; dz[none ? slack - 2 * qb.N : dst] = z[r];
             if constexpr (W) dw[none ? slack - 3 * qb.N : dst] = w[r];
+            if constexpr (KEYS) dk[none ? qb.N + (size_t)lane : dst] = key_pack(kfr, x[r], y[r], z[r]);
             const double rf = right ? 1.0 : 0.0, lf = ch == 0u ? 1.0 : 0.0;
             const double ex = x[r] - (right ? m0R : m0L), ey = y[r] - (right ? m1R : m1L), ez = z[r] - (right ? m2R : m2L);
             const double wx = w[r] * ex, wy = w[r] * ey, wz = w[r] * ez;
@@ -937,11 +1041,11 @@
 }
 
 void launch_minmax(const QuantBuffers &qb, const Tile *d_tiles, int ntiles, size_t px, NodeDev *d_nodes, hipStream_t s, bool from_end,
-                   const RoundDyn *dyn, const double *px_src, const RoundLists *lists) {
+                   MinmaxRoute *d_route, const RoundDyn *dyn, const double *px_src, const RoundLists *lists) {
     if (!ntiles) return;
-    KTIME_DYN("k_minmax", s, 24.0, px, px_src);
-    if (dyn && lists) hipLaunchKernelGGL(k_minmax<true>, ntiles, 256, 0, s, qb, d_tiles, d_nodes, from_end ? 1 : 0, dyn, *lists);
-    else hipLaunchKernelGGL(k_minmax<false>, ntiles, 256, 0, s, qb, d_tiles, d_nodes, from_end ? 1 : 0, dyn, RoundLists{});
+    KTIME_DYN("k_minmax_keys", s, 24.0, px, px_src);
+    if (dyn && lists) hipLaunchKernelGGL(k_minmax_keys<true>, ntiles, 256, 0, s, qb, d_tiles, d_nodes, from_end ? 1 : 0, dyn, *lists, d_route);
+    else hipLaunchKernelGGL(k_minmax_keys<false>, ntiles, 256, 0, s, qb, d_tiles, d_nodes, from_end ? 1 : 0, dyn, RoundLists{}, d_route);
     HIP_CHECK(hipGetLastError());
 }
 
@@ -1059,37 +1163,40 @@
 
 std::atomic<int> g_debug_fault{0};
 void launch_cut(bool weighted, NodeDev *d_nodes, const int *d_round_nodes, int nround, const double *d_hist,
-                const unsigned long long *d_hsize, const unsigned int *d_hcount, unsigned char *d_lut, hipStream_t s, const RoundDyn *dyn, const double *nr_src) {
+                const unsigned long long *d_hsize, const unsigned int *d_hcount, unsigned char *d_lut, hipStream_t s, const RoundDyn *dyn, const double *nr_src,
+                const KeyRoot &kroot) {
     if (!nround) return;
     KTIME_DYN("k_cut", s, (double)kNQ_LQ * 2 * kBuckets * 8, nround, nr_src);
     const int fault = g_debug_fault.load(std::memory_order_relaxed);
-    if (weighted) hipLaunchKernelGGL(k_cut<true>, nround, 512, 0, s, d_nodes, d_round_nodes, d_hist, d_hsize, d_hcount, d_lut, fault, dyn);
-    else hipLaunchKernelGGL(k_cut<false>, nround, 512, 0, s, d_nodes, d_round_nodes, d_hist, d_hsize, d_hcount, d_lut, fault, dyn);
+    if (weighted) hipLaunchKernelGGL(k_cut<true>, nround, 512, 0, s, d_nodes, d_round_nodes, d_hist, d_hsize, d_hcount, d_lut, fault, dyn, kroot);
+    else hipLaunchKernelGGL(k_cut<false>, nround, 512, 0, s, d_nodes, d_round_nodes, d_hist, d_hsize, d_hcount, d_lut, fault, dyn, kroot);
     HIP_CHECK(hipGetLastError());
 }
 
 void launch_partition(const QuantBuffers &qb, const Tile *d_ptiles, int nptiles, size_t px, const int *d_round_nodes,
                       const int *d_node_tile0, int nround, NodeDev *d_nodes, const unsigned char *d_lut,
                       unsigned int *d_tilecnt, unsigned long long *d_tileoff, bool fuse_cov, hipStream_t s, bool invariant, bool from_end,
-                      const RoundDyn *dyn, const double *px_src, bool gated) {
+                      const RoundDyn *dyn, const double *px_src, bool gated, bool keys) {
     const int fe = (from_end ? 1 : 0) | (gated ? 2 : 0);
     if (!nround) return;
     if (nptiles) { KTIME_DYN("k_count", s, 2.0, px, px_src); hipLaunchKernelGGL(k_count, nptiles, 256, 0, s, qb, d_ptiles, d_nodes, d_lut, d_tilecnt, fe & 1, dyn); }
     { KTIME_DYN("k_scan", s, 12.0 * kMaxChildren / (double)kTileP, dyn ? px : (size_t)nptiles * kTileP, px_src);
       hipLaunchKernelGGL(k_scan, nround, 1024, 0, s, d_round_nodes, d_node_tile0, d_nodes, d_tilecnt, d_tileoff, dyn); }
     if (nptiles) {
-        KTIME_DYN(fuse_cov ? "k_scatter_cov" : "k_scatter", s, (qb.weighted ? 66.0 : 50.0), px, px_src);
+        KTIME_DYN(fuse_cov ? "k_scatter_cov" : "k_scatter", s, (qb.weighted ? 66.0 : 50.0) + (fuse_cov && keys ? 4.0 : 0.0), px, px_src);
         if (fuse_cov) {
             const int gb = std::min(nptiles, 256 * ((invariant || qb.weighted) ? 2 : 3));
             const bool nt = 2 * (size_t)(qb.weighted ? 4 : 3) * qb.N * sizeof(double) > kInfinityCacheBytes;
             auto go = [&](auto kernel) {
                 hipLaunchKernelGGL(kernel, gb, 256, 0, s, qb, d_ptiles, nptiles, d_nodes, (const NodeDev *)d_nodes, d_tileoff, fe, dyn);
             };
-            if (invariant) {
-                if (qb.weighted) { if (nt) go(k_scatter_bin<true, true, true>); else go(k_scatter_bin<true, true, false>); }
-                else { if (nt) go(k_scatter_bin<false, true, true>); else go(k_scatter_bin<false, true, false>); }
-            } else if (qb.weighted) { if (nt) go(k_scatter_bin<true, false, true>); else go(k_scatter_bin<true, false, false>); }
-            else { if (nt) go(k_scatter_bin<false, false, true>); else go(k_scatter_bin<false, false, false>); }
+            auto pick = [&](auto w, auto inv, auto ntl) {
+                constexpr bool Wc = decltype(w)::value, Ic = decltype(inv)::value, Nc = decltype(ntl)::value;
+                if (keys) go(k_scatter_bin<Wc, Ic, Nc, true>); else go(k_scatter_bin<Wc, Ic, Nc, false>);
+            };
+            auto pick_nt = [&](auto w, auto inv) { if (nt) pick(w, inv, std::true_type{}); else pick(w, inv, std::false_type{}); };
+            if (invariant) { if (qb.weighted) pick_nt(std::true_type{}, std::true_type{}); else pick_nt(std::false_type{}, std::true_type{}); }
+            else { if (qb.weighted) pick_nt(std::true_type{}, std::false_type{}); else pick_nt(std::false_type{}, std::false_type{}); }
             if (gated) {
                 HIP_CHECK(hipGetLastError());
                 const int fg = (from_end ? 1 : 0) | 4;
```

Result: no change. 3165, median of 2 (-0.1%).
